# LiYu0524/Domain-RAG

Hardware: AMD Instinct MI355X
Metric: composited images/sec @1024^2, 30 Flux-Redux steps (higher is better)
Workload: dtype bf16; 1 GPU; Flux-Redux outpaint (Fill) 1024x1024, 30 steps, batch=8 per GPU (BASELINE configs[2]); global_batch=8, parallelism=dp1, weights=seeded random init of the FLUX.1-Fill-dev architecture

## Files before the change

domain-rag_amd/_lib.py:

```python
from __future__ import annotations

import ctypes
import os

HERE = os.path.dirname(os.path.abspath(__file__))
LIB_PATH = os.path.join(HERE, "lib", "libdomainrag_hip.so")
if os.environ.get("DRAG_LIB"):
    LIB_PATH = os.environ["DRAG_LIB"]

c_void_p, c_int, c_int64, c_float = ctypes.c_void_p, ctypes.c_int32, ctypes.c_int64, ctypes.c_float


class GemmArgs(ctypes.Structure):
    _fields_ = [
        ("A", c_void_p), ("W", c_void_p), ("C", c_void_p),
        ("bias", c_void_p), ("gate", c_void_p), ("resid", c_void_p),
        ("M", c_int), ("N", c_int), ("K", c_int),
        ("lda", c_int), ("a_rows_per_batch", c_int), ("a_batch_stride", c_int64),
        ("ldc", c_int), ("c_rows_per_batch", c_int), ("c_batch_stride", c_int64),
        ("ldg", c_int), ("act", c_int), ("act_n0", c_int), ("out_f32", c_int),
        ("C2", c_void_p), ("ldc2", c_int), ("n_split", c_int),
    ]


class ConvArgs(ctypes.Structure):
    _fields_ = [("x", c_void_p), ("w", c_void_p), ("y", c_void_p), ("bias", c_void_p), ("resid", c_void_p)] + \
               [(n, c_int) for n in ("B", "Ho", "Wo", "Hp", "Wp", "Cin", "Cout", "ldy", "stride", "oy", "ox", "act")]


class ResampleArgs(ctypes.Structure):
    _fields_ = [("src", c_void_p), ("dst", c_void_p), ("tmp", c_void_p), ("batch", c_int), ("channels", c_int),
                ("src_h", c_int), ("src_w", c_int), ("src_image_stride", c_int64), ("src_row_stride", c_int),
                ("out_h", c_int), ("out_w", c_int), ("dst_image_stride", c_int64), ("dst_row_stride", c_int),
                ("kx", c_void_p), ("bx", c_void_p), ("ksize_x", c_int), ("ky", c_void_p), ("by", c_void_p), ("ksize_y", c_int),
                ("tmp_row0", c_int), ("tmp_rows", c_int), ("src_col0", c_int), ("src_row0", c_int)]


class Conv2dF32Args(ctypes.Structure):
    _fields_ = [(n, c_void_p) for n in ("x", "w", "y", "scale", "shift", "addend", "resid")] + \
               [(n, c_int) for n in ("B", "Hi", "Wi", "Cin", "ldx", "Ho", "Wo", "Cout", "ldy", "ld_add", "ld_res",
                                     "KH", "KW", "stride", "pad", "pad_mode", "transposed", "act")]


SIGNATURES = {
    "drag_version": (c_int, []),
    "drag_last_error": (ctypes.c_char_p, []),
    "drag_set_option": (c_int, [ctypes.c_char_p, c_int]),
    "drag_get_option": (c_int, [ctypes.c_char_p, ctypes.POINTER(ctypes.c_int32)]),
    "drag_option_name": (ctypes.c_char_p, [c_int]),
    "drag_experiments_built": (c_int, []),
    "drag_gemm_bf16": (c_int, [ctypes.POINTER(GemmArgs), c_void_p]),
    "drag_gemm_bf16_pair": (c_int, [ctypes.POINTER(GemmArgs), ctypes.POINTER(GemmArgs), c_void_p]),
    "drag_gemm_bf16_pair_merges": (c_int, [c_int, c_int, c_int, c_int]),
    "drag_gemm_bf16_choice": (c_int, [c_int, c_int, c_int, c_int]),
    "drag_conv3x3_bf16_choice": (c_int, [c_int64, c_int, c_int]),
    "drag_gemm_bf16_cost": (c_int64, [c_int, c_int, c_int, c_int]),
    "drag_gemm_set_workspace": (c_int, [c_void_p, c_int64]),
    "drag_gemm_bf16_splitk_slices": (c_int, [ctypes.POINTER(GemmArgs)]),
    "drag_gemm_bf16_pair_splitk_slices": (c_int, [ctypes.POINTER(GemmArgs), ctypes.POINTER(GemmArgs)]),
    "drag_qk_norm_rope_vt_bf16": (c_int, [c_void_p] * 8 + [c_int] * 5 + [c_float, c_void_p]),
    "drag_attention_bf16": (c_int, [c_void_p] * 4 + [c_int] * 4 + [c_int64, c_int, c_int64, c_float, c_void_p]),
    "drag_k_norm_rope_vt_bf16": (c_int, [c_void_p] * 6 + [c_int] * 5 + [c_float, c_void_p]),
    "drag_attention_qprep_bf16": (c_int, [c_void_p] * 4 + [c_int] * 4 + [c_int64, c_int, c_int64, c_float] + [c_void_p] * 4 + [c_int, c_float, c_void_p]),
    "drag_attention_bf16_choice": (c_int, [c_int, c_int, c_int]),
    "drag_attention_v_bf16": (c_int, [c_void_p] * 4 + [c_int] * 4 + [c_int64, c_int, c_int64, c_float] + [c_void_p] * 4 + [c_int, c_float, c_void_p]),
    "drag_layernorm_modulate_bf16": (c_int, [c_void_p] * 6 + [c_int] * 4 + [c_int64, c_int, c_int, c_float, c_void_p]),
    "drag_act_bf16": (c_int, [c_void_p, c_void_p, c_int64, c_int, c_void_p]),
    "drag_timestep_embedding_bf16": (c_int, [c_void_p, c_void_p, c_int, c_int, c_void_p]),
    "drag_flow_euler_step_bf16": (c_int, [c_void_p, c_void_p, c_float, c_int64, c_void_p]),
    "drag_add_bf16": (c_int, [c_void_p, c_void_p, c_void_p, c_int64, c_void_p]),
    "drag_cast_f32_to_bf16": (c_int, [c_void_p, c_void_p, c_int64, c_void_p]),
    "drag_cast_bf16_to_f32": (c_int, [c_void_p, c_void_p, c_int64, c_void_p]),
    "drag_cosine_topk_workspace_bytes": (c_int64, [c_int64, c_int]),
    "drag_cosine_topk_f32": (c_int, [c_void_p, c_void_p, c_int64, c_int, c_int, c_int, c_void_p, c_void_p, c_void_p, c_void_p]),
    "drag_cosine_scores_f32": (c_int, [c_void_p, c_void_p, c_int64, c_int, c_int, c_void_p, c_void_p]),
    "drag_l2_normalize_f32": (c_int, [c_void_p, c_int64, c_int, c_void_p]),
    "drag_patchify_u8": (c_int, [c_void_p, c_void_p] + [c_int] * 5 + [ctypes.POINTER(c_float), ctypes.POINTER(c_float), c_void_p]),
    "drag_resample_u8": (c_int, [ctypes.POINTER(ResampleArgs), c_void_p]),
    "drag_scale_sum_bf16": (c_int, [c_void_p, c_void_p, c_void_p, c_int, c_int, c_int64, c_void_p]),
    "drag_resnet_stem_style_workspace_bytes": (c_int64, [c_int] * 3),
    "drag_resnet_stem_style_f32": (c_int, [c_void_p] * 5 + [c_int] * 3 + [c_float, c_void_p, c_void_p]),
    "drag_patchify_f32_nchw": (c_int, [c_void_p, c_void_p] + [c_int] * 5 + [c_void_p]),
    "drag_conv3x3_bf16": (c_int, [ctypes.POINTER(ConvArgs), c_void_p]),
    "drag_groupnorm_workspace_bytes": (c_int64, [c_int] * 4),
    "drag_groupnorm_silu_bf16": (c_int, [c_void_p] * 4 + [c_int] * 7 + [c_float, c_void_p, c_void_p]),
    "drag_pad_copy_bf16": (c_int, [c_void_p, c_void_p] + [c_int] * 5 + [c_void_p]),
    "drag_softmax_rows_f32_bf16": (c_int, [c_void_p, c_void_p, c_int64, c_int, c_int, c_float, c_void_p]),
    "drag_unpack_latents_bf16": (c_int, [c_void_p, c_void_p] + [c_int] * 5 + [c_float, c_float, c_void_p]),
    "drag_sample_pack_latents_bf16": (c_int, [c_void_p] * 3 + [c_int] * 5 + [c_float, c_float, c_void_p]),
    "drag_image_preprocess_u8": (c_int, [c_void_p] * 3 + [c_int] * 4 + [c_void_p]),
    "drag_image_postprocess_u8": (c_int, [c_void_p, c_void_p, c_int64, c_int, c_void_p]),
    "drag_mask_pack_u8": (c_int, [c_void_p, c_void_p] + [c_int] * 4 + [c_void_p]),
    "drag_flow_euler_rows_bf16": (c_int, [c_void_p, c_void_p, c_int64, c_int, c_int, c_int, c_float, c_void_p]),
    "drag_scale_noise_rows_bf16": (c_int, [c_void_p, c_void_p, c_int64, c_int, c_int, c_int, c_float, c_void_p]),
    "drag_conv2d_f32": (c_int, [ctypes.POINTER(Conv2dF32Args), c_void_p]),
    "drag_rfft2_f32": (c_int, [c_void_p] * 3 + [c_int] * 5 + [c_void_p] * 3),
    "drag_irfft2_f32": (c_int, [c_void_p] * 4 + [c_int] * 6 + [c_void_p] * 3),
    "drag_lama_prepare_u8": (c_int, [c_void_p] * 3 + [c_int] * 4 + [c_void_p]),
    "drag_vit_prepare_u8": (c_int, [c_void_p, c_void_p, c_int64, ctypes.POINTER(c_float), ctypes.POINTER(c_float), c_void_p]),
    "drag_vit_prepare_f32": (c_int, [c_void_p, c_void_p, c_int, c_int64, c_void_p]),
    "drag_layernorm_f32": (c_int, [c_void_p] * 4 + [c_int64, c_int, c_int64, c_int64, c_float, c_void_p]),
    "drag_clip_embed_ln_f32": (c_int, [c_void_p] * 6 + [c_int] * 3 + [c_float, c_void_p]),
    "drag_attention_small_f32": (c_int, [c_void_p, c_void_p] + [c_int] * 6 + [c_float, c_void_p]),
    "drag_lama_blend_u8": (c_int, [c_void_p, c_int, c_void_p, c_void_p, c_void_p] + [c_int] * 4 + [c_void_p]),
    "drag_cv_resize_linear_u8_f32": (c_int, [c_void_p] * 5 + [c_int] * 3 + [c_void_p]),
    "drag_textenc_attention_bf16": (c_int, [c_void_p] * 4 + [c_int] * 4 + [c_int64, c_int, c_int64, c_float, c_void_p, c_int, c_int, c_void_p]),
    "drag_t5_rmsnorm_bf16": (c_int, [c_void_p] * 3 + [c_int, c_int, c_float, c_void_p]),
    "drag_gated_new_gelu_bf16": (c_int, [c_void_p, c_void_p, c_int64, c_int, c_void_p]),
    "drag_quick_gelu_bf16": (c_int, [c_void_p, c_void_p, c_int64, c_void_p]),
    "drag_embed_gather_bf16": (c_int, [c_void_p] * 4 + [c_int64, c_int, c_int, c_int64, c_void_p]),
    "drag_file_sizes": (c_int, [c_void_p, c_int64, c_void_p, c_int]),
    "drag_read_files": (c_int, [c_void_p, c_int64, c_void_p, c_void_p, c_void_p, c_int]),
    "drag_jpeg_parse": (c_int, [c_void_p, c_void_p, c_int, c_void_p, c_void_p]),
    "drag_jpeg_decode_rgb": (c_int, [c_void_p] * 4 + [c_int, c_int64, c_int64, c_void_p, c_int64] + [c_void_p] * 5),
    "drag_png_plan": (c_int, [c_int] * 4 + [c_void_p, c_void_p]),
    "drag_png_encode": (c_int, [c_void_p] + [c_int] * 4 + [c_void_p, c_int64, c_void_p, c_int64, c_void_p, c_void_p]),
}

_lib = None


def load() -> ctypes.CDLL:
    global _lib
    if _lib is not None:
        return _lib
    if not os.path.exists(LIB_PATH):
        raise RuntimeError(
            f"{LIB_PATH} not found: the HIP extension has not been built "
            "(run `python -c 'import __graft_entry__ as g; g.build()'`). "
            "domain-rag_amd has no CPU / eager fallback.")
    import torch
    lib = ctypes.CDLL(LIB_PATH)
    for name, (res, args) in SIGNATURES.items():
        fn = getattr(lib, name)
        fn.restype = res
        fn.argtypes = args
    _lib = lib
    return lib


def check(rc: int, what: str) -> None:
    if rc != 0:
        msg = load().drag_last_error().decode(errors="replace")
        raise RuntimeError(f"{what} failed (rc={rc}): {msg}")
```

domain-rag_amd/csrc/attention.hip:

```cpp
#include "drag_common.h"
#pragma clang diagnostic ignored "-Winline-asm"
#include "attn_q64_tile.h"
#ifdef DRAG_EXPERIMENTS
#include "attn_q64_tile_exp.h"
#endif
#include <stdlib.h>
#include <type_traits>

namespace {

struct PrepArgs {
  bf16_t* qkv;
  bf16_t* vt;
  const bf16_t *wq_txt, *wk_txt, *wq_img, *wk_img;
  const float *cosT, *sinT;
  int B, S, H, ld, s_txt, s_pad;
  float eps;
  int skip_q;
};

__global__ __launch_bounds__(256) void qk_norm_rope_vt_kernel(PrepArgs p) {
  __shared__ __attribute__((aligned(16))) bf16_t sv[64 * 136];
  const int tid = threadIdx.x;
  const int s0 = blockIdx.x * 64, h = blockIdx.y, b = blockIdx.z;
// ... 12 lines not shown
      const bool ok = s < p.S;
      const int sc = ok ? s : p.S - 1;
      bf16_t* ptr = base + (long long)sc * p.ld + which * HD + h * 128 + sub * 8;
      const u32x4_t raw = *(const u32x4_t*)ptr;
      float x[8];
#pragma unroll
      for (int j = 0; j < 4; ++j) {
        x[2 * j] = bf2f((bf16_t)(raw[j] & 0xffff));
        x[2 * j + 1] = bf2f((bf16_t)(raw[j] >> 16));
      }
      float ss = 0.f;
#pragma unroll
      for (int j = 0; j < 8; ++j) ss += x[j] * x[j];
      ss += __shfl_xor(ss, 8, 64);
      ss += __shfl_xor(ss, 4, 64);
      ss += __shfl_xor(ss, 2, 64);
      ss += __shfl_xor(ss, 1, 64);
      const float rs = rsqrtf(ss * (1.0f / 128.0f) + p.eps);
      u32x4_t wr = (u32x4_t){0u, 0u, 0u, 0u};
      if (do_norm) {
        const bf16_t* wsel = which == 0 ? (sc < p.s_txt ? p.wq_txt : p.wq_img) : (sc < p.s_txt ? p.wk_txt : p.wk_img);
        wr = *(const u32x4_t*)(wsel + sub * 8);
      }
      f32x4_t c4 = (f32x4_t){1.f, 1.f, 1.f, 1.f}, s4 = (f32x4_t){0.f, 0.f, 0.f, 0.f};
      if (do_rope) {
        c4 = *(const f32x4_t*)(p.cosT + (long long)sc * 64 + sub * 4);
        s4 = *(const f32x4_t*)(p.sinT + (long long)sc * 64 + sub * 4);
      }
      u32x4_t o;
#pragma unroll
      for (int j = 0; j < 4; ++j) {
        float a0 = x[2 * j], a1 = x[2 * j + 1];
        if (do_norm) {
          a0 = rbf(rbf(a0 * rs) * bf2f((bf16_t)(wr[j] & 0xffff)));
          a1 = rbf(rbf(a1 * rs) * bf2f((bf16_t)(wr[j] >> 16)));
        }
        const float r0 = a0 * c4[j] - a1 * s4[j];
        const float r1 = a1 * c4[j] + a0 * s4[j];
        o[j] = pack2bf(r0, r1);
      }
      if (ok) *(u32x4_t*)ptr = o;
    }
  }

  if (p.vt == nullptr) return;
  for (int i = tid; i < 64 * 16; i += 256) {
    const int r = i >> 4, c = i & 15;
    const int s = s0 + r;
    u32x4_t v = (u32x4_t){0u, 0u, 0u, 0u};
    if (s < p.S) v = *(const u32x4_t*)(base + (long long)s * p.ld + 2 * HD + h * 128 + c * 8);
    *(u32x4_t*)(sv + r * 136 + c * 8) = v;
  }
  __syncthreads();
  bf16_t* vtb = p.vt + ((long long)(b * p.H + h) * 128) * p.s_pad + s0;
  for (int i = tid; i < 128 * 8; i += 256) {
    const int d = i >> 3, g8 = i & 7;
    uint32_t w[4];
#pragma unroll
    for (int j = 0; j < 8; j += 2) {
      const int q0 = 8 * g8 + j, q1 = q0 + 1;
      const int k0 = (q0 & ~15) + 8 * (((q0 & 15) & 7) >> 2) + 4 * ((q0 & 15) >> 3) + (q0 & 3);
      const int k1 = (q1 & ~15) + 8 * (((q1 & 15) & 7) >> 2) + 4 * ((q1 & 15) >> 3) + (q1 & 3);
      w[j >> 1] = (uint32_t)sv[k0 * 136 + d] | ((uint32_t)sv[k1 * 136 + d] << 16);
    }
    *(u32x4_t*)(vtb + (long long)d * p.s_pad + 8 * g8) = (u32x4_t){w[0], w[1], w[2], w[3]};
  }
}

struct AttnArgs {
  const bf16_t *q, *k, *vt;
  const bf16_t* v;
  bf16_t* out;
  int B, S, H, ld_qk, ld_o, s_pad;
  long long qk_bs, o_bs;
  float c;
  unsigned k_bytes, vt_bytes;
  unsigned k_bytes_all, vt_bytes_all;
  const bf16_t *wq_txt, *wq_img;
  const float *cosT, *sinT;
  int s_txt;
  float eps;
  int tune;
  int items;
};

constexpr float DEFER_THR = 8.0f;
constexpr int KT_BYTES = 64 * 256;
constexpr int VT_BYTES = 128 * 128;

template <int NW, int SCHED, bool QPREP, bool PMAX, bool VROW = false, bool PERSIST = false>
__global__ __launch_bounds__(512, 2) void attention_d128_kernel(AttnArgs p) {
  __shared__ __attribute__((aligned(16))) char smem[2 * KT_BYTES + 2 * VT_BYTES];
  const int w = wave_id(), l = lane_id();
  const int hh = l >> 5;
  constexpr int QB = NW * 32;
  constexpr int CPW = 16 / NW;
  const int nqb = (p.S + QB - 1) / QB;
  const int xcd = blockIdx.x & 7;
  int loc = blockIdx.x >> 3;
  const int nloc = ((p.B * p.H + 7) / 8) * nqb;
  const int lstep = PERSIST ? (int)(gridDim.x >> 3) : nloc;
  if (((loc / nqb) * 8 + xcd) >= p.B * p.H) return;
  int b, h, q0;
  unsigned soK, soV;
  auto item_offsets = [&](int lc, int& bb, int& hd, unsigned& ok, unsigned& ov) {
    const int bh = (lc / nqb) * 8 + xcd;
    bb = bh / p.H; hd = bh - bb * p.H;
    ok = (unsigned)(((long long)bb * p.qk_bs + hd * 128) * 2);
    ov = VROW ? ok : (unsigned)((((long long)(bb * p.H + hd)) * 128) * p.s_pad * 2);
  };
  item_offsets(loc, b, h, soK, soV);
  q0 = (loc - (loc / nqb) * nqb) * QB + w * 32;

  bf16x8_t qf[8];
  __amdgpu_buffer_rsrc_t rsK, rsV;
  if constexpr (PERSIST) {
    rsK = __builtin_amdgcn_make_buffer_rsrc((void*)p.k, 0, p.k_bytes_all, 0x00020000);
    rsV = __builtin_amdgcn_make_buffer_rsrc((void*)(VROW ? p.v : p.vt), 0, VROW ? p.k_bytes_all : p.vt_bytes_all, 0x00020000);
  } else {
    const long long kb = ((long long)b * p.qk_bs + h * 128) * 2;
    rsK = __builtin_amdgcn_make_buffer_rsrc((void*)((const char*)p.k + kb), 0, p.k_bytes, 0x00020000);
    if constexpr (VROW) rsV = __builtin_amdgcn_make_buffer_rsrc((void*)((const char*)p.v + kb), 0, p.k_bytes, 0x00020000);
    else rsV = __builtin_amdgcn_make_buffer_rsrc((void*)((const char*)p.vt + (long long)(b * p.H + h) * 128 * p.s_pad * 2), 0, p.vt_bytes, 0x00020000);
    soK = 0; soV = 0;
  }
  unsigned soKn = soK, soVn = soV;
  int krow[4];
  unsigned kslot[4], voff[4];
  const unsigned vrslot = (unsigned)(((l & 15) ^ (4 * ((l >> 4) & 3))) * 16);
#pragma unroll
  for (int i = 0; i < 4; ++i) {
    if (i >= CPW) break;
    const int c = w * CPW + i;
    krow[i] = c * 4 + (l >> 4);
    kslot[i] = (unsigned)(((l & 15) ^ (krow[i] & 15)) * 16);
    const int vrow = c * 8 + (l >> 3);
    const int vslot = (l & 7) ^ ((vrow >> 1) & 7);
    voff[i] = (unsigned)(((long long)vrow * p.s_pad + vslot * 8) * 2);
  }
  auto stage_k1 = [&](int buf, int kv0, int i) {
    const int c = w * CPW + i;
    const bool nx = PERSIST && kv0 >= p.s_pad;
    const int kvr = nx ? kv0 - p.s_pad : kv0;
    const int kr = min(kvr + krow[i], p.S - 1);
    const unsigned ko = (unsigned)((long long)kr * p.ld_qk * 2) + kslot[i];
    __builtin_amdgcn_raw_ptr_buffer_load_lds(rsK, (DRAG_LDS void*)((DRAG_LDS char*)smem + buf * KT_BYTES + c * 1024), 16, ko, nx ? soKn : soK, 0, 0);
  };
  auto stage_k = [&](int buf, int kv0) {
#pragma unroll
    for (int i = 0; i < 4; ++i) {
      if (i >= CPW) break;
      stage_k1(buf, kv0, i);
    }
  };
  auto stage_v1 = [&](int buf, int kv0, int i) {
    const int c = w * CPW + i;
    const bool nx = PERSIST && kv0 >= p.s_pad;
    const int kvr = nx ? kv0 - p.s_pad : kv0;
    const unsigned so = nx ? soVn : soV;
    DRAG_LDS char* dV = (DRAG_LDS char*)smem + 2 * KT_BYTES + buf * VT_BYTES + c * 1024;
    if constexpr (VROW) {
      const int vr = min(kvr + krow[i], p.S - 1);
      __builtin_amdgcn_raw_ptr_buffer_load_lds(rsV, (DRAG_LDS void*)dV, 16, (unsigned)((long long)vr * p.ld_qk * 2) + vrslot, so, 0, 0);
    } else {
      __builtin_amdgcn_raw_ptr_buffer_load_lds(rsV, (DRAG_LDS void*)dV, 16, voff[i], so + (unsigned)(kvr * 2), 0, 0);
    }
  };
  auto stage_v = [&](int buf, int kv0) {
#pragma unroll
    for (int i = 0; i < 4; ++i) {
      if (i >= CPW) break;
      stage_v1(buf, kv0, i);
    }
  };

  const int krd = (l & 31) * 256;
  const int kx = l & 15;
  const int vrd = (l & 31) * 128;
  const int vx = ((l & 31) >> 1) & 7;

  f32x16_t oacc[4];
  float m_run, l_run;

  const int nkv = p.s_pad / 64;
  f32x16_t scur[2], snext[2];
  {
  int ak[8], av[4];
#pragma unroll
  for (int ks = 0; ks < 8; ++ks) ak[ks] = krd + (((2 * ks + hh) ^ kx) << 4);
#pragma unroll
  for (int s2 = 0; s2 < 4; ++s2) av[s2] = vrd + (((2 * s2 + hh) ^ vx) << 4);
  int avd[4];
  {
    const int si = l & 15, g1 = (l >> 4) & 1;
#pragma unroll
// ... 110 lines not shown
    asm volatile("s_waitcnt vmcnt(0)" ::: "memory");
    __syncthreads();
    const float mt = PMAX ? mt_carry : mask_and_max(sc, kv0);
    if (!__all((mt - m_run) * p.c <= DEFER_THR)) {
      const float m_new = fmaxf(m_run, mt);
      const float alpha = __builtin_amdgcn_exp2f((m_run - m_new) * p.c);
      l_run *= alpha;
      m_run = m_new;
#pragma unroll
      for (int i = 0; i < 4; ++i)
#pragma unroll
        for (int r = 0; r < 16; ++r) oacc[i][r] *= alpha;
    }
    const float nmc = -(m_run * p.c);
    float ps = 0.f;
    u32x4_t pk[4];
    {
      bf16x8_t kf = *(const bf16x8_t*)(smem + (ak[0] + KN));
      bf16x8_t vpipe;
#pragma unroll
      for (int g = 0; g < 16; ++g) {
        const bf16x8_t kcur = kf;
        if (g < 15) {
          const int t1 = (g + 1) >> 3, ks1 = (g + 1) & 7;
          kf = *(const bf16x8_t*)(smem + (ak[ks1] + (KN + t1 * (32 * 256))));
        }
        bf16x8_t vfg;
        if (SCHED == 1 && g >= 4) vfg = read_v((g >> 2) - 1, g & 3, VB);
        if (SCHED == 2) {
          vfg = vpipe;
          if (g >= 3 && g < 15) vpipe = read_v(((g + 1) >> 2) - 1, (g + 1) & 3, VB);
        }
        sn[g >> 3] = __builtin_amdgcn_mfma_f32_32x32x16_bf16(kcur, qf[g & 7], (g & 7) == 0 ? zero16 : sn[g >> 3], 0, 0, 0);
        if (g < CPW) stage_k1(PAR, kv0 + 128, g);
        else if (g < 2 * CPW) stage_v1((PAR + 1) & 1, kv0 + 64, g - CPW);
        float y0, y1;
        asm volatile("v_fma_f32 %0, %2, %4, %5\n\tv_fma_f32 %1, %3, %4, %5"
                     : "=&v"(y0), "=&v"(y1) : "v"(sc[g >> 3][(2 * g) & 15]), "v"(sc[g >> 3][((2 * g) & 15) + 1]), "s"(p.c), "v"(nmc));
        const float e0 = __builtin_amdgcn_exp2f(y0);
        const float e1 = __builtin_amdgcn_exp2f(y1);
        ps += e0 + e1;
        uint32_t wd = pack2bf(e0, e1);
        asm volatile("" : "+v"(wd), "+v"(ps));
        pk[g >> 2][g & 3] = wd;
        if (SCHED >= 1 && g >= 4)
          oacc[g & 3] = __builtin_amdgcn_mfma_f32_32x32x16_bf16(vfg, __builtin_bit_cast(bf16x8_t, pk[(g >> 2) - 1]), oacc[g & 3], 0, 0, 0);
        __builtin_amdgcn_sched_barrier(0);
      }
    }
    l_run += ps;
    bf16x8_t pf[4];
#pragma unroll
    for (int s2 = 0; s2 < 4; ++s2) pf[s2] = __builtin_bit_cast(bf16x8_t, pk[s2]);
#pragma unroll
    for (int s2 = (SCHED >= 1 ? 3 : 0); s2 < 4; ++s2)
#pragma unroll
      for (int dt = 0; dt < 4; ++dt) {
        const bf16x8_t vf = read_v(s2, dt, VB);
        oacc[dt] = __builtin_amdgcn_mfma_f32_32x32x16_bf16(vf, pf[s2], oacc[dt], 0, 0, 0);
      }
    if (PMAX) mt_carry = mask_and_max(sn, kv0 + 64);
  };
  for (int it = 0; it < nkv; it += 2) {
    body(it, std::integral_constant<int, 0>{}, scur, snext);
    if (it + 1 < nkv) body(it + 1, std::integral_constant<int, 1>{}, snext, scur);
  }

  const float lt = l_run + __shfl_xor(l_run, 32, 64);
  const float inv = 1.0f / lt;
  const int qrow = q0 + (l & 31);
  if (p.tune & 2) {
    bf16_t* op = p.out + (long long)b * p.o_bs + (long long)qrow * p.ld_o + h * 128 + 8 * hh;
#pragma unroll
    for (int dt = 0; dt < 4; ++dt)
#pragma unroll
      for (int g = 0; g < 4; g += 2) {
        uint32_t a0 = pack2bf(oacc[dt][4 * g] * inv, oacc[dt][4 * g + 1] * inv);
        uint32_t a1 = pack2bf(oacc[dt][4 * g + 2] * inv, oacc[dt][4 * g + 3] * inv);
        uint32_t b0 = pack2bf(oacc[dt][4 * g + 4] * inv, oacc[dt][4 * g + 5] * inv);
        uint32_t b1 = pack2bf(oacc[dt][4 * g + 6] * inv, oacc[dt][4 * g + 7] * inv);
        const auto r0 = __builtin_amdgcn_permlane32_swap(a0, b0, false, false);
        const auto r1 = __builtin_amdgcn_permlane32_swap(a1, b1, false, false);
        const u32x4_t o = {r0[0], r1[0], r0[1], r1[1]};
        if (qrow < p.S) *(u32x4_t*)(op + 32 * dt + 8 * g) = o;
      }
  } else if (qrow < p.S) {
    bf16_t* op = p.out + (long long)b * p.o_bs + (long long)qrow * p.ld_o + h * 128 + 4 * hh;
#pragma unroll
    for (int dt = 0; dt < 4; ++dt)
#pragma unroll
      for (int g = 0; g < 4; ++g) {
        u32x2_t o;
        o[0] = pack2bf(oacc[dt][4 * g] * inv, oacc[dt][4 * g + 1] * inv);
        o[1] = pack2bf(oacc[dt][4 * g + 2] * inv, oacc[dt][4 * g + 3] * inv);
        *(u32x2_t*)(op + 32 * dt + 8 * g) = o;
      }
  }
  if (!has_next) break;
  loc += lstep;
  item_offsets(loc, b, h, soK, soV);
  q0 = (loc - (loc / nqb) * nqb) * QB + w * 32;
  }
  }
}


#define Q64_MFMA_S0(d, a, b) asm volatile("v_mfma_f32_32x32x16_bf16 %0, %1, %2, 0" : "=&v"(d) : "v"(a), "a"(b))
#define Q64_MFMA_S(d, a, b) asm volatile("v_mfma_f32_32x32x16_bf16 %0, %1, %2, %0" : "+v"(d) : "v"(a), "a"(b))
#define Q64_SETTLE_S(s4) asm volatile("s_nop 15\n\ts_nop 7" : "+v"(s4[0][0]), "+v"(s4[0][1]), "+v"(s4[1][0]), "+v"(s4[1][1]))
#define Q64_SETTLE_O(o, qg) asm volatile("s_nop 15\n\ts_nop 7" : "+a"(o[qg][0]), "+a"(o[qg][1]), "+a"(o[qg][2]), "+a"(o[qg][3]))

template <int OFF>
__device__ __forceinline__ void q64_lds_read(bf16x8_t& d, unsigned addr) { asm volatile("ds_read_b128 %0, %1 offset:%2" : "=v"(d) : "v"(addr), "n"(OFF)); }
template <int N>
__device__ __forceinline__ void q64_landed(bf16x8_t& a) { asm volatile("s_waitcnt lgkmcnt(%1)" : "+v"(a) : "n"(N)); }
template <int N>
__device__ __forceinline__ void q64_landed(bf16x8_t& a, bf16x8_t& b) { asm volatile("s_waitcnt lgkmcnt(%2)" : "+v"(a), "+v"(b) : "n"(N)); }
template <int N>
__device__ __forceinline__ void q64_landed(bf16x8_t& a, bf16x8_t& b, bf16x8_t& c, bf16x8_t& d) {
  asm volatile("s_waitcnt lgkmcnt(%4)" : "+v"(a), "+v"(b), "+v"(c), "+v"(d) : "n"(N));
}
__device__ __forceinline__ void q64_max3(float& d, float a, float b, float c) { asm volatile("v_max3_f32 %0, %1, %2, %3" : "=v"(d) : "v"(a), "v"(b), "v"(c)); }
#define Q64P_MFMA_O(d, a, pw) asm volatile("v_mfma_f32_32x32x16_bf16 %0, %1, %2, %0" : "+a"(d) : "v"(a), "v"(pw))
#define Q64_V1 "v_fma_f32 %[ya0], %[sa0], %[c], %[nma]\n\t"
#define Q64_V2 "v_fma_f32 %[ya1], %[sa1], %[c], %[nma]\n\t"
#define Q64_V3 "v_exp_f32 %[ya0], %[ya0]\n\t"
#define Q64_V4 "v_fma_f32 %[yb0], %[sb0], %[c], %[nmb]\n\t"
#define Q64_V5 "v_exp_f32 %[ya1], %[ya1]\n\t"
#define Q64_V6 "v_fma_f32 %[yb1], %[sb1], %[c], %[nmb]\n\t"
#define Q64_V7 "v_add_f32 %[ta], %[ya0], %[ya1]\n\t"
#define Q64_V8 "v_exp_f32 %[yb0], %[yb0]\n\t"
#define Q64_V9 "v_add_f32 %[psa], %[psa], %[ta]\n\t"
#define Q64_V10 "v_exp_f32 %[yb1], %[yb1]\n\t"
#define Q64_V11 "v_cvt_pk_bf16_f32 %[wa], %[ya0], %[ya1]\n\t"
#define Q64_V12 "v_add_f32 %[tb], %[yb0], %[yb1]\n\t"
#define Q64_V13 "v_add_f32 %[psb], %[psb], %[tb]\n\t"
#define Q64_V14 "v_cvt_pk_bf16_f32 %[wb], %[yb0], %[yb1]"
#define Q64_SC_IN(sc, T, E0) [sa0] "v"(sc[0][T][E0]), [sa1] "v"(sc[0][T][E0 + 1]), [sb0] "v"(sc[1][T][E0]), [sb1] "v"(sc[1][T][E0 + 1])
#define Q64_STEP_HI_A(C0, S0CONS, N, o0_, o1_, vf_, p0_, p1_, s0_, kf_, q0_, d1_, a1_, F1, d2_, a2_, F2, sc, T, E0, cc, nma_, nmb_)        \
  asm volatile("s_waitcnt lgkmcnt(%[n])\n\t" Q64_V1 Q64_V2                                                                                \
               "v_mfma_f32_32x32x16_bf16 %[o0], %[vf], %[p0], %[o0]\n\t"                                                                  \
               "ds_read_b128 %[d1], %[a1] offset:%[f1]\n\t" Q64_V3                                                                        \
               "v_mfma_f32_32x32x16_bf16 %[o1], %[vf], %[p1], %[o1]\n\t"                                                                  \
               "ds_read_b128 %[d2], %[a2] offset:%[f2]\n\t" Q64_V4 Q64_V5 Q64_V6                                                          \
               "v_mfma_f32_32x32x16_bf16 %[s0], %[kf], %[q0], " C0                                                                        \
               : [o0] "+a"(o0_), [o1] "+a"(o1_), [s0] S0CONS(s0_), [d1] "=&v"(d1_), [d2] "=&v"(d2_), [ya0] "=&v"(yA0), [ya1] "=&v"(yA1),  \
                 [yb0] "=&v"(yB0), [yb1] "=&v"(yB1)                                                                                       \
               : [n] "n"(N), [vf] "v"(vf_), [p0] "v"(p0_), [p1] "v"(p1_), [kf] "v"(kf_), [q0] "a"(q0_), [a1] "v"(a1_), [f1] "n"(F1),      \
                 [a2] "v"(a2_), [f2] "n"(F2), Q64_SC_IN(sc, T, E0), [c] "s"(cc), [nma] "v"(nma_), [nmb] "v"(nmb_))
#define Q64_STEP_HI_B(C1, S1CONS, s1_, kf_, q1_)                                                                                          \
  asm volatile(Q64_V7 Q64_V8 Q64_V9 Q64_V10 "v_mfma_f32_32x32x16_bf16 %[s1], %[kf], %[q1], " C1 "\n\t" Q64_V11 Q64_V12 Q64_V13 Q64_V14    \
               : [s1] S1CONS(s1_), [yb0] "+v"(yB0), [yb1] "+v"(yB1), [psa] "+v"(ps[0]), [psb] "+v"(ps[1]), [wa] "=&v"(wA),                \
                 [wb] "=&v"(wB), [ta] "=&v"(sA), [tb] "=&v"(sB)                                                                           \
               : [kf] "v"(kf_), [q1] "a"(q1_), [ya0] "v"(yA0), [ya1] "v"(yA1))
#define Q64_STEP_LO_A(WAIT, READ2, C0, C1, SCONS, N, s0_, s1_, kf_, q0_, q1_, d1_, a1_, F1, d2_, a2_, F2, sc, T, E0, cc, nma_, nmb_)       \
  asm volatile(WAIT Q64_V1 Q64_V2 "v_mfma_f32_32x32x16_bf16 %[s0], %[kf], %[q0], " C0 "\n\t"                                              \
               "ds_read_b128 %[d1], %[a1] offset:%[f1]\n\t" READ2 Q64_V3 Q64_V4 Q64_V5 Q64_V6 Q64_V7                                      \
               "v_mfma_f32_32x32x16_bf16 %[s1], %[kf], %[q1], " C1                                                                        \
               : [s0] SCONS(s0_), [s1] SCONS(s1_), [d1] "=&v"(d1_), [d2] "=&v"(d2_), [ya0] "=&v"(yA0), [ya1] "=&v"(yA1), [yb0] "=&v"(yB0),\
                 [yb1] "=&v"(yB1), [ta] "=&v"(sA)                                                                                         \
               : [n] "n"(N), [kf] "v"(kf_), [q0] "a"(q0_), [q1] "a"(q1_), [a1] "v"(a1_), [f1] "n"(F1), [a2] "v"(a2_), [f2] "n"(F2),       \
                 Q64_SC_IN(sc, T, E0), [c] "s"(cc), [nma] "v"(nma_), [nmb] "v"(nmb_))
#define Q64_STEP_LO_B(kf_)                                                                                                                \
  asm volatile(Q64_V8 Q64_V9 Q64_V10 Q64_V11 Q64_V12 Q64_V13 Q64_V14                                                                      \
               : [yb0] "+v"(yB0), [yb1] "+v"(yB1), [psa] "+v"(ps[0]), [psb] "+v"(ps[1]), [wa] "=&v"(wA), [wb] "=&v"(wB), [tb] "=&v"(sB)   \
               : [ya0] "v"(yA0), [ya1] "v"(yA1), [ta] "v"(sA), "v"(kf_))
template <class F, int G = 0>
__device__ __forceinline__ void q64_unroll16(F&& f) {
  if constexpr (G < 16) {
    f(std::integral_constant<int, G>{});
    q64_unroll16<F, G + 1>(f);
  }
}

#if DRAG_EXP
__device__ unsigned long long g_attn_stamps[512];
#define ATTN_STAMP(slot)                                                                                                  \
  do {                                                                                                                     \
    if (blockIdx.x == 0 && w == 0 && l == 0 && (slot) < 512) g_attn_stamps[(slot)] = __builtin_amdgcn_s_memtime();         \
  } while (0)
#else
#define ATTN_STAMP(slot) do { } while (0)
#endif
template <bool QPREP>
__global__ __launch_bounds__(256, 1) void attention_q64_kernel(AttnArgs p) {
  extern __shared__ __attribute__((aligned(16))) char smem[];
  const int w = wave_id(), l = lane_id();
  ATTN_STAMP(0);
  const int hh = l >> 5;
  constexpr int QB = 256, CPW = 4;
  const int nqb = (p.S + QB - 1) / QB;
  struct Item { int b, h, q0; };
  auto decode = [&](int item, Item& t) -> bool {
    const int xcd = item & 7, loc = item >> 3;
    const int bh = (loc / nqb) * 8 + xcd;
    t.b = bh / p.H;
    t.h = bh - t.b * p.H;
    t.q0 = (loc - (loc / nqb) * nqb) * QB + w * 64;
    return bh < p.B * p.H;
  };
  int item = (int)blockIdx.x;
  Item cur;
  if (!decode(item, cur)) return;

  bf16x8_t qf[2][8];
  auto k_descr = [&](const Item& t) {
    return __builtin_amdgcn_make_buffer_rsrc((void*)(p.k + (long long)t.b * p.qk_bs + t.h * 128), 0, p.k_bytes, 0x00020000);
  };
  auto v_descr = [&](const Item& t) {
    return __builtin_amdgcn_make_buffer_rsrc((void*)(p.vt + ((long long)(t.b * p.H + t.h) * 128) * p.s_pad), 0, p.vt_bytes, 0x00020000);
  };
  __amdgpu_buffer_rsrc_t rsK = k_descr(cur), rsV = v_descr(cur);
  int ksub = 0, vsub = 0;
  unsigned koff[4], voff[4];
#pragma unroll
  for (int i = 0; i < 4; ++i) {
    const int c = w * CPW + i;
    const int krow = c * 4 + (l >> 4);
    koff[i] = (unsigned)krow * (unsigned)(p.ld_qk * 2) + (unsigned)(((l & 15) ^ (krow & 15)) * 16);
    const int vrow = c * 8 + (l >> 3);
    const int vslot = (l & 7) ^ ((vrow >> 1) & 7);
    voff[i] = (unsigned)(((long long)vrow * p.s_pad + vslot * 8) * 2);
  }
  auto stage_k1 = [&](int buf, int kv0, int i) {
    const int c = w * CPW + i;
    const unsigned ko = koff[i] + (unsigned)(kv0 - ksub) * (unsigned)(p.ld_qk * 2);
    __builtin_amdgcn_raw_ptr_buffer_load_lds(rsK, (DRAG_LDS void*)((DRAG_LDS char*)smem + buf * KT_BYTES + c * 1024), 16, ko, 0, 0, 0);
  };
  auto stage_v1 = [&](int buf, int kv0, int i) {
    const int c = w * CPW + i;
    __builtin_amdgcn_raw_ptr_buffer_load_lds(rsV, (DRAG_LDS void*)((DRAG_LDS char*)smem + 2 * KT_BYTES + buf * VT_BYTES + c * 1024),
                                             16, voff[i], (kv0 - vsub) * 2, 0, 0);
  };
  const int krd = (l & 31) * 256, kx = l & 15;
  const int vrd = (l & 31) * 128, vx = ((l & 31) >> 1) & 7;
  int ak[8], av[4];
#pragma unroll
  for (int ks = 0; ks < 8; ++ks) ak[ks] = krd + (((2 * ks + hh) ^ kx) << 4);
#pragma unroll
  for (int s2 = 0; s2 < 4; ++s2) av[s2] = vrd + (((2 * s2 + hh) ^ vx) << 4);
  const unsigned lds0 = (unsigned)(size_t)(DRAG_LDS char*)smem;
  unsigned akl[8], avl[4];
  {
#pragma unroll
    for (int i = 0; i < 8; ++i) akl[i] = lds0 + (unsigned)ak[i];
#pragma unroll
    for (int i = 0; i < 4; ++i) avl[i] = lds0 + (unsigned)av[i];
#pragma unroll
    for (int i = 0; i < 8; ++i) asm volatile("" : "+v"(akl[i]));
#pragma unroll
    for (int i = 0; i < 4; ++i) asm volatile("" : "+v"(avl[i]));
  }

  const int nkv = p.s_pad / 64;
  const bool paired = (nkv & 1) == 0 && nkv >= 4;
  const f32x16_t zero16 = {0.f, 0.f, 0.f, 0.f, 0.f, 0.f, 0.f, 0.f, 0.f, 0.f, 0.f, 0.f, 0.f, 0.f, 0.f, 0.f};
  auto stage_first = [&]() {
#pragma unroll
    for (int i = 0; i < 4; ++i) stage_k1(0, 0, i);
#pragma unroll
    for (int i = 0; i < 4; ++i) stage_v1(0, 0, i);
    if (nkv > 1) {
#pragma unroll
      for (int i = 0; i < 4; ++i) stage_k1(1, 64, i);
    }
  };
  auto lane_now = [&]() { int v = l; asm volatile("" : "+v"(v)); return v; };
  DRAG_LDS char* const qlds = (DRAG_LDS char*)smem + 2 * KT_BYTES + 2 * VT_BYTES + w * 16384;
  auto q_request = [&](const Item& t, const int ll) {
    __amdgpu_buffer_rsrc_t rsQ = __builtin_amdgcn_make_buffer_rsrc((void*)(p.q + (long long)t.b * p.qk_bs + t.h * 128), 0, p.k_bytes, 0x00020000);
#pragma unroll
    for (int qg = 0; qg < 2; ++qg) {
      const int qr = min(t.q0 + 32 * qg + (ll & 31), p.S - 1);
      const unsigned vo = (unsigned)qr * (unsigned)(p.ld_qk * 2) + (unsigned)((ll >> 5) * 16);
#pragma unroll
      for (int ks = 0; ks < 8; ++ks)
        __builtin_amdgcn_raw_ptr_buffer_load_lds(rsQ, (DRAG_LDS void*)(qlds + (qg * 8 + ks) * 1024), 16, vo, ks * 32, 0, 0);
    }
  };
  auto q_fragments = [&](const Item& t, const int ll) {
    const int hh = ll >> 5;
// ... 214 lines not shown
        dma();
        Q64_STEP_HI_B("%[s1]", "+v", sn[1][T], kfr[G % 3], qa[1][G & 7]);
      } else if constexpr (G == 8) {
        Q64_STEP_HI_A("0", "=&v", younger, oacc[0][G & 3], oacc[1][G & 3], vfr[G % 3], pk[0][(G >> 2) - 1], pk[1][(G >> 2) - 1], sn[0][T],
                      kfr[G % 3], qa[0][G & 7], kfr[(G + 2) % 3], akl[(G + 2) & 7], KOFF, vfr[(G + 2) % 3], avl[((G + 2) >> 2) - 1], VOFF, sc, T, E0,
                      p.c, nmc[0], nmc[1]);
        dma();
        Q64_STEP_HI_B("0", "=&v", sn[1][T], kfr[G % 3], qa[1][G & 7]);
      } else if constexpr (G >= 4) {
        Q64_STEP_HI_A("%[s0]", "+v", younger, oacc[0][G & 3], oacc[1][G & 3], vfr[G % 3], pk[0][(G >> 2) - 1], pk[1][(G >> 2) - 1], sn[0][T],
                      kfr[G % 3], qa[0][G & 7], kfr[(G + 2) % 3], akl[(G + 2) & 7], KOFF, vfr[(G + 2) % 3], avl[((G + 2) >> 2) - 1], VOFF, sc, T, E0,
                      p.c, nmc[0], nmc[1]);
        dma();
        Q64_STEP_HI_B("%[s1]", "+v", sn[1][T], kfr[G % 3], qa[1][G & 7]);
      } else if constexpr (G == 0) {
        bf16x8_t none;
        Q64_STEP_LO_A("", "", "0", "0", "=&v", 0, sn[0][T], sn[1][T], kfr[0], qa[0][0], qa[1][0], kfr[2], akl[2], KOFF, none, akl[2], 0, sc, T, E0,
                      p.c, nmc[0], nmc[1]);
        dma();
        Q64_STEP_LO_B(kfr[0]);
      } else if constexpr (G == 1) {
        bf16x8_t none;
        Q64_STEP_LO_A("s_waitcnt lgkmcnt(%[n])\n\t", "", "%[s0]", "%[s1]", "+v", younger, sn[0][T], sn[1][T], kfr[G % 3], qa[0][G], qa[1][G],
                      kfr[(G + 2) % 3], akl[G + 2], KOFF, none, akl[2], 0, sc, T, E0, p.c, nmc[0], nmc[1]);
        dma();
        Q64_STEP_LO_B(kfr[G % 3]);
      } else {
        Q64_STEP_LO_A("s_waitcnt lgkmcnt(%[n])\n\t", "ds_read_b128 %[d2], %[a2] offset:%[f2]\n\t", "%[s0]", "%[s1]", "+v", younger, sn[0][T],
                      sn[1][T], kfr[G % 3], qa[0][G], qa[1][G], kfr[(G + 2) % 3], akl[G + 2], KOFF, vfr[(G + 2) % 3], avl[((G + 2) >> 2) - 1], VOFF,
                      sc, T, E0, p.c, nmc[0], nmc[1]);
        dma();
        Q64_STEP_LO_B(kfr[G % 3]);
      }
      pk[0][G >> 2][G & 3] = wA;
      pk[1][G >> 2][G & 3] = wB;
    };
    q64_unroll16(step);
    q64_landed<0>(vtr[0], vtr[1], vtr[2], vtr[3]);
#pragma unroll
    for (int qg = 0; qg < 2; ++qg) l_run[qg] += ps[qg];
  };
  {
    using P0 = std::integral_constant<int, 0>;
    using P1 = std::integral_constant<int, 1>;
    ATTN_STAMP(1);
    body(0, P0{}, scur, snext, std::true_type{});
    if (nkv > 1) body(1, P1{}, snext, scur, std::false_type{});
    for (int it = 2; it < nkv; it += 2) {
      body(it, P0{}, scur, snext, std::false_type{});
      if (it + 1 < nkv) body(it + 1, P1{}, snext, scur, std::false_type{});
    }
#pragma unroll
    for (int dt = 0; dt < 4; ++dt)
#pragma unroll
      for (int qg = 0; qg < 2; ++qg) Q64P_MFMA_O(oacc[qg][dt], vtr[dt], pk[qg][3]);
    ATTN_STAMP(2 + 2 * nkv);
  }
  const int le = lane_now();
  Item nxt = cur;
  if (has_next) {
    decode(item + (int)gridDim.x, nxt);
    q_request(nxt, le);
  }

#pragma unroll
  for (int qg = 0; qg < 2; ++qg) {
    Q64_SETTLE_O(oacc, qg);
    const float lt = l_run[qg] + __shfl_xor(l_run[qg], 32, 64);
    const float inv = 1.0f / lt;
    const int qrow = q0 + 32 * qg + (le & 31);
    if (p.tune & 2) {
      bf16_t* op = p.out + (long long)b * p.o_bs + (long long)qrow * p.ld_o + h * 128 + 8 * (le >> 5);
#pragma unroll
      for (int dt = 0; dt < 4; ++dt)
#pragma unroll
        for (int g = 0; g < 4; g += 2) {
          uint32_t a0 = pack2bf(oacc[qg][dt][4 * g] * inv, oacc[qg][dt][4 * g + 1] * inv);
          uint32_t a1 = pack2bf(oacc[qg][dt][4 * g + 2] * inv, oacc[qg][dt][4 * g + 3] * inv);
          uint32_t b0 = pack2bf(oacc[qg][dt][4 * g + 4] * inv, oacc[qg][dt][4 * g + 5] * inv);
          uint32_t b1 = pack2bf(oacc[qg][dt][4 * g + 6] * inv, oacc[qg][dt][4 * g + 7] * inv);
          const auto r0 = __builtin_amdgcn_permlane32_swap(a0, b0, false, false);
          const auto r1 = __builtin_amdgcn_permlane32_swap(a1, b1, false, false);
          const u32x4_t o = {r0[0], r1[0], r0[1], r1[1]};
          if (qrow < p.S) *(u32x4_t*)(op + 32 * dt + 8 * g) = o;
        }
    } else if (qrow < p.S) {
      bf16_t* op = p.out + (long long)b * p.o_bs + (long long)qrow * p.ld_o + h * 128 + 4 * (le >> 5);
#pragma unroll
      for (int dt = 0; dt < 4; ++dt)
#pragma unroll
        for (int g = 0; g < 4; ++g) {
          u32x2_t o;
          o[0] = pack2bf(oacc[qg][dt][4 * g] * inv, oacc[qg][dt][4 * g + 1] * inv);
          o[1] = pack2bf(oacc[qg][dt][4 * g + 2] * inv, oacc[qg][dt][4 * g + 3] * inv);
          *(u32x2_t*)(op + 32 * dt + 8 * g) = o;
        }
    }
  }
  ATTN_STAMP(3 + 2 * (p.s_pad / 64));
  if (!has_next) break;
  stores_behind = q0 + 64 <= p.S ? ((p.tune & 2) ? 16 : 32) : 0;
  wait_older_than_stores();
  q_fragments(nxt, le);
  q_to_agprs();
  ATTN_STAMP(5 + 2 * (p.s_pad / 64));
  item += (int)gridDim.x;
  cur = nxt;
  if (!paired) {
    rsK = k_descr(cur);
    rsV = v_descr(cur);
  }
  ksub = vsub = 0;
  staged = paired;
  }
}


typedef __attribute__((ext_vector_type(32))) float aq_f32x32_t;
typedef __attribute__((ext_vector_type(8))) uint32_t aq_u32x8_t;
typedef __attribute__((ext_vector_type(16))) uint32_t aq_u32x16_t;

template <bool QPREP, bool FOLD, int VAR = 0>
__global__ __launch_bounds__(256, 1) void attention_q64g_kernel(AttnArgs p) {
  static_assert(QPREP || !FOLD, "the fold needs the q preparation");
  static_assert(VAR == 0 || (FOLD && DRAG_EXP), "variants: fold form, experiment builds");
  extern __shared__ __attribute__((aligned(16))) char smem[];
  const int w = wave_id(), l = lane_id();
  constexpr int QB = 256, CPW = 4;
  const int nqb = (p.S + QB - 1) / QB;
  struct Item { int b, h, q0; };
  auto decode = [&](int item, Item& t) -> bool {
    const int xcd = item & 7, loc = item >> 3;
    const int bh = (loc / nqb) * 8 + xcd;
    t.b = bh / p.H;
    t.h = bh - t.b * p.H;
    t.q0 = (loc - (loc / nqb) * nqb) * QB + w * 64;
    return bh < p.B * p.H;
  };
  int item = (int)blockIdx.x;
  Item cur;
  if (!decode(item, cur)) return;
  auto k_descr = [&](const Item& t) {
    return __builtin_amdgcn_make_buffer_rsrc((void*)(p.k + (long long)t.b * p.qk_bs + t.h * 128), 0, p.k_bytes, 0x00020000);
  };
  auto v_descr = [&](const Item& t) {
    return __builtin_amdgcn_make_buffer_rsrc((void*)(p.vt + ((long long)(t.b * p.H + t.h) * 128) * p.s_pad), 0, p.vt_bytes, 0x00020000);
  };
  auto lane_now = [&]() { int v = l; asm volatile("" : "+v"(v)); return v; };
  const unsigned lds0 = (unsigned)(size_t)(DRAG_LDS char*)smem;
  auto lane_consts = [&](int ll, aq_u32x8_t& akl, aq_u32x16_t& misc) {
    const int hh = ll >> 5;
    const int krd = (ll & 31) * 256, kx = ll & 15;
    const int vrd = (ll & 31) * 128, vx = ((ll & 31) >> 1) & 7;
#pragma unroll
    for (int ks = 0; ks < 8; ++ks) akl[ks] = lds0 + (unsigned)(krd + (((2 * ks + hh) ^ kx) << 4));
#pragma unroll
    for (int s2 = 0; s2 < 4; ++s2) misc[s2] = lds0 + (unsigned)(vrd + (((2 * s2 + hh) ^ vx) << 4));
#pragma unroll
    for (int i = 0; i < 4; ++i) {
      const int c = w * CPW + i;
      const int krow = c * 4 + (ll >> 4);
      misc[4 + i] = (unsigned)krow * (unsigned)(p.ld_qk * 2) + (unsigned)(((ll & 15) ^ (krow & 15)) * 16);
      const int vrow = c * 8 + (ll >> 3);
      const int vslot = (ll & 7) ^ ((vrow >> 1) & 7);
      misc[8 + i] = (unsigned)(((long long)vrow * p.s_pad + vslot * 8) * 2);
      misc[12 + i] = 0u;
    }
  };
  auto stage_first = [&](const Item& t, int ll) {
    __amdgpu_buffer_rsrc_t rsK = k_descr(t), rsV = v_descr(t);
#pragma unroll
    for (int i = 0; i < 4; ++i) {
      const int c = w * CPW + i;
      const int krow = c * 4 + (ll >> 4);
      const unsigned ko = (unsigned)krow * (unsigned)(p.ld_qk * 2) + (unsigned)(((ll & 15) ^ (krow & 15)) * 16);
      const int vrow = c * 8 + (ll >> 3);
      const int vslot = (ll & 7) ^ ((vrow >> 1) & 7);
      const unsigned vo = (unsigned)(((long long)vrow * p.s_pad + vslot * 8) * 2);
      __builtin_amdgcn_raw_ptr_buffer_load_lds(rsK, (DRAG_LDS void*)((DRAG_LDS char*)smem + c * 1024), 16, ko, 0, 0, 0);
      __builtin_amdgcn_raw_ptr_buffer_load_lds(rsV, (DRAG_LDS void*)((DRAG_LDS char*)smem + 2 * KT_BYTES + c * 1024), 16, vo, 0, 0, 0);
      __builtin_amdgcn_raw_ptr_buffer_load_lds(rsK, (DRAG_LDS void*)((DRAG_LDS char*)smem + KT_BYTES + c * 1024), 16,
                                               ko + 64u * (unsigned)(p.ld_qk * 2), 0, 0, 0);
    }
  };
  DRAG_LDS char* const qlds = (DRAG_LDS char*)smem + 2 * KT_BYTES + 2 * VT_BYTES + w * 16384;
  auto q_request = [&](const Item& t, const int ll) {
    __amdgpu_buffer_rsrc_t rsQ = __builtin_amdgcn_make_buffer_rsrc((void*)(p.q + (long long)t.b * p.qk_bs + t.h * 128), 0, p.k_bytes, 0x00020000);
#pragma unroll
    for (int qg = 0; qg < 2; ++qg) {
      const int qr = min(t.q0 + 32 * qg + (ll & 31), p.S - 1);
      const unsigned vo = (unsigned)qr * (unsigned)(p.ld_qk * 2) + (unsigned)((ll >> 5) * 16);
#pragma unroll
      for (int ks = 0; ks < 8; ++ks)
        __builtin_amdgcn_raw_ptr_buffer_load_lds(rsQ, (DRAG_LDS void*)(qlds + (qg * 8 + ks) * 1024), 16, vo, ks * 32, 0, 0);
    }
  };
  auto q_fragments = [&](const Item& t, const int ll, aq_f32x32_t (&qin)[2]) {
    const int hh = ll >> 5;
#pragma unroll
    for (int qg = 0; qg < 2; ++qg) {
      u32x4_t raw[8];
#pragma unroll
      for (int ks = 0; ks < 8; ++ks) raw[ks] = *(const DRAG_LDS u32x4_t*)(qlds + (qg * 8 + ks) * 1024 + ll * 16);
      if constexpr (!QPREP) {
#pragma unroll
        for (int ks = 0; ks < 8; ++ks)
#pragma unroll
          for (int j = 0; j < 4; ++j) {
            const uint32_t word = raw[ks][j];
            qin[qg][4 * ks + j] = __builtin_bit_cast(float, word);
          }
      } else {
        const int qr = min(t.q0 + 32 * qg + (ll & 31), p.S - 1);
        const bf16_t* wsel = (qr < p.s_txt ? p.wq_txt : p.wq_img) + hh * 8;
        const float* cp = p.cosT + (long long)qr * 64 + hh * 4;
        const float* sp = p.sinT + (long long)qr * 64 + hh * 4;
        u32x4_t wr[8];
        f32x4_t c4[8], s4[8];
#pragma unroll
// ... 32 lines not shown
  q_request(cur, l);
  asm volatile("s_waitcnt vmcnt(0)" ::: "memory");
  q_fragments(cur, l, qin);
  int stores_behind = 0;
  auto wait_older_than_stores = [&]() {
    if (stores_behind == 16) asm volatile("s_waitcnt vmcnt(16)" ::: "memory");
    else if (stores_behind == 32) asm volatile("s_waitcnt vmcnt(32)" ::: "memory");
    else asm volatile("s_waitcnt vmcnt(0)" ::: "memory");
  };
  for (;;) {
    const int b = cur.b, h = cur.h, q0 = cur.q0;
    const bool has_next = item + (int)gridDim.x < p.items;
    Item nxt = cur;
    const bool have = has_next && decode(item + (int)gridDim.x, nxt);
    const __amdgpu_buffer_rsrc_t rsK = k_descr(cur), rsV = v_descr(cur);
    const __amdgpu_buffer_rsrc_t rsKn = have ? k_descr(nxt) : __builtin_amdgcn_make_buffer_rsrc((void*)p.k, 0, 0, 0x00020000);
    const __amdgpu_buffer_rsrc_t rsVn = have ? v_descr(nxt) : __builtin_amdgcn_make_buffer_rsrc((void*)p.vt, 0, 0, 0x00020000);
    aq_u32x8_t akl;
    aq_u32x16_t misc;
    lane_consts(lane_now(), akl, misc);
    const unsigned ldsw = (unsigned)__builtin_amdgcn_readfirstlane((int)(lds0 + (unsigned)w * 4096u));
    const unsigned npairs = (unsigned)(nkv - 2) / 2u;
    const unsigned ktile = 64u * (unsigned)(p.ld_qk * 2);
    const unsigned nvalid = (unsigned)(p.S - (nkv - 1) * 64);
    wait_older_than_stores();
    __syncthreads();
    aq_f32x32_t o4[4];
    f32x2_t lrun;
    [[maybe_unused]] f32x16_t lacc[2];
#define AQ64_OUTS "={a[0:31]}"(o4[0]), "={a[32:63]}"(o4[1]), "={a[64:95]}"(o4[2]), "={a[96:127]}"(o4[3]), "={v[208:209]}"(lrun)
#define AQ64_INS "{a[128:159]}"(qin[0]), "{a[160:191]}"(qin[1]), "{v[176:183]}"(akl), "{v[184:199]}"(misc), [rsk] "s"(rsK), [rsv] "s"(rsV), \
                 [rskn] "s"(rsKn), [rsvn] "s"(rsVn), [npairs] "s"(npairs), [ktile] "s"(ktile), [nvalid] "s"(nvalid), [ldsw] "s"(ldsw)
    if constexpr (!FOLD) asm volatile(AQ64_ITEM_NOFOLD : AQ64_OUTS : AQ64_INS, [c] "s"(p.c) : AQ64_CLOBBERS);
    else if constexpr (VAR == 0) asm volatile(AQ64_ITEM_FOLD : AQ64_OUTS : AQ64_INS : AQ64_CLOBBERS);
#if DRAG_EXP
    else if constexpr (VAR == 1) asm volatile(AQ64_ITEM_FOLD_V1 : AQ64_OUTS : AQ64_INS : AQ64_CLOBBERS);
    else if constexpr (VAR == 2) asm volatile(AQ64_ITEM_FOLD_V2 : AQ64_OUTS : AQ64_INS : AQ64_CLOBBERS);
    else if constexpr (VAR == 3) asm volatile(AQ64_ITEM_FOLD_V3 : AQ64_OUTS : AQ64_INS : AQ64_CLOBBERS);
    else if constexpr (VAR == 4) asm volatile(AQ64_ITEM_FOLD_V4 : AQ64_OUTS : AQ64_INS : AQ64_CLOBBERS);
    else if constexpr (VAR == 5) asm volatile(AQ64_ITEM_FOLD_V5 : AQ64_OUTS : AQ64_INS : AQ64_CLOBBERS);
    else if constexpr (VAR == 6) asm volatile(AQ64_ITEM_FOLD_V6 : AQ64_OUTS : AQ64_INS : AQ64_CLOBBERS);
    else if constexpr (VAR == 7) asm volatile(AQ64_ITEM_FOLD_V7 : AQ64_OUTS : AQ64_INS : AQ64_CLOBBERS);
    else if constexpr (VAR == 8) asm volatile(AQ64_ITEM_FOLD_V8 : AQ64_OUTS : AQ64_INS : AQ64_CLOBBERS);
    else if constexpr (VAR == 9) asm volatile(AQ64_ITEM_FOLD_V9 : AQ64_OUTS : AQ64_INS : AQ64_CLOBBERS);
    else if constexpr (VAR == 10) asm volatile(AQ64_ITEM_FOLD_V10 : AQ64_OUTS : AQ64_INS : AQ64_CLOBBERS);
    else if constexpr (VAR == 11) asm volatile(AQ64_ITEM_FOLD_V11 : AQ64_OUTS : AQ64_INS : AQ64_CLOBBERS);
    else if constexpr (VAR == 12) asm volatile(AQ64_ITEM_FOLD_V12 : AQ64_OUTS : AQ64_INS : AQ64_CLOBBERS);
    else if constexpr (VAR == 13) asm volatile(AQ64_ITEM_FOLD_V13 : AQ64_OUTS : AQ64_INS : AQ64_CLOBBERS);
    else if constexpr (VAR == 14) asm volatile(AQ64_ITEM_FOLD_V14 : AQ64_OUTS : AQ64_INS : AQ64_CLOBBERS);
    else if constexpr (VAR == 15) asm volatile(AQ64_ITEM_FOLD_V15 : AQ64_OUTS : AQ64_INS : AQ64_CLOBBERS);
    else if constexpr (VAR == 16) asm volatile(AQ64_ITEM_FOLD_V16 : AQ64_OUTS : AQ64_INS : AQ64_CLOBBERS);
    else if constexpr (VAR == 17) asm volatile(AQ64_ITEM_FOLD_V17 : AQ64_OUTS : AQ64_INS : AQ64_CLOBBERS);
    else if constexpr (VAR == 19) asm volatile(AQ64_ITEM_FOLD_V19 : AQ64_OUTS : AQ64_INS : AQ64_CLOBBERS);
    else if constexpr (VAR == 18)
      asm volatile(AQ64_ITEM_FOLD_V18
                   : "={a[0:31]}"(o4[0]), "={a[32:63]}"(o4[1]), "={a[64:95]}"(o4[2]), "={a[96:127]}"(o4[3]), "={a[224:239]}"(lacc[0]), "={a[240:255]}"(lacc[1])
                   : AQ64_INS : AQ64_CLOBBERS_LSUM);
#endif
#undef AQ64_OUTS
#undef AQ64_INS
    const int le = lane_now();
    if (has_next) q_request(nxt, le);
#pragma unroll
    for (int qg = 0; qg < 2; ++qg) {
      float lt;
      if constexpr (VAR == 18) lt = lacc[qg][0];
      else lt = lrun[qg] + __shfl_xor(lrun[qg], 32, 64);
      const float inv = 1.0f / lt;
      const int qrow = q0 + 32 * qg + (le & 31);
      auto oa = [&](int dt, int r) -> float { return o4[2 * qg + (dt >> 1)][16 * (dt & 1) + r]; };
      if (p.tune & 2) {
        bf16_t* op = p.out + (long long)b * p.o_bs + (long long)qrow * p.ld_o + h * 128 + 8 * (le >> 5);
#pragma unroll
        for (int dt = 0; dt < 4; ++dt)
#pragma unroll
          for (int g = 0; g < 4; g += 2) {
            uint32_t a0 = pack2bf(oa(dt, 4 * g) * inv, oa(dt, 4 * g + 1) * inv);
            uint32_t a1 = pack2bf(oa(dt, 4 * g + 2) * inv, oa(dt, 4 * g + 3) * inv);
            uint32_t b0 = pack2bf(oa(dt, 4 * g + 4) * inv, oa(dt, 4 * g + 5) * inv);
            uint32_t b1 = pack2bf(oa(dt, 4 * g + 6) * inv, oa(dt, 4 * g + 7) * inv);
            const auto r0 = __builtin_amdgcn_permlane32_swap(a0, b0, false, false);
            const auto r1 = __builtin_amdgcn_permlane32_swap(a1, b1, false, false);
            const u32x4_t o = {r0[0], r1[0], r0[1], r1[1]};
            if (qrow < p.S) *(u32x4_t*)(op + 32 * dt + 8 * g) = o;
          }
      } else if (qrow < p.S) {
        bf16_t* op = p.out + (long long)b * p.o_bs + (long long)qrow * p.ld_o + h * 128 + 4 * (le >> 5);
#pragma unroll
        for (int dt = 0; dt < 4; ++dt)
#pragma unroll
          for (int g = 0; g < 4; ++g) {
            u32x2_t o;
            o[0] = pack2bf(oa(dt, 4 * g) * inv, oa(dt, 4 * g + 1) * inv);
            o[1] = pack2bf(oa(dt, 4 * g + 2) * inv, oa(dt, 4 * g + 3) * inv);
            *(u32x2_t*)(op + 32 * dt + 8 * g) = o;
          }
      }
    }
    if (!has_next) break;
    stores_behind = q0 + 64 <= p.S ? ((p.tune & 2) ? 16 : 32) : 0;
    wait_older_than_stores();
    q_fragments(nxt, le, qin);
    item += (int)gridDim.x;
    cur = nxt;
  }
}

}

#if DRAG_EXP
extern "C" int drag_debug_attn_stamps(unsigned long long* host, int n) {
  return hipMemcpyFromSymbol(host, HIP_SYMBOL(g_attn_stamps), (size_t)n * sizeof(unsigned long long)) == hipSuccess ? 0 : -1;
}
#endif

extern "C" int drag_qk_norm_rope_vt_bf16(void* qkv, void* vt, const void* wq_txt, const void* wk_txt,
                                         const void* wq_img, const void* wk_img, const float* rope_cos,
                                         const float* rope_sin, int32_t B, int32_t S, int32_t H, int32_t ld,
                                         int32_t s_txt, float eps, void* stream) {
  DRAG_CHECK(qkv && vt, "drag_qk_norm_rope_vt_bf16: null pointer");
  DRAG_CHECK((wq_txt && wk_txt && wq_img && wk_img) || (!wq_txt && !wk_txt && !wq_img && !wk_img),
             "drag_qk_norm_rope_vt_bf16: norm weights are all-or-none");
  DRAG_CHECK((rope_cos == nullptr) == (rope_sin == nullptr), "drag_qk_norm_rope_vt_bf16: cos/sin come in pairs");
  DRAG_CHECK(B > 0 && S > 0 && H > 0 && ld >= 3 * H * 128 && ld % 8 == 0, "drag_qk_norm_rope_vt_bf16: bad shape");
  PrepArgs p;
  p.qkv = (bf16_t*)qkv; p.vt = (bf16_t*)vt;
  p.wq_txt = (const bf16_t*)wq_txt; p.wk_txt = (const bf16_t*)wk_txt;
  p.wq_img = (const bf16_t*)wq_img; p.wk_img = (const bf16_t*)wk_img;
  p.cosT = rope_cos; p.sinT = rope_sin;
  p.B = B; p.S = S; p.H = H; p.ld = ld; p.s_txt = s_txt; p.s_pad = (S + 63) / 64 * 64; p.eps = eps;
  p.skip_q = 0;
  hipLaunchKernelGGL(qk_norm_rope_vt_kernel, dim3((S + 63) / 64, H, B), dim3(256), 0, (hipStream_t)stream, p);
  DRAG_LAUNCH_CHECK();
  return 0;
}

extern "C" int drag_k_norm_rope_vt_bf16(void* qkv, void* vt, const void* wk_txt, const void* wk_img, const float* rope_cos,
                                        const float* rope_sin, int32_t B, int32_t S, int32_t H, int32_t ld, int32_t s_txt,
                                        float eps, void* stream) {
  DRAG_CHECK(qkv, "drag_k_norm_rope_vt_bf16: null pointer");
  DRAG_CHECK((wk_txt == nullptr) == (wk_img == nullptr), "drag_k_norm_rope_vt_bf16: norm weights come in pairs");
  DRAG_CHECK((rope_cos == nullptr) == (rope_sin == nullptr), "drag_k_norm_rope_vt_bf16: cos/sin come in pairs");
  DRAG_CHECK(B > 0 && S > 0 && H > 0 && ld >= 3 * H * 128 && ld % 8 == 0, "drag_k_norm_rope_vt_bf16: bad shape");
  PrepArgs p;
  p.qkv = (bf16_t*)qkv; p.vt = (bf16_t*)vt;
  p.wq_txt = (const bf16_t*)wk_txt; p.wk_txt = (const bf16_t*)wk_txt;
  p.wq_img = (const bf16_t*)wk_img; p.wk_img = (const bf16_t*)wk_img;
  p.cosT = rope_cos; p.sinT = rope_sin;
  p.B = B; p.S = S; p.H = H; p.ld = ld; p.s_txt = s_txt; p.s_pad = (S + 63) / 64 * 64; p.eps = eps;
  p.skip_q = 1;
  hipLaunchKernelGGL(qk_norm_rope_vt_kernel, dim3((S + 63) / 64, H, B), dim3(256), 0, (hipStream_t)stream, p);
  DRAG_LAUNCH_CHECK();
  return 0;
}

static int attention_launch(const void* q, const void* k, const void* vt, void* out, int32_t B, int32_t S, int32_t H,
                            int32_t ld_qk, int64_t qk_batch_stride, int32_t ld_o, int64_t o_batch_stride, float scale,
                            const void* wq_txt, const void* wq_img, const float* rope_cos, const float* rope_sin, int32_t s_txt,
                            float eps, void* stream, bool vrow = false);

static void attention_family(int32_t S, bool vrow, bool& w8, bool& q64) {
  w8 = !drag_opt(DRAG_OPT_ATTN_W4) && S >= 4096;
  const int q64opt = drag_opt(DRAG_OPT_ATTN_Q64);
  q64 = !vrow && q64opt != 2 && ((q64opt == 1 && S >= 1024) || (q64opt == 0 && w8 && (!DRAG_EXP || drag_opt(DRAG_OPT_ATTN_PERSIST) == 0)));
}

static bool attention_generated(int32_t S) {
  const int nkv = (S + 63) / 64;
  return drag_opt(DRAG_OPT_ATTN_GEN) != 1 && nkv % 2 == 0 && nkv >= 4;
}

extern "C" int drag_attention_bf16_choice(int32_t S, int32_t v_row_major, int32_t q_prep) {
  bool w8, q64;
  attention_family(S, v_row_major != 0, w8, q64);
  if (q64 && attention_generated(S)) return q_prep && drag_opt(DRAG_OPT_ATTN_GEN) != 2 ? 641 : 640;
  return q64 ? 64 : (w8 ? 8 : 4);
}

extern "C" int drag_attention_bf16(const void* q, const void* k, const void* vt, void* out, int32_t B, int32_t S,
                                   int32_t H, int32_t ld_qk, int64_t qk_batch_stride, int32_t ld_o,
                                   int64_t o_batch_stride, float scale, void* stream) {
  return attention_launch(q, k, vt, out, B, S, H, ld_qk, qk_batch_stride, ld_o, o_batch_stride, scale, nullptr, nullptr, nullptr,
                          nullptr, 0, 0.f, stream);
}

extern "C" int drag_attention_qprep_bf16(const void* q, const void* k, const void* vt, void* out, int32_t B, int32_t S,
                                         int32_t H, int32_t ld_qk, int64_t qk_batch_stride, int32_t ld_o,
                                         int64_t o_batch_stride, float scale, const void* wq_txt, const void* wq_img,
                                         const float* rope_cos, const float* rope_sin, int32_t s_txt, float eps, void* stream) {
  DRAG_CHECK(wq_txt && wq_img && rope_cos && rope_sin,
             "drag_attention_qprep_bf16: the fused q preparation needs both norm weights and both RoPE tables "
             "(drag_attention_bf16 takes an already prepared q)");
  DRAG_CHECK(s_txt >= 0 && s_txt <= S, "drag_attention_qprep_bf16: 0 <= s_txt <= S");
  return attention_launch(q, k, vt, out, B, S, H, ld_qk, qk_batch_stride, ld_o, o_batch_stride, scale, wq_txt, wq_img, rope_cos,
                          rope_sin, s_txt, eps, stream);
}

extern "C" int drag_attention_v_bf16(const void* q, const void* k, const void* v, void* out, int32_t B, int32_t S, int32_t H,
                                     int32_t ld_qk, int64_t qk_batch_stride, int32_t ld_o, int64_t o_batch_stride, float scale,
                                     const void* wq_txt, const void* wq_img, const float* rope_cos, const float* rope_sin,
                                     int32_t s_txt, float eps, void* stream) {
  const int given = (wq_txt != nullptr) + (wq_img != nullptr) + (rope_cos != nullptr) + (rope_sin != nullptr);
  DRAG_CHECK(given == 0 || given == 4, "drag_attention_v_bf16: the fused q preparation takes both norm weights and both RoPE tables, or none");
  DRAG_CHECK(given == 0 || (s_txt >= 0 && s_txt <= S), "drag_attention_v_bf16: 0 <= s_txt <= S");
  return attention_launch(q, k, v, out, B, S, H, ld_qk, qk_batch_stride, ld_o, o_batch_stride, scale, wq_txt, wq_img, rope_cos,
                          rope_sin, s_txt, eps, stream, true);
}

#if DRAG_EXP
static int persist_slots() {
  const int opt = drag_opt(DRAG_OPT_ATTN_PERSIST);
  if (opt >= 3) return opt;
  static int ncu8 = 0;
  if (ncu8 == 0) {
    int dev = 0, n = 0;
    if (hipGetDevice(&dev) != hipSuccess || hipDeviceGetAttribute(&n, hipDeviceAttributeMultiprocessorCount, dev) != hipSuccess || n <= 0) n = 256;
    ncu8 = n / 8 > 0 ? n / 8 : 1;
  }
  return ncu8;
}
#endif

static int attention_launch(const void* q, const void* k, const void* vt, void* out, int32_t B, int32_t S, int32_t H,
                            int32_t ld_qk, int64_t qk_batch_stride, int32_t ld_o, int64_t o_batch_stride, float scale,
                            const void* wq_txt, const void* wq_img, const float* rope_cos, const float* rope_sin, int32_t s_txt,
                            float eps, void* stream, bool vrow) {
  DRAG_CHECK(q && k && vt && out, "drag_attention_bf16: null pointer");
  DRAG_CHECK(B > 0 && S > 0 && H > 0, "drag_attention_bf16: bad shape");
  DRAG_CHECK(ld_qk % 8 == 0 && ld_o % 4 == 0, "drag_attention_bf16: ld_qk %% 8, ld_o %% 4 required");
  AttnArgs p;
  p.q = (const bf16_t*)q; p.k = (const bf16_t*)k; p.vt = (const bf16_t*)vt; p.v = (const bf16_t*)vt; p.out = (bf16_t*)out;
  p.B = B; p.S = S; p.H = H; p.ld_qk = ld_qk; p.ld_o = ld_o; p.s_pad = (S + 63) / 64 * 64;
  p.qk_bs = qk_batch_stride; p.o_bs = o_batch_stride;
  p.c = scale * 1.4426950408889634f;
  p.wq_txt = (const bf16_t*)wq_txt; p.wq_img = (const bf16_t*)wq_img; p.cosT = rope_cos; p.sinT = rope_sin;
  p.s_txt = s_txt; p.eps = eps;
  const long long kspan = ((long long)(S - 1) * ld_qk + 128) * 2;
  const long long vspan = (long long)128 * p.s_pad * 2;
  DRAG_CHECK(kspan < (1ll << 31), "drag_attention_bf16: K span must be < 2 GiB per (batch, head)");
  p.k_bytes = (unsigned)kspan; p.vt_bytes = (unsigned)vspan;
  const long long kall = ((long long)(B - 1) * qk_batch_stride + (H - 1) * 128) * 2 + kspan, vall = (long long)B * H * vspan;
  const bool fits32 = kall < (1ll << 32) && vall < (1ll << 32);
  p.k_bytes_all = fits32 ? (unsigned)kall : 0u; p.vt_bytes_all = fits32 ? (unsigned)vall : 0u;
  const int groups = (B * H + 7) / 8;
  bool w8, q64;
  attention_family(S, vrow, w8, q64);
  const int QB = (w8 || q64) ? 256 : 128;
  const int nqb2 = (S + QB - 1) / QB;
  const dim3 grid(8 * groups * nqb2);
  const int sched = drag_opt(DRAG_OPT_ATTN_SCHED);
  const bool qprep = wq_txt != nullptr;
  p.tune = drag_opt(DRAG_OPT_ATTN_TUNE);
  if (ld_o % 8 != 0 || ((uintptr_t)out & 15) != 0 || o_batch_stride % 8 != 0) p.tune &= ~2;
  const hipStream_t st = (hipStream_t)stream;
#define DRAG_ATTN_LAUNCH(NW, SC, QP, PM) hipLaunchKernelGGL((attention_d128_kernel<NW, SC, QP, PM>), grid, dim3(NW * 64), 0, st, p)
#define DRAG_ATTN_PICK(NW)                                                                           \
  do {                                                                                               \
    if (DRAG_EXP && sched == 3) { if (qprep) DRAG_ATTN_LAUNCH(NW, DRAG_EXP ? 2 : 1, true, true); else DRAG_ATTN_LAUNCH(NW, DRAG_EXP ? 2 : 1, false, true); }        \
    else if (sched >= 2) { if (qprep) DRAG_ATTN_LAUNCH(NW, 1, true, true); else DRAG_ATTN_LAUNCH(NW, 1, false, true); }   \
    else if (sched == 1) { if (qprep) DRAG_ATTN_LAUNCH(NW, 1, true, false); else DRAG_ATTN_LAUNCH(NW, 1, false, false); } \
    else { if (qprep) DRAG_ATTN_LAUNCH(NW, 0, true, false); else DRAG_ATTN_LAUNCH(NW, 0, false, false); }                 \
  } while (0)
  if (vrow) {
    if (w8) { if (qprep) hipLaunchKernelGGL((attention_d128_kernel<8, 1, true, true, true>), grid, dim3(512), 0, st, p);
              else hipLaunchKernelGGL((attention_d128_kernel<8, 1, false, true, true>), grid, dim3(512), 0, st, p); }
    else { if (qprep) hipLaunchKernelGGL((attention_d128_kernel<4, 1, true, true, true>), grid, dim3(256), 0, st, p);
           else hipLaunchKernelGGL((attention_d128_kernel<4, 1, false, true, true>), grid, dim3(256), 0, st, p); }
  } else if (q64) {
    constexpr int lds64 = 2 * KT_BYTES + 2 * VT_BYTES + 4 * 16384;
    static unsigned long long ready64 = 0;
    static int ncu64 = 0;
    int dev64 = 0;
    (void)hipGetDevice(&dev64);
    if (!((ready64 >> (dev64 & 63)) & 1ull)) {
      DRAG_CHECK(hipFuncSetAttribute(reinterpret_cast<const void*>(&attention_q64_kernel<true>), hipFuncAttributeMaxDynamicSharedMemorySize, lds64) == hipSuccess &&
                 hipFuncSetAttribute(reinterpret_cast<const void*>(&attention_q64_kernel<false>), hipFuncAttributeMaxDynamicSharedMemorySize, lds64) == hipSuccess,
                 "drag_attention: hipFuncSetAttribute(MaxDynamicSharedMemorySize) failed");
      ready64 |= 1ull << (dev64 & 63);
    }
    if (ncu64 == 0) {
      int n = 0;
      if (hipDeviceGetAttribute(&n, hipDeviceAttributeMultiprocessorCount, dev64) != hipSuccess || n <= 0) n = 256;
      ncu64 = (n & ~7) ? (n & ~7) : 8;
    }
    p.items = (int)grid.x;
    const int nkv64 = p.s_pad / 64;
    const int popt = drag_opt(DRAG_OPT_ATTN_WALK);
    const int pgrid = popt >= 8 && popt % 8 == 0 ? popt : ncu64;
    const bool walk = popt != 2 && (B * H) % 8 == 0 && (popt >= 8 || (nkv64 % 2 == 0 && nkv64 >= 4)) && p.items > pgrid;
    const dim3 grid64(walk ? (unsigned)pgrid : grid.x);
    const int gen = drag_opt(DRAG_OPT_ATTN_GEN);
    if (attention_generated(S)) {
      static unsigned long long readyg = 0;
      if (!((readyg >> (dev64 & 63)) & 1ull)) {
        DRAG_CHECK(hipFuncSetAttribute(reinterpret_cast<const void*>(&attention_q64g_kernel<true, true>), hipFuncAttributeMaxDynamicSharedMemorySize, lds64) == hipSuccess &&
                   hipFuncSetAttribute(reinterpret_cast<const void*>(&attention_q64g_kernel<true, false>), hipFuncAttributeMaxDynamicSharedMemorySize, lds64) == hipSuccess &&
                   hipFuncSetAttribute(reinterpret_cast<const void*>(&attention_q64g_kernel<false, false>), hipFuncAttributeMaxDynamicSharedMemorySize, lds64) == hipSuccess,
                   "drag_attention: hipFuncSetAttribute(MaxDynamicSharedMemorySize) failed");
        readyg |= 1ull << (dev64 & 63);
      }
#if DRAG_EXP
      if (qprep && gen >= 11 && gen <= 29) {
#define DRAG_AQV(V_) case 10 + V_: DRAG_CHECK(hipFuncSetAttribute(reinterpret_cast<const void*>(&attention_q64g_kernel<true, true, V_>), hipFuncAttributeMaxDynamicSharedMemorySize, lds64) == hipSuccess, "hipFuncSetAttribute"); \
        hipLaunchKernelGGL((attention_q64g_kernel<true, true, V_>), grid64, dim3(256), lds64, st, p); break
        switch (gen) { DRAG_AQV(1); DRAG_AQV(2); DRAG_AQV(3); DRAG_AQV(4); DRAG_AQV(5); DRAG_AQV(6); DRAG_AQV(7); DRAG_AQV(8); DRAG_AQV(9); DRAG_AQV(10); DRAG_AQV(11); DRAG_AQV(12); DRAG_AQV(13); DRAG_AQV(14); DRAG_AQV(15); DRAG_AQV(16); DRAG_AQV(17); DRAG_AQV(18); DRAG_AQV(19); }
#undef DRAG_AQV
      } else
#endif
      if (qprep && gen != 2) hipLaunchKernelGGL((attention_q64g_kernel<true, true>), grid64, dim3(256), lds64, st, p);
      else if (qprep) hipLaunchKernelGGL((attention_q64g_kernel<true, false>), grid64, dim3(256), lds64, st, p);
      else hipLaunchKernelGGL((attention_q64g_kernel<false, false>), grid64, dim3(256), lds64, st, p);
    } else if (qprep) hipLaunchKernelGGL((attention_q64_kernel<true>), grid64, dim3(256), lds64, st, p);
    else hipLaunchKernelGGL((attention_q64_kernel<false>), grid64, dim3(256), lds64, st, p);
#if DRAG_EXP
  } else if (w8 && sched == 2 && drag_opt(DRAG_OPT_ATTN_PERSIST) != 0 && fits32 && (B * H) % 8 == 0 && (p.s_pad / 64) % 2 == 0 &&
             nqb2 * groups > persist_slots()) {
    const dim3 pgrid(8 * persist_slots());
    if (qprep) hipLaunchKernelGGL((attention_d128_kernel<8, 1, true, true, false, true>), pgrid, dim3(512), 0, st, p);
    else hipLaunchKernelGGL((attention_d128_kernel<8, 1, false, true, false, true>), pgrid, dim3(512), 0, st, p);
#endif
  } else if (w8) DRAG_ATTN_PICK(8); else DRAG_ATTN_PICK(4);
#undef DRAG_ATTN_PICK
#undef DRAG_ATTN_LAUNCH
  DRAG_LAUNCH_CHECK();
  return 0;
}
```

domain-rag_amd/csrc/drag_common.h:

```cpp
#pragma once
#include <hip/hip_runtime.h>
#include <stdint.h>
#include "../../include/domainrag_hip.h"

typedef uint16_t bf16_t;

typedef __attribute__((ext_vector_type(8))) __bf16 bf16x8_t;
typedef __attribute__((ext_vector_type(8))) short short8_t;
typedef __attribute__((ext_vector_type(4))) short short4_t;
typedef __attribute__((ext_vector_type(4))) float f32x4_t;
typedef __attribute__((ext_vector_type(16))) float f32x16_t;
typedef __attribute__((ext_vector_type(4))) uint32_t u32x4_t;
typedef __attribute__((ext_vector_type(2))) uint32_t u32x2_t;

#define DRAG_LDS __attribute__((address_space(3)))

__device__ __forceinline__ float bf2f(bf16_t v) { return __uint_as_float(((uint32_t)v) << 16); }

typedef __attribute__((ext_vector_type(2))) float f32x2_t;
typedef __attribute__((ext_vector_type(2))) __bf16 bf16x2_t;

__device__ __forceinline__ bf16_t f2bf(float f) { return __builtin_bit_cast(bf16_t, (__bf16)f); }
__device__ __forceinline__ uint32_t pack2bf(float lo, float hi) {
  const f32x2_t v = {lo, hi};
  return __builtin_bit_cast(uint32_t, __builtin_convertvector(v, bf16x2_t));
}
__device__ __forceinline__ float rbf(float f) { return bf2f(f2bf(f)); }

__device__ __forceinline__ int wave_id() { return __builtin_amdgcn_readfirstlane((int)(threadIdx.x >> 6)); }
__device__ __forceinline__ int lane_id() { return (int)(threadIdx.x & 63); }

__device__ __forceinline__ float fast_sigmoid(float z) {
  return __builtin_amdgcn_rcpf(1.0f + __builtin_amdgcn_exp2f(-1.4426950408889634f * z));
}
__device__ __forceinline__ float act_gelu_tanh(float x) {
  const float k0 = 0.7978845608028654f, k1 = 0.044715f;
  const float u2 = 2.0f * k0 * x * (1.0f + k1 * x * x);
  return x * fast_sigmoid(u2);
}
__device__ __forceinline__ float act_gelu_erf(float x) { return 0.5f * x * (1.0f + erff(x * 0.7071067811865476f)); }
__device__ __forceinline__ float act_silu(float x) { return x * fast_sigmoid(x); }
__device__ __forceinline__ float act_quick_gelu(float x) { return x * fast_sigmoid(1.702f * x); }


__device__ __forceinline__ float apply_act(float x, int act) {
  switch (act) {
    case DRAG_ACT_GELU_TANH: return act_gelu_tanh(x);
    case DRAG_ACT_SILU: return act_silu(x);
    case DRAG_ACT_QUICK_GELU: return act_quick_gelu(x);
    case DRAG_ACT_GELU_ERF: return act_gelu_erf(x);
    default: return x;
  }
}

__device__ __forceinline__ int xcd_remap(int bid, int nwg) {
  const int q = nwg >> 3, r = nwg & 7;
  const int xcd = bid & 7, loc = bid >> 3;
  return (xcd < r ? xcd * (q + 1) : r * (q + 1) + (xcd - r) * q) + loc;
}

__device__ __forceinline__ float wave_sum(float v) {
#pragma unroll
  for (int m = 32; m >= 1; m >>= 1) v += __shfl_xor(v, m, 64);
  return v;
}
__device__ __forceinline__ float wave_max(float v) {
#pragma unroll
  for (int m = 32; m >= 1; m >>= 1) v = fmaxf(v, __shfl_xor(v, m, 64));
  return v;
}

#define DRAG_OPT_PRODUCT 0
#define DRAG_OPT_EXP_ANY (-1)
#define DRAG_OPTIONS(X)                                     \
  X(ATTN_SCHED, "attn_sched", 2, 3)                         \
  X(ATTN_W4, "attn_w4", 0, DRAG_OPT_PRODUCT)                \
  X(ATTN_TUNE, "attn_tune", 2, DRAG_OPT_PRODUCT)            \
  X(ATTN_Q64, "attn_q64", 0, DRAG_OPT_PRODUCT)              \
  X(GEMM_KERNEL, "gemm_kernel", 0, DRAG_OPT_PRODUCT)        \
  X(LN_GENERIC, "ln_generic", 0, DRAG_OPT_PRODUCT)          \
  X(GEMM_GROUP_M, "gemm_group_m", 0, DRAG_OPT_PRODUCT)      \
  X(TOPK_GRID, "topk_grid", 0, DRAG_OPT_PRODUCT)            \
  X(TOPK_DEPTH, "topk_depth", 0, DRAG_OPT_PRODUCT)          \
  X(ATTN_PERSIST, "attn_persist", 0, DRAG_OPT_EXP_ANY)      \
  X(TOPK_SELECT, "topk_select", 0, DRAG_OPT_PRODUCT)        \
  X(TOPK_DENSE_SAMPLE, "topk_dense_sample", 0, DRAG_OPT_PRODUCT) \
  X(TOPK_QT, "topk_qt", 0, DRAG_OPT_EXP_ANY)                \
  X(GEMM_PAIR, "gemm_pair", 0, DRAG_OPT_PRODUCT)            \
  X(GEMM_EPILOGUE, "gemm_epilogue", 0, DRAG_OPT_PRODUCT)    \
  X(TOPK_PATH, "topk_path", 0, DRAG_OPT_PRODUCT)            \
  X(TOPK_QREG, "topk_qreg", 0, DRAG_OPT_PRODUCT)            \
  X(GEMM_W4, "gemm_w4", 0, DRAG_OPT_PRODUCT)                \
  X(ATTN_WALK, "attn_walk", 0, DRAG_OPT_PRODUCT)            \
  X(GEMM_SPLITK, "gemm_splitk", 0, DRAG_OPT_PRODUCT)        \
  X(ATTN_GEN, "attn_gen", 0, DRAG_OPT_PRODUCT)              \
  X(GEMM_T128, "gemm_t128", 0, DRAG_OPT_PRODUCT)            \
  X(GEMM_NO_96, "gemm_no_96", 0, DRAG_OPT_PRODUCT)          \
  X(GEMM_NO_192, "gemm_no_192", 0, DRAG_OPT_PRODUCT)        \
  X(GEMM_NONPERSISTENT, "gemm_nonpersistent", 0, DRAG_OPT_PRODUCT) \
  X(GEMM_NARROW, "gemm_narrow", 0, DRAG_OPT_PRODUCT)        \
  X(CONV_NO_SMALL_COUT, "conv_no_small_cout", 0, DRAG_OPT_PRODUCT) \
  X(CONV_NO_LIN, "conv_no_lin", 0, DRAG_OPT_PRODUCT)        \
  X(CONV_TILE, "conv_tile", 0, DRAG_OPT_PRODUCT)
#define DRAG_OPT_ENUM(id, name, def, exp) DRAG_OPT_##id,
enum { DRAG_OPTIONS(DRAG_OPT_ENUM) DRAG_OPT_COUNT };
#undef DRAG_OPT_ENUM
int drag_opt(int idx);
#ifdef DRAG_EXPERIMENTS
#define DRAG_EXP 1
#else
#define DRAG_EXP 0
#endif

void drag_set_error(const char* msg);
#define DRAG_CHECK(cond, msg)          \
  do {                                 \
    if (!(cond)) {                     \
      drag_set_error(msg);             \
      return -1;                       \
    }                                  \
  } while (0)
#define DRAG_LAUNCH_CHECK()                                  \
  do {                                                       \
    hipError_t e__ = hipGetLastError();                      \
    if (e__ != hipSuccess) {                                 \
      drag_set_error(hipGetErrorString(e__));                \
      return -2;                                             \
    }                                                        \
  } while (0)
```

domain-rag_amd/csrc/gemm_bf16.hip:

```cpp
#include "drag_common.h"
#pragma clang diagnostic ignored "-Winline-asm"
#include <stdlib.h>

namespace {

constexpr int BM = 128, BN = 128, BK = 64;
constexpr int TILE_BYTES = BM * BK * 2;

struct RowMap {
  int rpb;
  long long bs;
  int ld;
  __device__ __forceinline__ long long off(int r) const {
    int b = r / rpb;
    int s = r - b * rpb;
    return (long long)b * bs + (long long)s * ld;
  }
};

struct ConvMap {
  int Ho, Wo, Hp, Wp, Cin, stride, oy, ox;
  __device__ __forceinline__ long long off(int m) const {
    const int hw = Ho * Wo;
    const int b = m / hw;
// ... 812 lines not shown
  pick_tile(p, (int)blockIdx.x, tm, tn);
  pick_segment(p, tm);
  const int m0 = tm * 256, n0 = tn * 256;
  const long long a0 = p.am.off(m0);
  const int wrows = min(256, p.N - n0);
  const unsigned long long pa = (unsigned long long)(uintptr_t)(p.A + a0), pw = (unsigned long long)(uintptr_t)(p.W + (long long)n0 * p.K);
  auto uni = [](uint32_t v) { return (uint32_t)__builtin_amdgcn_readfirstlane((int)v); };
  const long long a_span = (p.am.off(min(m0 + 255, p.M - 1)) - a0 + p.K) * 2;
  const u32x4_t rsA = {uni((uint32_t)pa), uni((uint32_t)(pa >> 32) & 0xffffu), uni((uint32_t)a_span), 0x00020000u};
  const u32x4_t rsW = {uni((uint32_t)pw), uni((uint32_t)(pw >> 32) & 0xffffu), uni((uint32_t)((long long)wrows * p.K * 2)), 0x00020000u};
  u32x8_t voA, voW;
#pragma unroll
  for (int i = 0; i < 8; ++i) {
    const int row = (w * 8 + i) * 8 + (l >> 3);
    const int slot = (l & 7) ^ ((row >> 1) & 7);
    const int ra = min(m0 + row, p.M - 1);
    voA[i] = (unsigned)((p.am.off(ra) - a0 + slot * 8) * 2);
    const int rw = min(row, wrows - 1);
    voW[i] = (unsigned)(((long long)rw * p.K + slot * 8) * 2);
  }
  const unsigned lds0 = (unsigned)(size_t)(DRAG_LDS char*)smem;
  const unsigned ldsw = (unsigned)__builtin_amdgcn_readfirstlane((int)(lds0 + (unsigned)w * 8192u));
  const int p0 = (l >> 4) ^ ((l & 15) >> 1);
  const int fa = (wr * 128 + (l & 15)) * 128;
  const int fb = A_BYTES + (wc * 128 + (l & 15)) * 128;
  u32x8_t rd;
#pragma unroll
  for (int b = 0; b < 2; ++b)
#pragma unroll
    for (int ks = 0; ks < 2; ++ks) {
      rd[4 * b + ks] = lds0 + (unsigned)(b * STAGE + fa + ((p0 ^ (ks * 4)) << 4));
      rd[4 * b + 2 + ks] = lds0 + (unsigned)(b * STAGE + fb + ((p0 ^ (ks * 4)) << 4));
    }
  f32x32_t accrow[8];
#pragma unroll
  for (int i = 0; i < 8; ++i)
#pragma unroll
    for (int r = 0; r < 32; ++r) accrow[i][r] = 0.f;
  unsigned n2 = (unsigned)(p.K / 128 - 1);
  unsigned soff = 0;
  const u32x2_t wrv = {lds0 + (unsigned)(w * 8192 + l * 16), lds0 + (unsigned)(STAGE + w * 8192 + l * 16)};
#define G4W_OUTS                                                                                                                              \
  "+{a[0:31]}"(accrow[0]), "+{a[32:63]}"(accrow[1]), "+{a[64:95]}"(accrow[2]), "+{a[96:127]}"(accrow[3]), "+{a[128:159]}"(accrow[4]),        \
      "+{a[160:191]}"(accrow[5]), "+{a[192:223]}"(accrow[6]), "+{a[224:255]}"(accrow[7]), [n2] "+s"(n2), [soff] "+s"(soff)
#define G4W_INS "{v[128:135]}"(voA), "{v[136:143]}"(voW), "{v[144:151]}"(rd), [rsa] "s"(rsA), [rsw] "s"(rsW), [ldsw] "s"(ldsw)
  if constexpr (V == 1) {
    asm volatile(G4W_D_STAGE0 G4W_FIRST_READS G4W_D_LOOP G4W_D_TAIL : G4W_OUTS : G4W_INS : G4W_CLOBBERS, "scc", "memory");
  } else if constexpr (V == 2) {
    asm volatile(G4W_D_STAGE0 G4W_FIRST_READS G4W_D2_LOOP G4W_D_TAIL : G4W_OUTS : G4W_INS : G4W_CLOBBERS, "scc", "memory");
  } else if constexpr (V == 3) {
    asm volatile(G4W_D_STAGE0 G4W_FIRST_READS G4W_D2_LOOP_A G4W_D_TAIL : G4W_OUTS : G4W_INS : G4W_CLOBBERS, "scc", "memory");
  } else if constexpr (V == 4) {
    asm volatile(G4W_D_STAGE0 G4W_FIRST_READS G4W_D2_LOOP_B G4W_D_TAIL : G4W_OUTS : G4W_INS : G4W_CLOBBERS, "scc", "memory");
  } else if constexpr (V == 5) {
    asm volatile(G4W_D_STAGE0 G4W_FIRST_READS G4W_D2_LOOP_C G4W_D_TAIL : G4W_OUTS : G4W_INS : G4W_CLOBBERS, "scc", "memory");
  } else {
    asm volatile(G4W_R_STAGE0 G4W_FIRST_READS G4W_R_LOOP G4W_R_TAIL : G4W_OUTS : G4W_INS, "{v[152:153]}"(wrv) : G4W_CLOBBERS_R, "scc", "memory");
  }
#undef G4W_OUTS
#undef G4W_INS
  f32x4_t acc[8][8];
#pragma unroll
  for (int mi = 0; mi < 8; ++mi)
#pragma unroll
    for (int ni = 0; ni < 8; ++ni)
#pragma unroll
      for (int r = 0; r < 4; ++r) acc[mi][ni][r] = accrow[mi][4 * ni + r];
  const GemmKArgs pd = dest_of(p, n0);
  if (p.wide) {
    __syncthreads();
    staged_epilogue<8, 256, 256, 8>(pd, m0, m0 + wr * 128, n0, n0 + wc * 128, l, acc, smem + w * 4096);
  } else {
    wave_epilogue<8, 256, 256, 8>(pd, m0, m0 + wr * 128 + (l & 15), n0, n0 + wc * 128 + (l >> 4) * 4, acc);
  }
}

#endif

typedef __attribute__((ext_vector_type(16))) uint32_t u32x16_t;
struct W4Tile {
  u32x4_t rsA, rsW;
  u32x16_t vo;
  int m0, n0;
};
__device__ __forceinline__ void w4_tile_state(const GemmKArgs& p, int tile, int w, int l, bool valid, W4Tile& t) {
  auto uni = [](uint32_t v) { return (uint32_t)__builtin_amdgcn_readfirstlane((int)v); };
  int tm, tn;
  pick_tile(p, tile, tm, tn);
  const int m0 = __builtin_amdgcn_readfirstlane(tm * 256), n0 = __builtin_amdgcn_readfirstlane(tn * 256);
  t.m0 = m0;
  t.n0 = n0;
  long long a0 = p.am.off(m0);
  const int wrows = min(256, p.N - n0);
  const bf16_t *Ab = p.A, *Wb = p.W;
  if (p.w_boff) {
    const int sl = m0 / p.am.rpb, r = m0 - sl * p.am.rpb;
    Wb += (long long)sl * p.w_boff;
    if (p.split_m1 > 0 && r >= p.split_m1) {
      Ab = p.A2; Wb = p.W2 + (long long)sl * p.w_boff;
      a0 = (long long)sl * p.am.bs + (long long)(r - p.split_m1) * p.am.ld;
    }
  }
  const unsigned long long pa = (unsigned long long)(uintptr_t)(Ab + a0), pw = (unsigned long long)(uintptr_t)(Wb + (long long)n0 * p.ldw);
  const bool interior = m0 + 256 <= p.M && wrows == 256 && m0 / p.am.rpb == (m0 + 255) / p.am.rpb;
  const long long a_span = interior ? ((long long)255 * p.am.ld + p.K) * 2 : (p.am.off(min(m0 + 255, p.M - 1)) - a0 + p.K) * 2;
  t.rsA = (u32x4_t){uni((uint32_t)pa), uni((uint32_t)(pa >> 32) & 0xffffu), valid ? uni((uint32_t)a_span) : 0u, 0x00020000u};
  t.rsW = (u32x4_t){uni((uint32_t)pw), uni((uint32_t)(pw >> 32) & 0xffffu), valid ? uni((uint32_t)(((long long)(wrows - 1) * p.ldw + p.K) * 2)) : 0u, 0x00020000u};
  if (interior) {
#pragma unroll
    for (int i = 0; i < 8; ++i) {
      const int row = (w * 8 + i) * 8 + (l >> 3);
      const int slot = (l & 7) ^ ((row >> 1) & 7);
      t.vo[i] = (unsigned)((row * p.am.ld + slot * 8) * 2);
      t.vo[8 + i] = (unsigned)((row * p.ldw + slot * 8) * 2);
    }
    return;
  }
#pragma unroll
  for (int i = 0; i < 8; ++i) {
    const int row = (w * 8 + i) * 8 + (l >> 3);
    const int slot = (l & 7) ^ ((row >> 1) & 7);
    const int ra = min(m0 + row, p.M - 1);
    t.vo[i] = (unsigned)((p.am.off(ra) - a0 + slot * 8) * 2);
    const int rw = min(row, wrows - 1);
    t.vo[8 + i] = (unsigned)(((long long)rw * p.ldw + slot * 8) * 2);
  }
}

#if DRAG_EXP
__device__ unsigned long long g_w4_stamps[8 * 64];
#define W4_STAMP(slot)                                                                                   \
  do {                                                                                                   \
    if (blockIdx.x == 0 && w == 0 && l == 0 && tile_no < 64) g_w4_stamps[tile_no * 8 + (slot)] = __builtin_amdgcn_s_memtime(); \
  } while (0)
#else
#define W4_STAMP(slot) do { } while (0)
#endif

__global__ __launch_bounds__(256, 1) void gemm_bf16_w4p(GemmKArgs p) {
  constexpr int A_BYTES = 256 * 128, STAGE = 2 * A_BYTES;
  extern __shared__ __attribute__((aligned(16))) char smem[];
  const int w = wave_id();
  const int l = lane_id();
  const int wr = w >> 1, wc = w & 1;
  const int P = (int)gridDim.x;
  const int nwg = p.tiles_m * p.tiles_n;
  int vb = (int)blockIdx.x;
  const unsigned lds0 = (unsigned)(size_t)(DRAG_LDS char*)smem;
  const unsigned ldsw = (unsigned)__builtin_amdgcn_readfirstlane((int)(lds0 + (unsigned)w * 8192u));
  auto lane_now = [&]() { int v = l; asm volatile("" : "+v"(v)); return v; };
  auto args_now = [&]() {
    GemmKArgs q = p;
    asm volatile("" : "+s"(q.tiles_n), "+s"(q.tiles_m), "+s"(q.group_m), "+s"(q.am.rpb), "+s"(q.cm.rpb), "+s"(q.M), "+s"(q.K), "+s"(q.am.ld), "+s"(q.cm.ld), "+s"(q.ldw));
    return q;
  };
  auto read_addrs = [&](int lv) {
    const int p0 = (lv >> 4) ^ ((lv & 15) >> 1);
    const int fa = (wr * 128 + (lv & 15)) * 128;
    const int fb = A_BYTES + (wc * 128 + (lv & 15)) * 128;
    u32x8_t rd;
#pragma unroll
    for (int b = 0; b < 2; ++b)
#pragma unroll
      for (int ks = 0; ks < 2; ++ks) {
        rd[4 * b + ks] = lds0 + (unsigned)(b * STAGE + fa + ((p0 ^ (ks * 4)) << 4));
        rd[4 * b + 2 + ks] = lds0 + (unsigned)(b * STAGE + fb + ((p0 ^ (ks * 4)) << 4));
      }
    return rd;
  };
  W4Tile cur, nxt;
  w4_tile_state(p, vb, w, lane_now(), true, cur);
  unsigned soff = 0;
  asm volatile(G4W_D_STAGE0_NOWAIT : [soff] "+s"(soff)
               : "{v[128:143]}"(cur.vo), [rsa] "s"(cur.rsA), [rsw] "s"(cur.rsW), [ldsw] "s"(ldsw) : "scc", "m0", "memory");
  int stores_behind = 0;
  [[maybe_unused]] int tile_no = 0;
  const bool late = DRAG_EXP && p.w4_late_state != 0;
  if (late) w4_tile_state(args_now(), vb + P < nwg ? vb + P : vb, w, lane_now(), vb + P < nwg, nxt);
  for (;;) {
    W4_STAMP(0);
    const bool have_next = vb + P < nwg;
    const int lt = lane_now();
    if (!late) w4_tile_state(args_now(), have_next ? vb + P : vb, w, lt, have_next, nxt);
    const u32x8_t rd = read_addrs(lt);
    W4_STAMP(1);
    if (stores_behind == 32) asm volatile("s_waitcnt vmcnt(32)" ::: "memory");
    else asm volatile("s_waitcnt vmcnt(0)" ::: "memory");
    W4_STAMP(2);
    f32x32_t accrow[8];
    unsigned n2 = (unsigned)(p.K / 128 - 2);
    asm volatile(G4W_P_FIRST G4W_P_PAIR0 G4W_P_LOOP G4W_P_TAIL
                 : "={a[0:31]}"(accrow[0]), "={a[32:63]}"(accrow[1]), "={a[64:95]}"(accrow[2]), "={a[96:127]}"(accrow[3]),
                   "={a[128:159]}"(accrow[4]), "={a[160:191]}"(accrow[5]), "={a[192:223]}"(accrow[6]), "={a[224:255]}"(accrow[7]),
                   [n2] "+s"(n2), [soff] "+s"(soff)
                 : "{v[128:143]}"(cur.vo), "{v[224:239]}"(nxt.vo), "{v[144:151]}"(rd), [rsa] "s"(cur.rsA), [rsw] "s"(cur.rsW),
                   [rsa2] "s"(nxt.rsA), [rsw2] "s"(nxt.rsW), [ldsw] "s"(ldsw)
                 : G4W_CLOBBERS, "scc", "memory");
    W4_STAMP(3);
    W4Tile nn;
    if (late) {
      const bool have2 = vb + 2 * P < nwg;
      w4_tile_state(args_now(), have2 ? vb + 2 * P : vb, w, lane_now(), have2, nn);
    }
    const int le = lane_now();
    f32x4_t acc[8][8];
#pragma unroll
    for (int mi = 0; mi < 8; ++mi)
#pragma unroll
      for (int ni = 0; ni < 8; ++ni)
#pragma unroll
        for (int r = 0; r < 4; ++r) acc[mi][ni][r] = accrow[mi][4 * ni + r];
    const GemmKArgs pe = args_now();
    const int m0 = cur.m0, n0 = cur.n0;
    const GemmKArgs pd = dest_of(pe, n0);
    bool fast = false;
    if (pd.wide) fast = staged_epilogue<8, 256, 256, 8>(pd, m0, m0 + wr * 128, n0, n0 + wc * 128, le, acc, smem + 2 * STAGE + w * 4096);
    else wave_epilogue<8, 256, 256, 8>(pd, m0, m0 + wr * 128 + (le & 15), n0, n0 + wc * 128 + (le >> 4) * 4, acc);
    stores_behind = fast ? 32 : 0;
    W4_STAMP(4);
    ++tile_no;
    if (!have_next) break;
    cur = nxt;
    if (late) nxt = nn;
    vb += P;
  }
}

constexpr int T2_HALF = 128 * BK * 2;
constexpr int T2_BUF = 4 * T2_HALF;

#define T2_BARRIER()                      \
  do {                                    \
    __builtin_amdgcn_sched_barrier(0);    \
    __builtin_amdgcn_s_barrier();         \
    __builtin_amdgcn_sched_barrier(0);    \
  } while (0)

template <int MODE, bool SEG>
__device__ __forceinline__ void t256_body(const GemmKArgs& p) {
  __shared__ __attribute__((aligned(16))) char smem[2 * T2_BUF + 8 * 2048];
  const int w = wave_id();
  const int l = lane_id();
  const int wr = w >> 2, wc = w & 3;
  const int P = (int)gridDim.x;
  const int nwg = p.tiles_m * p.tiles_n;
  int vb = (int)blockIdx.x;

  __amdgpu_buffer_rsrc_t rsA, rsW;
  unsigned vo[4][2];
  int lo[4][2];
  auto chunk_row0 = [&](int pc, int sub) {
    if (pc == 0) return 8 * sub;
    if (pc == 3) return 64 + 8 * sub;
    if (pc == 1) return sub < 4 ? 8 * sub : 64 + 8 * (sub - 4);
    return sub < 4 ? 32 + 8 * sub : 96 + 8 * (sub - 4);
  };
#pragma unroll
  for (int pc = 0; pc < 4; ++pc)
#pragma unroll
    for (int c2 = 0; c2 < 2; ++c2) {
      const int c = w * 2 + c2, half = c >> 3;
      lo[pc][c2] = ((pc == 0 || pc == 3 ? 0 : 2) + half) * T2_HALF + chunk_row0(pc, c & 7) * 128;
    }
  auto load_state = [&](int tile) {
    int tm, tn;
    pick_tile(p, tile, tm, tn);
    const bf16_t* A = p.A;
    const bf16_t* W = p.W;
    int M = p.M;
    RowMap am = p.am;
    if (SEG && p.seg_tiles_m > 0 && tm >= p.seg_tiles_m) { tm -= p.seg_tiles_m; A = p.A2; W = p.W2; M = p.M2; am = p.am2; }
    const int m0 = tm * 256, n0 = tn * 256;
    const long long a0 = MODE == 0 ? am.off(m0) : p.cv.off(m0);
    rsA = __builtin_amdgcn_make_buffer_rsrc((void*)(A + a0), 0, 0x7ffffff0u, 0x00020000);
    const int wrows = min(256, p.N - n0);
    rsW = __builtin_amdgcn_make_buffer_rsrc((void*)(W + (long long)n0 * p.K), 0, (unsigned)((long long)wrows * p.K * 2),
                                            0x00020000);
#pragma unroll
    for (int pc = 0; pc < 4; ++pc)
#pragma unroll
      for (int c2 = 0; c2 < 2; ++c2) {
        const int c = w * 2 + c2, half = c >> 3;
        const int row = chunk_row0(pc, c & 7) + (l >> 3);
        const int slot = (l & 7) ^ ((row >> 1) & 7);
        if (pc == 0 || pc == 3) {
          const int ra = min(m0 + half * 128 + row, M - 1);
          vo[pc][c2] = (unsigned)(((MODE == 0 ? am.off(ra) : p.cv.off(ra)) - a0 + slot * 8) * 2);
        } else {
          const int rw = min(half * 128 + row, wrows - 1);
          vo[pc][c2] = (unsigned)(((long long)rw * p.K + slot * 8) * 2);
        }
      }
  };
  const int cchunks = MODE == 1 ? p.cv.Cin / BK : 1;
  const int nk = p.K / BK;
// ... 158 lines not shown
  if (best && cbest * 10 <= cost * 9) {
    if (cost_out) *cost_out = cbest;
    return best;
  }
  if (pick != 24 && pick != 23 && M >= 1024 && N >= 256 && K >= 256 && !drag_opt(DRAG_OPT_GEMM_T128)) {
    const long long c256 = ((tile_rows(M1, M2, 256) * ((N + 255) / 256) + 255) / 256) * (256 + 256);
    if (c256 < cost) { pick = 2; cost = c256; }
  }
  if (cost_out) *cost_out = cost;
  return pick;
}

static int t256_grid(int ntiles) {
  static int ncu = 0;
  if (ncu == 0) {
    int dev = 0, n = 0;
    if (hipGetDevice(&dev) != hipSuccess || hipDeviceGetAttribute(&n, hipDeviceAttributeMultiprocessorCount, dev) != hipSuccess || n <= 0)
      n = 256;
    ncu = n & ~7;
    if (ncu == 0) ncu = 8;
  }
  if (drag_opt(DRAG_OPT_GEMM_NONPERSISTENT)) return ntiles;
  return ntiles < ncu ? ntiles : ncu;
}

static int fill_common(GemmKArgs& k, const void* A, const void* W, void* C, const void* bias, const void* gate,
                       const void* resid, int M, int N, int K, int ldc, int c_rpb, long long c_bs, int ldg, int act,
                       int act_n0, int out_f32) {
  k.A = (const bf16_t*)A; k.W = (const bf16_t*)W; k.C = C;
  k.bias = (const bf16_t*)bias; k.gate = (const bf16_t*)gate; k.resid = (const bf16_t*)resid;
  k.M = M; k.N = N; k.K = K;
  k.cm.rpb = c_rpb > 0 ? c_rpb : M; k.cm.bs = c_bs; k.cm.ld = ldc;
  k.ldg = ldg; k.act = act; k.act_n0 = act_n0; k.out_f32 = out_f32;
  k.a_bytes = 0; k.w_bytes = 0;
  k.ldw = K; k.w_boff = 0; k.split_m1 = 0;
  k.C2 = nullptr; k.ld2 = 0; k.n_split = 0;
  k.seg_tiles_m = 0; k.A2 = nullptr; k.W2 = nullptr; k.Cs2 = nullptr; k.bias2 = nullptr; k.gate2 = nullptr; k.resid2 = nullptr;
  k.M2 = 0; k.ldg2 = 0; k.wide2 = 0; k.am2 = RowMap{1, 0, 0}; k.cm2 = RowMap{1, 0, 0};
  k.epi_generic = drag_opt(DRAG_OPT_GEMM_EPILOGUE) == 1;
  k.w4_late_state = drag_opt(DRAG_OPT_GEMM_EPILOGUE) == 2;
  k.group_m = drag_opt(DRAG_OPT_GEMM_GROUP_M) > 0 ? drag_opt(DRAG_OPT_GEMM_GROUP_M) : (K >= 8192 || N >= 16384 ? 4 : 8);
  k.wide = !out_f32 && N % 8 == 0 && ldc % 8 == 0 && ((uintptr_t)C & 15) == 0 && (k.cm.rpb >= M || c_bs % 8 == 0) &&
           (!resid || ((uintptr_t)resid & 15) == 0) && (!gate || (((uintptr_t)gate & 15) == 0 && ldg % 8 == 0)) &&
           !drag_opt(DRAG_OPT_GEMM_NARROW);
  k.tiles_m = (M + BM - 1) / BM; k.tiles_n = (N + BN - 1) / BN;
  return k.tiles_m * k.tiles_n;
}

static int gemm_prepare(GemmKArgs& k, const drag_gemm_args* a, bool k_slices = false) {
  DRAG_CHECK(a != nullptr, "drag_gemm_bf16: null args");
  DRAG_CHECK(a->A && a->W && a->C, "drag_gemm_bf16: null operand pointer");
  DRAG_CHECK(a->M > 0 && a->N > 0 && a->K > 0, "drag_gemm_bf16: M, N, K must be positive");
  DRAG_CHECK(a->K % BK == 0, "drag_gemm_bf16: K must be a multiple of 64 (pad the weight)");
  DRAG_CHECK(a->N % 4 == 0, "drag_gemm_bf16: N must be a multiple of 4");
  DRAG_CHECK(a->lda % 8 == 0 && a->ldc % 4 == 0, "drag_gemm_bf16: lda %% 8 and ldc %% 4 required");
  DRAG_CHECK(!(a->gate && !a->resid), "drag_gemm_bf16: gate needs resid");
  DRAG_CHECK(a->act == DRAG_ACT_NONE || a->act == DRAG_ACT_GELU_TANH || a->act == DRAG_ACT_SILU || a->act == DRAG_ACT_QUICK_GELU,
             "drag_gemm_bf16: fused activation must be none, gelu-tanh, silu or quick-gelu (erf GELU: use drag_act_bf16)");
  fill_common(k, a->A, a->W, a->C, a->bias, a->gate, a->resid, a->M, a->N, a->K, a->ldc, a->c_rows_per_batch, a->c_batch_stride, a->ldg,
              a->act, a->act_n0, a->out_f32);
  k.am.rpb = a->a_rows_per_batch > 0 ? a->a_rows_per_batch : a->M;
  k.am.bs = a->a_batch_stride; k.am.ld = a->lda;
  k.cv = ConvMap{1, 1, 1, 1, 64, 1, 0, 0};
  DRAG_CHECK(k_slices || k.am.rpb >= a->M || k.am.bs >= (long long)(k.am.rpb - 1) * k.am.ld,
             "drag_gemm_bf16: a_batch_stride must not be smaller than one batch of rows");
  DRAG_CHECK(((long long)BM * a->lda + a->K) * 2 < (1ll << 30) && (long long)BN * a->K * 2 < (1ll << 31) &&
                 (k_slices || k.am.rpb >= a->M || (k.am.bs - (long long)(k.am.rpb - 1) * k.am.ld) * 2 < (1ll << 30)),
             "drag_gemm_bf16: tile span too large for 32-bit offsets");
  if (a->C2 != nullptr) {
    DRAG_CHECK(a->n_split > 0 && a->n_split < a->N && a->n_split % 256 == 0, "drag_gemm_bf16: n_split must be a multiple of 256 inside (0, N)");
    DRAG_CHECK(!a->out_f32 && !a->gate && !a->resid && a->c_rows_per_batch <= 0, "drag_gemm_bf16: the two-destination form takes dense bf16 outputs without gate / residual");
    DRAG_CHECK(a->ldc2 >= a->N - a->n_split && a->ldc >= a->n_split, "drag_gemm_bf16: ldc / ldc2 too small for their column ranges");
    k.C2 = a->C2; k.ld2 = a->ldc2; k.n_split = a->n_split;
    k.wide = k.wide && a->ldc2 % 8 == 0 && ((uintptr_t)a->C2 & 15) == 0;
    DRAG_CHECK(k.wide || a->ldc2 % 4 == 0, "drag_gemm_bf16: ldc2 % 4 required");
  }
  return 0;
}

static int gemm_choice(long long M1, long long M2, int N, int K, long long* cost_out = nullptr) {
  const int force = drag_opt(DRAG_OPT_GEMM_KERNEL);
  long long cost = 0;
  int choice;
  const bool w4_ok = M2 == 0 && N >= 256 && K >= 256 && K % 128 == 0;
  if (force >= 10) choice = force;
  else if (force == 3) choice = w4_ok ? 3 : ((N >= 256 && K >= 256) ? 2 : 0);
  else if (force == 2) choice = (N >= 256 && K >= 256) ? 2 : 0;
  else if (force == 1) choice = 0;
  else if (use_t256(M1, M2, N, K)) {
    choice = 2;
    cost = ((tile_rows(M1, M2, 256) * ((N + 255) / 256) + 255) / 256) * (256 + 256);
    const long long tiles4 = tile_rows(M1, 0, 256) * ((N + 255) / 256);
    const int w4 = drag_opt(DRAG_OPT_GEMM_W4);
    const bool enough = w4 == 2 ? true : w4 == 3 ? tiles4 >= 256 : tiles4 >= 256 && (K >= 8192 || tiles4 >= 768);
    if (w4_ok && w4 != 1 && enough) choice = 3;
  } else choice = deep_policy(M1, M2, N, K, &cost);
  if (cost_out) *cost_out = cost;
  return choice;
}

static int gemm_launch(const drag_gemm_args* a, const drag_gemm_args* b, void* stream, int w_total_k = 0, const drag_gemm_args* split_second = nullptr) {
  GemmKArgs k, k2;
  if (int rc = gemm_prepare(k, a, w_total_k > 0)) return rc;
  if (w_total_k > 0) {
    k.ldw = w_total_k; k.w_boff = a->K;
    if (split_second) { k.split_m1 = a->a_rows_per_batch - split_second->M; k.A2 = (const bf16_t*)split_second->A; k.W2 = (const bf16_t*)split_second->W; }
  }
  if (b != nullptr) {
    if (int rc = gemm_prepare(k2, b)) return rc;
    k.A2 = k2.A; k.W2 = k2.W; k.Cs2 = k2.C; k.bias2 = k2.bias; k.gate2 = k2.gate; k.resid2 = k2.resid;
    k.M2 = k2.M; k.ldg2 = k2.ldg; k.wide2 = k2.wide; k.am2 = k2.am; k.cm2 = k2.cm;
  }
  const int choice = w_total_k > 0 ? 3 : gemm_choice(a->M, b ? b->M : 0, a->N, a->K);
  const hipStream_t st_ = (hipStream_t)stream;
  auto tiles_of = [&](int tm) {
    k.tiles_m = (a->M + tm - 1) / tm;
    if (b) { k.seg_tiles_m = k.tiles_m; k.tiles_m += (b->M + tm - 1) / tm; }
  };
  if (choice == 3) {
    k.tiles_m = (a->M + 255) / 256; k.tiles_n = (a->N + 255) / 256;
    if (drag_opt(DRAG_OPT_GEMM_GROUP_M) <= 0) k.group_m = a->N >= 16384 ? 2 : (a->N <= 3072 && a->K < 8192 ? 8 : 4);
    constexpr int lds4 = 131072 + 4 * 4096;
    static unsigned long long ready4 = 0;
    int dev4 = 0;
    (void)hipGetDevice(&dev4);
    if (!((ready4 >> (dev4 & 63)) & 1ull)) {
      DRAG_CHECK(hipFuncSetAttribute(reinterpret_cast<const void*>(&gemm_bf16_w4p), hipFuncAttributeMaxDynamicSharedMemorySize, lds4) == hipSuccess,
                 "drag_gemm_bf16: hipFuncSetAttribute(MaxDynamicSharedMemorySize) failed");
      ready4 |= 1ull << (dev4 & 63);
    }
    hipLaunchKernelGGL(gemm_bf16_w4p, dim3(t256_grid(k.tiles_m * k.tiles_n)), dim3(256), lds4, st_, k);
  } else if (choice == 2) {
    tiles_of(256); k.tiles_n = (a->N + 255) / 256;
    const dim3 g(t256_grid(k.tiles_m * k.tiles_n));
    if (b) hipLaunchKernelGGL(gemm_bf16_t256_pair, g, dim3(512), 0, st_, k);
    else hipLaunchKernelGGL((gemm_bf16_t256<0>), g, dim3(512), 0, st_, k);
  } else if (choice) {
    const int deep = choice;
    const int ni = deep >= 100 ? 6 : 4, mi = (deep % 100) / 10, st = deep % 10;
    DRAG_CHECK((deep >= 400 && deep <= 405) || ((mi >= 1 && mi <= 4) && st >= 2 && st <= 4), "drag_gemm_bf16: gemm_kernel must be 0, 1, 2, 10 * MI + ST or 100 + 10 * MI + ST of a gemm_bf16_deep<MI, ST, NI> that is built");
    tiles_of(deep >= 400 ? 256 : 32 * mi); k.tiles_n = (a->N + 32 * ni - 1) / (32 * ni);
    const dim3 g(k.tiles_m * k.tiles_n);
#define DRAG_DEEP_LAUNCH(MI_, ST_, NI_)                                                                                    \
  {                                                                                                                        \
    constexpr int lds = ST_ * (32 * MI_ + 32 * NI_) * 128;                                                                 \
    static unsigned long long ready = 0;         \
    int dev_ = 0;                                                                                                          \
    (void)hipGetDevice(&dev_);                                                                                             \
    if (!((ready >> (dev_ & 63)) & 1ull)) {                                                                                \
      DRAG_CHECK(hipFuncSetAttribute(reinterpret_cast<const void*>(&gemm_bf16_deep<MI_, ST_, NI_>),                       \
                                     hipFuncAttributeMaxDynamicSharedMemorySize, lds) == hipSuccess,                      \
                 "drag_gemm_bf16: hipFuncSetAttribute(MaxDynamicSharedMemorySize) failed");                               \
      ready |= 1ull << (dev_ & 63);                                                                                        \
    }                                                                                                                      \
    hipLaunchKernelGGL((gemm_bf16_deep<MI_, ST_, NI_>), g, dim3(256), lds, st_, k);                                       \
  }                                                                                                                        \
  break
#define DRAG_DEEP(MI_, ST_) case 10 * MI_ + ST_: DRAG_DEEP_LAUNCH(MI_, ST_, 4)
#define DRAG_DEEP6(MI_, ST_) case 100 + 10 * MI_ + ST_: DRAG_DEEP_LAUNCH(MI_, ST_, 6)
#if DRAG_EXP
    if (deep >= 400 && deep <= 405) {
      DRAG_CHECK(a->K % 128 == 0 && a->K >= 256 && b == nullptr, "drag_gemm_bf16: gemm_kernel 400 (gemm_bf16_w4) needs K % 128 == 0, K >= 256, one segment");
      k.tiles_m = (a->M + 255) / 256; k.tiles_n = (a->N + 255) / 256;
      const dim3 g4(k.tiles_m * k.tiles_n);
#define DRAG_W4(V_) case 400 + V_: DRAG_CHECK(hipFuncSetAttribute(reinterpret_cast<const void*>(&gemm_bf16_w4<V_>), hipFuncAttributeMaxDynamicSharedMemorySize, 131072) == hipSuccess, "hipFuncSetAttribute"); \
      hipLaunchKernelGGL((gemm_bf16_w4<V_>), g4, dim3(256), 131072, st_, k); break
      switch (deep) { DRAG_W4(0); DRAG_W4(1); DRAG_W4(2); DRAG_W4(3); DRAG_W4(4); DRAG_W4(5); default: DRAG_CHECK(false, "drag_gemm_bf16: gemm_kernel 400..405"); }
#undef DRAG_W4
      DRAG_LAUNCH_CHECK();
      return 0;
    }
#endif
    switch (deep) {
      DRAG_DEEP(4, 2); DRAG_DEEP(4, 3);
      DRAG_DEEP(3, 2); DRAG_DEEP(3, 3);
      DRAG_DEEP(2, 2); DRAG_DEEP(2, 3); DRAG_DEEP(2, 4);
      DRAG_DEEP(1, 3); DRAG_DEEP(1, 4);
      DRAG_DEEP6(1, 3); DRAG_DEEP6(2, 3); DRAG_DEEP6(3, 3); DRAG_DEEP6(4, 3);
      DRAG_DEEP6(3, 2); DRAG_DEEP6(4, 2); DRAG_DEEP6(3, 4); DRAG_DEEP6(4, 4);
      default: DRAG_CHECK(false, "drag_gemm_bf16: gemm_kernel names a gemm_bf16_deep<MI, ST, NI> that is not built (42 43 32 33 22 23 24 13 14 | 113 123 133 143 132 142 134 144)");
    }
#undef DRAG_DEEP
#undef DRAG_DEEP6
#undef DRAG_DEEP_LAUNCH
  } else {
    tiles_of(BM); k.tiles_n = (a->N + BN - 1) / BN;
    hipLaunchKernelGGL(gemm_bf16_t128<0>, dim3(k.tiles_m * k.tiles_n), dim3(256), 0, st_, k);
  }
  DRAG_LAUNCH_CHECK();
  return 0;
}

static void* g_splitk_ws[64];
static long long g_splitk_ws_bytes[64];
extern "C" int drag_gemm_set_workspace(void* ptr, int64_t bytes) {
  int dev = 0;
  DRAG_CHECK(hipGetDevice(&dev) == hipSuccess && dev >= 0 && dev < 64, "drag_gemm_set_workspace: no current device");
  DRAG_CHECK((ptr == nullptr) == (bytes <= 0) && ((uintptr_t)ptr & 255) == 0, "drag_gemm_set_workspace: a 256-byte aligned device buffer and its size, or (null, 0)");
  g_splitk_ws[dev] = ptr;
  g_splitk_ws_bytes[dev] = ptr ? (long long)bytes : 0;
  return 0;
}

// ... 47 lines not shown
  if (hipGetDevice(&dev) != hipSuccess || dev < 0 || dev >= 64 || g_splitk_ws[dev] == nullptr) return 0;
  auto fits = [](const drag_gemm_args* x) {
    return x->M % 256 == 0 && x->N % 256 == 0 && !x->out_f32 && !x->C2 && x->act == DRAG_ACT_NONE &&
           !(x->a_rows_per_batch > 0 && x->a_rows_per_batch < x->M) &&
           x->ldc % 4 == 0 && x->ldg % 4 == 0 && !(x->c_rows_per_batch > 0 && x->c_batch_stride % 4);
  };
  if (!fits(a) || (b && (!fits(b) || b->lda != a->lda || b->N != a->N || b->K != a->K))) return 0;
  const long long rows = a->M + (b ? b->M : 0);
  const long long tiles = (rows / 256) * (a->N / 256);
  int best = 0;
  for (int s = 2; s <= 8; ++s) {
    if (a->K % (128 * s) || a->K / s < 1024 || tiles * s > 256) continue;
    if ((long long)s * rows * a->N * 4 > g_splitk_ws_bytes[dev]) continue;
    best = s;
  }
  if (opt >= 2) return (opt <= 8 && a->K % (128 * opt) == 0 && a->K / opt >= 256 && (long long)opt * rows * a->N * 4 <= g_splitk_ws_bytes[dev]) ? opt : 0;
  return (tiles <= 96 && a->K >= 12288) ? best : 0;
}

static int splitk_reduce(const drag_gemm_args* a, int S, int slice_rows, int row0, const float* part, void* stream) {
  SplitReduceArgs r{};
  r.part = part; r.slice_rows = slice_rows; r.row0 = row0; r.C = (bf16_t*)a->C;
  r.bias = (const bf16_t*)a->bias; r.gate = (const bf16_t*)a->gate; r.resid = (const bf16_t*)a->resid;
  r.S = S; r.M = a->M; r.N = a->N; r.ldg = a->ldg;
  r.cm.rpb = a->c_rows_per_batch > 0 ? a->c_rows_per_batch : a->M; r.cm.bs = a->c_batch_stride; r.cm.ld = a->ldc;
  const long long n = (long long)a->M * (a->N / 4);
  const dim3 g((unsigned)((n + 255) / 256));
  switch (S) {
#define DRAG_RED(S_) case S_: hipLaunchKernelGGL(splitk_reduce_kernel<S_>, g, dim3(256), 0, (hipStream_t)stream, r); break
    DRAG_RED(2); DRAG_RED(3); DRAG_RED(4); DRAG_RED(5); DRAG_RED(6); DRAG_RED(7); DRAG_RED(8);
#undef DRAG_RED
    default: DRAG_CHECK(false, "drag_gemm_bf16: 2 ... 8 K slices");
  }
  DRAG_LAUNCH_CHECK();
  return 0;
}

static int gemm_splitk(const drag_gemm_args* a, const drag_gemm_args* b, int S, void* stream) {
  int dev = 0;
  (void)hipGetDevice(&dev);
  const int rows = a->M + (b ? b->M : 0);
  drag_gemm_args v{};
  v.A = a->A; v.W = a->W; v.C = g_splitk_ws[dev];
  v.M = S * rows; v.N = a->N; v.K = a->K / S;
  v.lda = a->lda; v.a_rows_per_batch = rows; v.a_batch_stride = a->K / S;
  v.ldc = a->N; v.c_rows_per_batch = rows; v.c_batch_stride = (long long)rows * a->N;
  v.out_f32 = 1;
  if (int rc = gemm_launch(&v, nullptr, stream, a->K, b)) return rc;
  if (int rc = splitk_reduce(a, S, rows, 0, (const float*)g_splitk_ws[dev], stream)) return rc;
  return b ? splitk_reduce(b, S, rows, a->M, (const float*)g_splitk_ws[dev], stream) : 0;
}

extern "C" int drag_gemm_bf16(const drag_gemm_args* a, void* stream) {
  if (a != nullptr && a->A && a->W && a->C && a->M > 0 && a->N > 0 && a->K > 0) {
    if (const int S = splitk_slices(a)) {
      DRAG_CHECK(!(a->gate && !a->resid), "drag_gemm_bf16: gate needs resid");
      return gemm_splitk(a, nullptr, S, stream);
    }
  }
  return gemm_launch(a, nullptr, stream);
}
extern "C" int drag_gemm_bf16_splitk_slices(const drag_gemm_args* a) { return a ? splitk_slices(a) : 0; }
extern "C" int drag_gemm_bf16_pair_splitk_slices(const drag_gemm_args* a, const drag_gemm_args* b) { return a && b ? splitk_slices(a, b) : 0; }
#if DRAG_EXP
extern "C" int drag_debug_w4_stamps(unsigned long long* host, int n) {
  return hipMemcpyFromSymbol(host, HIP_SYMBOL(g_w4_stamps), (size_t)n * sizeof(unsigned long long)) == hipSuccess ? 0 : -1;
}
#endif

extern "C" int drag_gemm_bf16_choice(int M1, int M2, int N, int K) { return gemm_choice(M1, M2 > 0 ? M2 : 0, N, K); }
extern "C" int64_t drag_gemm_bf16_cost(int M1, int M2, int N, int K) {
  long long c = 0;
  gemm_choice(M1, M2 > 0 ? M2 : 0, N, K, &c);
  return (int64_t)c;
}

extern "C" int drag_gemm_bf16_pair_merges(int M1, int M2, int N, int K) {
  const int opt = drag_opt(DRAG_OPT_GEMM_PAIR);
  if (opt == 1) return 0;
  if (opt == 2) return 1;
  long long c1 = 0, c2 = 0, cm = 0;
  const int k1 = gemm_choice(M1, 0, N, K, &c1);
  const int k2 = gemm_choice(M2, 0, N, K, &c2);
  gemm_choice(M1, M2, N, K, &cm);
  if (cm <= 0) return 0;
  auto persistent = [](int k) { return k == 2 || k == 3; };
  return cm < c1 + c2 || (cm == c1 + c2 && (!persistent(k1) || !persistent(k2)));
}

extern "C" int drag_gemm_bf16_pair(const drag_gemm_args* a, const drag_gemm_args* b, void* stream) {
  DRAG_CHECK(a != nullptr && b != nullptr, "drag_gemm_bf16_pair: null args");
  DRAG_CHECK(a->N == b->N && a->K == b->K, "drag_gemm_bf16_pair: the two problems must share N and K");
  DRAG_CHECK(a->act == b->act && a->act_n0 == b->act_n0 && a->out_f32 == b->out_f32, "drag_gemm_bf16_pair: the two problems must share activation and output type");
  DRAG_CHECK(a->C2 == nullptr && b->C2 == nullptr, "drag_gemm_bf16_pair: no two-destination outputs");
  DRAG_CHECK((a->gate != nullptr) == (b->gate != nullptr) && (a->resid != nullptr) == (b->resid != nullptr) && (a->bias != nullptr) == (b->bias != nullptr),
             "drag_gemm_bf16_pair: the two problems must have the same epilogue operands");
  if (a->A && a->W && a->C && b->A && b->W && b->C && a->M > 0 && b->M > 0 && a->N > 0 && a->K > 0) {
    if (const int S = splitk_slices(a, b)) {
      DRAG_CHECK(!(a->gate && !a->resid), "drag_gemm_bf16_pair: gate needs resid");
      return gemm_splitk(a, b, S, stream);
    }
  }
  if (!drag_gemm_bf16_pair_merges(a->M, b->M, a->N, a->K)) {
    if (int rc = drag_gemm_bf16(a, stream)) return rc;
    return drag_gemm_bf16(b, stream);
  }
  return gemm_launch(a, b, stream);
}

extern "C" int drag_conv3x3_bf16_choice(int64_t M, int Cout, int Cin) { return use_t256(M, 0, Cout, 9 * Cin) ? 2 : 0; }

extern "C" int drag_conv3x3_bf16(const drag_conv_args* a, void* stream) {
  DRAG_CHECK(a != nullptr && a->x && a->w && a->y, "drag_conv3x3_bf16: null pointer");
  DRAG_CHECK(a->B > 0 && a->Ho > 0 && a->Wo > 0 && a->Hp > 0 && a->Wp > 0, "drag_conv3x3_bf16: bad shape");
  DRAG_CHECK(a->Cin % BK == 0, "drag_conv3x3_bf16: Cin must be a multiple of 64 (zero-pad channels)");
  DRAG_CHECK(a->Cout % 4 == 0 && a->ldy % 4 == 0, "drag_conv3x3_bf16: Cout and ldy must be multiples of 4");
  DRAG_CHECK(a->stride == 1 || a->stride == 2, "drag_conv3x3_bf16: stride 1 or 2");
  DRAG_CHECK(a->act == DRAG_ACT_NONE || a->act == DRAG_ACT_GELU_TANH || a->act == DRAG_ACT_SILU || a->act == DRAG_ACT_QUICK_GELU,
             "drag_conv3x3_bf16: fused activation must be none, gelu-tanh, silu or quick-gelu");
  DRAG_CHECK((a->Ho - 1) * a->stride + a->oy + 2 <= a->Hp - 1 && (a->Wo - 1) * a->stride + a->ox + 2 <= a->Wp - 1,
             "drag_conv3x3_bf16: taps leave the padded input");
  GemmKArgs k;
  const long long M = (long long)a->B * a->Ho * a->Wo;
  DRAG_CHECK(M < (1ll << 31), "drag_conv3x3_bf16: too many output pixels");
  const int grid = fill_common(k, a->x, a->w, a->y, a->bias, nullptr, a->resid, (int)M, a->Cout, 9 * a->Cin, a->ldy, 0, 0,
                               0, a->act, 0, 0);
  k.am.rpb = (int)M; k.am.bs = 0; k.am.ld = a->Cin;
  k.cv = ConvMap{a->Ho, a->Wo, a->Hp, a->Wp, a->Cin, a->stride, a->oy, a->ox};
  DRAG_CHECK(((long long)(BM * a->stride + 3 * a->Wp * 2) * a->Cin) * 2 < (1ll << 30), "drag_conv3x3_bf16: tile span too large");
  if (use_t256(M, 0, a->Cout, 9 * a->Cin)) {
    k.tiles_m = (int)((M + 255) / 256); k.tiles_n = (a->Cout + 255) / 256;
    hipLaunchKernelGGL(gemm_bf16_t256<1>, dim3(t256_grid(k.tiles_m * k.tiles_n)), dim3(512), 0, (hipStream_t)stream, k);
  } else
    hipLaunchKernelGGL(gemm_bf16_t128<1>, dim3(grid), dim3(256), 0, (hipStream_t)stream, k);
  DRAG_LAUNCH_CHECK();
  return 0;
}
```

domain-rag_amd/flux.py:

```python
from __future__ import annotations

import math

import torch

import os

from . import ops
from .flux_params import FluxConfig

_SEPARATE_QPREP = os.environ.get("DRAG_QPREP_SEPARATE", "") not in ("", "0")
_FUSED_QKV_MLP = {"": None, "0": False}.get(os.environ.get("DRAG_QKV_MLP_FUSED", ""), True)


def rope_tables(ids: torch.Tensor, axes_dims=(16, 56, 56), theta: float = 10000.0):
    cos, sin = [], []
    pos = ids.detach().to("cpu", torch.float64)
    for i, d in enumerate(axes_dims):
        freqs = 1.0 / (theta ** (torch.arange(0, d, 2, dtype=torch.float64) / d))
        ang = torch.outer(pos[:, i], freqs)
        cos.append(ang.cos().float())
        sin.append(ang.sin().float())
    return torch.cat(cos, dim=1).contiguous(), torch.cat(sin, dim=1).contiguous()

# ... 130 lines not shown
            gp = ops.timestep_embedding(self._g1000, 256)
            h = ops.gemm(gp, w[pre + "guidance_embedder.linear_1.weight"], bias=w[pre + "guidance_embedder.linear_1.bias"], act=ops.ACT_SILU)
            emb = ops.gemm(h, w[pre + "guidance_embedder.linear_2.weight"], bias=w[pre + "guidance_embedder.linear_2.bias"], resid=emb)
        h = ops.gemm(pooled, w[pre + "text_embedder.linear_1.weight"], bias=w[pre + "text_embedder.linear_1.bias"], act=ops.ACT_SILU)
        return ops.gemm(h, w[pre + "text_embedder.linear_2.weight"], bias=w[pre + "text_embedder.linear_2.bias"], resid=emb)

    def forward(self, hidden, enc, pooled, timestep, img_ids, txt_ids, guidance=None, taps: dict | None = None):
        cfg = self.cfg
        D, H = cfg.dim, cfg.num_attention_heads
        F = cfg.mlp_ratio * D
        B, Si, _ = hidden.shape
        St = enc.shape[1]
        S = St + Si
        ws = self._workspace(B, St, Si)
        x, nrm, qkv, vt, attn, catb, mod = ws["x"], ws["nrm"], ws["qkv"], ws["vt"], ws["attn"], ws["cat"], ws["mod"]
        cos, sin = self._rope(txt_ids, img_ids)
        hidden = hidden.contiguous(); enc = enc.contiguous(); pooled = pooled.contiguous()
        Mi, Mt, M = B * Si, B * St, B * S
        x_img = x.view(-1)[St * D:]
        scale = 1.0 / math.sqrt(cfg.attention_head_dim)

        ops.gemm(hidden.view(Mi, -1), self.w["x_embedder.weight"], out=x_img, bias=self.w["x_embedder.bias"], M=Mi,
                 c_rows_per_batch=Si, c_batch_stride=S * D, ldc=D)
        ops.gemm(enc.view(Mt, -1), self.w["context_embedder.weight"], out=x, bias=self.w["context_embedder.bias"], M=Mt,
                 c_rows_per_batch=St, c_batch_stride=S * D, ldc=D)
        if cfg.guidance_embeds and guidance is None:
            raise ValueError("this model has a guidance embedding: pass guidance")
        if timestep is not None:
            self._set_times(torch.as_tensor(timestep, dtype=torch.float32).cpu().reshape(-1),
                            None if guidance is None else torch.as_tensor(guidance, dtype=torch.float32).cpu().reshape(-1))
        temb = self._temb(pooled, cfg.guidance_embeds)
        st = ops.act(temb, ops.ACT_SILU)
        ops.gemm(st, self.mod_w, out=mod, bias=self.mod_b)
        modv = mod.view(-1)
        LM = self.mod_total
        if taps is not None:
            taps["temb"] = temb.clone()
            taps["x_embed"] = x[:, St:].clone(); taps["ctx_embed"] = x[:, :St].clone()

        nrm_img = nrm.view(-1)[: Mi * D]
        nrm_txt = nrm.view(-1)[Mi * D: (Mi + Mt) * D]
        qkv_img = qkv.view(-1)[St * 3 * D:]
        attn_img = attn.view(-1)[St * D:]
        hid = catb.view(-1)
        hid_txt = hid[Mi * F:]

        for i, blk in enumerate(self.double):
            mo, cmo = self.mod_off[(i, "norm1")], self.mod_off[(i, "norm1_context")]
            ops.layernorm(x_img, nrm_img, Mi, D, scale=modv[mo + D:], shift=modv[mo:], ldx=D, rows_per_batch=Si,
                          x_batch_stride=S * D, ld_mod=LM)
            ops.layernorm(x, nrm_txt, Mt, D, scale=modv[cmo + D:], shift=modv[cmo:], ldx=D, rows_per_batch=St,
                          x_batch_stride=S * D, ld_mod=LM)
            ops.gemm_pair(dict(a=nrm_img, w=blk["wqkv"], out=qkv_img, bias=blk["bqkv"], M=Mi, lda=D, c_rows_per_batch=Si,
                               c_batch_stride=S * 3 * D, ldc=3 * D),
                          dict(a=nrm_txt, w=blk["cwqkv"], out=qkv, bias=blk["cbqkv"], M=Mt, lda=D, c_rows_per_batch=St,
                               c_batch_stride=S * 3 * D, ldc=3 * D))
            if _SEPARATE_QPREP:
                ops.qk_norm_rope_vt(qkv, vt, blk["cnq"], blk["cnk"], blk["nq"], blk["nk"], cos, sin, B, S, H, 3 * D, St)
                ops.attention(qkv, qkv.view(-1)[D:], vt, attn, B, S, H, 3 * D, S * 3 * D, D, S * D, scale)
            else:
                ops.k_norm_rope_vt(qkv, vt, blk["cnk"], blk["nk"], cos, sin, B, S, H, 3 * D, St)
                ops.attention_qprep(qkv, qkv.view(-1)[D:], vt, attn, B, S, H, 3 * D, S * 3 * D, D, S * D, scale,
                                    blk["cnq"], blk["nq"], cos, sin, St)
            ops.gemm_pair(dict(a=attn_img, w=blk["wo"], out=x_img, bias=blk["bo"], M=Mi, a_rows_per_batch=Si, a_batch_stride=S * D,
                               lda=D, c_rows_per_batch=Si, c_batch_stride=S * D, ldc=D, gate=modv[mo + 2 * D:], resid=x_img, ldg=LM),
                          dict(a=attn, w=blk["cwo"], out=x, bias=blk["cbo"], M=Mt, a_rows_per_batch=St, a_batch_stride=S * D,
                               lda=D, c_rows_per_batch=St, c_batch_stride=S * D, ldc=D, gate=modv[cmo + 2 * D:], resid=x, ldg=LM))
            ops.layernorm(x_img, nrm_img, Mi, D, scale=modv[mo + 4 * D:], shift=modv[mo + 3 * D:], ldx=D,
                          rows_per_batch=Si, x_batch_stride=S * D, ld_mod=LM)
            ops.layernorm(x, nrm_txt, Mt, D, scale=modv[cmo + 4 * D:], shift=modv[cmo + 3 * D:], ldx=D,
                          rows_per_batch=St, x_batch_stride=S * D, ld_mod=LM)
            ops.gemm_pair(dict(a=nrm_img, w=blk["w1"], out=hid, bias=blk["b1"], act=ops.ACT_GELU_TANH, M=Mi, lda=D, ldc=F),
                          dict(a=nrm_txt, w=blk["cw1"], out=hid_txt, bias=blk["cb1"], act=ops.ACT_GELU_TANH, M=Mt, lda=D, ldc=F))
            ops.gemm_pair(dict(a=hid, w=blk["w2"], out=x_img, bias=blk["b2"], M=Mi, lda=F, c_rows_per_batch=Si,
                               c_batch_stride=S * D, ldc=D, gate=modv[mo + 5 * D:], resid=x_img, ldg=LM),
                          dict(a=hid_txt, w=blk["cw2"], out=x, bias=blk["cb2"], M=Mt, lda=F, c_rows_per_batch=St,
                               c_batch_stride=S * D, ldc=D, gate=modv[cmo + 5 * D:], resid=x, ldg=LM))
            if taps is not None:
                taps[f"double.{i}"] = x.clone()

        cat_mlp = catb.view(-1)[D:]
        fused_qkv_mlp = (3 * D) % 256 == 0 and (_FUSED_QKV_MLP if _FUSED_QKV_MLP is not None else
                                                ops.gemm_cost(M, 3 * D + F, D) * 10 <= (ops.gemm_cost(M, 3 * D, D) + ops.gemm_cost(M, F, D)) * 9)
        for i, blk in enumerate(self.single):
            mo = self.mod_off[("s", i)]
            ops.layernorm(x, nrm, M, D, scale=modv[mo + D:], shift=modv[mo:], ldx=D, ld_mod=LM, rows_per_batch=S,
                          x_batch_stride=S * D)
            if fused_qkv_mlp:
                ops.gemm(nrm, blk["wqkvm"], out=qkv, bias=blk["bqkvm"], act=ops.ACT_GELU_TANH, act_n0=3 * D, M=M, lda=D, ldc=3 * D,
                         out2=cat_mlp, ldc2=D + F, n_split=3 * D)
            else:
                ops.gemm(nrm, blk["wqkvm"][: 3 * D], out=qkv, bias=blk["bqkvm"][: 3 * D], M=M, lda=D, ldc=3 * D)
                ops.gemm(nrm, blk["wqkvm"][3 * D:], out=cat_mlp, bias=blk["bqkvm"][3 * D:], act=ops.ACT_GELU_TANH, M=M, lda=D, ldc=D + F)
            if _SEPARATE_QPREP:
                ops.qk_norm_rope_vt(qkv, vt, blk["nq"], blk["nk"], blk["nq"], blk["nk"], cos, sin, B, S, H, 3 * D, 0)
                ops.attention(qkv, qkv.view(-1)[D:], vt, catb, B, S, H, 3 * D, S * 3 * D, D + F, S * (D + F), scale)
            else:
                ops.k_norm_rope_vt(qkv, vt, blk["nk"], blk["nk"], cos, sin, B, S, H, 3 * D, 0)
                ops.attention_qprep(qkv, qkv.view(-1)[D:], vt, catb, B, S, H, 3 * D, S * 3 * D, D + F, S * (D + F), scale,
                                    blk["nq"], blk["nq"], cos, sin, 0)
            ops.gemm(catb, blk["wo"], out=x, bias=blk["bo"], M=M, lda=D + F, c_rows_per_batch=S, c_batch_stride=S * D,
                     ldc=D, gate=modv[mo + 2 * D:], resid=x, ldg=LM)
            if taps is not None:
                taps[f"single.{i}"] = x.clone()

        mo = self.mod_off["out"]
        ops.layernorm(x_img, nrm_img, Mi, D, scale=modv[mo:], shift=modv[mo + D:], ldx=D, rows_per_batch=Si,
                      x_batch_stride=S * D, ld_mod=LM)
        ops.gemm(nrm_img, self.w["proj_out.weight"], out=ws["out"], bias=self.w["proj_out.bias"], M=Mi, lda=D,
                 ldc=cfg.out_channels)
        return ws["out"].view(B, Si, cfg.out_channels)

    MAX_GRAPHS = 3

    def forward_graphed(self, hidden, enc, pooled, timestep, img_ids, txt_ids, guidance=None):
        t = torch.as_tensor(timestep, dtype=torch.float32).cpu().reshape(-1)
        g = None if guidance is None else torch.as_tensor(guidance, dtype=torch.float32).cpu().reshape(-1)
        rope_key = self._ids_key(txt_ids, img_ids)
        key = (hidden.data_ptr(), enc.data_ptr(), pooled.data_ptr(), tuple(hidden.shape), tuple(enc.shape), tuple(pooled.shape),
               guidance is None, rope_key)
        cache = self.__dict__.setdefault("_graphs", {})
        ent = cache.pop(key, None)
        if ent is None:
            while len(cache) >= self.MAX_GRAPHS:
                cache.pop(next(iter(cache)))
            self._ws_key = self._rope_key = None
            self._t1000 = self._g1000 = None
            self._set_times(t, g)
            rope = self._rope(txt_ids, img_ids)
            ws = self._workspace(hidden.shape[0], enc.shape[1], hidden.shape[1])
            self.forward(hidden, enc, pooled, None, img_ids, txt_ids, g)
            torch.cuda.synchronize()
            graph = torch.cuda.CUDAGraph()
            with torch.cuda.graph(graph):
                out = self.forward(hidden, enc, pooled, None, img_ids, txt_ids, g)
            ent = dict(graph=graph, out=out, ws=ws, rope=rope, times=(self._t1000, self._g1000))
            self._ws_key = self._rope_key = None
            self._t1000 = self._g1000 = None
        cache[key] = ent
        t1000, g1000 = ent["times"]
        t1000.copy_((t.to(torch.bfloat16) * 1000).float())
        if g is not None:
            g1000.copy_((g.to(torch.bfloat16) * 1000).float())
        ent["graph"].replay()
        return ent["out"]

    __call__ = forward
```

domain-rag_amd/ops.py:

```python
from __future__ import annotations

import contextlib
import ctypes
import os

import torch

from . import _lib
from ._lib import GemmArgs, check

ACT_NONE, ACT_GELU_TANH, ACT_SILU, ACT_QUICK_GELU, ACT_GELU_ERF = 0, 1, 2, 3, 4


class GemmRecorder:

    def __init__(self, every: int = 1, f32: bool = False):
        self.every = max(1, int(every))
        self.f32 = f32
        self.events = []
        self.shapes = []
        self.is_conv = []
        self.attn = []

    def totals(self):
# ... 74 lines not shown
            set_option(name, v)
            old.append((name, prev))
        yield
    finally:
        for name, prev in reversed(old):
            set_option(name, prev)


def experiments_built() -> bool:
    return bool(_lib.load().drag_experiments_built())


def _stream() -> int:
    return torch.cuda.current_stream().cuda_stream


def _p(t):
    return None if t is None else ctypes.c_void_p(t.data_ptr())


def _need(t: torch.Tensor, dtype, name: str):
    if not t.is_cuda:
        raise RuntimeError(f"{name}: expected a GPU tensor (domain-rag_amd has no CPU path)")
    if t.dtype != dtype:
        raise TypeError(f"{name}: expected {dtype}, got {t.dtype}")


def _gemm_args(a, w, out, bias, act, act_n0, gate, resid, out_f32, M, a_rows_per_batch, a_batch_stride, lda, c_rows_per_batch,
               c_batch_stride, ldc, ldg, out2, ldc2, n_split):
    _need(a, torch.bfloat16, "gemm.a")
    _need(w, torch.bfloat16, "gemm.w")
    N, K = w.shape
    if not w.is_contiguous():
        raise ValueError("gemm.w must be contiguous [N, K]")
    if M is None:
        M = a.numel() // K
        if lda is None:
            if a.dim() < 2 or a.stride(-1) != 1:
                raise ValueError("gemm.a must have unit inner stride")
            lda = a.stride(-2) if a.dim() >= 2 else K
    if lda is None:
        lda = K
    if out is None:
        out = torch.empty((M, N), dtype=torch.float32 if out_f32 else torch.bfloat16, device=a.device)
    if ldc is None:
        ldc = out.stride(-2) if out.dim() >= 2 and out.stride(-1) == 1 else N
    if c_rows_per_batch == 0 and (out2 is None or (0 < n_split < N and n_split % 256 == 0)):
        def _room(t):
            return t.untyped_storage().nbytes() // t.element_size() - t.storage_offset()
        cols = n_split if out2 is not None else N
        if (M - 1) * ldc + cols > _room(out):
            raise ValueError(f"gemm.out: {M} rows of stride {ldc} x {cols} columns do not fit the destination ({_room(out)} elements from its start)")
        if out2 is not None and (M - 1) * ldc2 + (N - n_split) > _room(out2):
            raise ValueError(f"gemm.out2: {M} rows of stride {ldc2} x {N - n_split} columns do not fit the destination ({_room(out2)} elements from its start)")
    args = GemmArgs()
    args.A, args.W, args.C = a.data_ptr(), w.data_ptr(), out.data_ptr()
    args.bias = bias.data_ptr() if bias is not None else None
    args.gate = gate.data_ptr() if gate is not None else None
    args.resid = resid.data_ptr() if resid is not None else None
    args.M, args.N, args.K = M, N, K
    args.lda, args.a_rows_per_batch, args.a_batch_stride = lda, a_rows_per_batch, a_batch_stride
    args.ldc, args.c_rows_per_batch, args.c_batch_stride = ldc, c_rows_per_batch, c_batch_stride
    args.ldg, args.act, args.act_n0, args.out_f32 = ldg, act, act_n0, int(out_f32)
    if out2 is not None:
        _need(out2, torch.bfloat16, "gemm.out2")
        args.C2, args.ldc2, args.n_split = out2.data_ptr(), ldc2, n_split
    return args, out, (M, N, K)


def _recorded(call, shape, kind=False):
    if _recorder is None:
        call()
        return
    s_ev, e_ev = torch.cuda.Event(enable_timing=True), torch.cuda.Event(enable_timing=True)
    s_ev.record()
    call()
    e_ev.record()
    M, N, K = shape
    _recorder.events.append((s_ev, e_ev, 2.0 * M * N * K))
    _recorder.shapes.append(shape)
    _recorder.is_conv.append(kind)


def _recorded_attention(call, B, S, H, qprep, vrow):
    if _recorder is None:
        call()
        return
    fam = _lib.load().drag_attention_bf16_choice(S, int(vrow), int(qprep))
    q = "true" if qprep else "false"
    gen = get_option("attn_gen")
    variant = f", {gen - 10}" if experiments_built() and 11 <= gen <= 29 else ""
    name = {64: f"attention_q64_kernel<{q}>", 640: f"attention_q64g_kernel<{q}, false>", 641: f"attention_q64g_kernel<{q}, true{variant}>"}.get(
        fam, f"attention_d128_kernel<{fam}, ..., {q}, ...>")
    s_ev, e_ev = torch.cuda.Event(enable_timing=True), torch.cuda.Event(enable_timing=True)
    s_ev.record()
    call()
    e_ev.record()
    _recorder.attn.append((s_ev, e_ev, 4.0 * S * S * 128 * H * B, name))


_gemm_workspaces: dict[int, torch.Tensor] = {}
_retired_workspaces: list[torch.Tensor] = []
_workspace_stream: dict[int, int] = {}


def _workspace_guard(a: torch.Tensor) -> None:
    idx = a.device.index
    if idx != torch.cuda.current_device():
        raise RuntimeError(f"gemm: operands on cuda:{idx} but the current device is cuda:{torch.cuda.current_device()} "
                           "(the library launches on — and takes the split-K workspace of — the current device)")
    if torch.cuda.is_current_stream_capturing():
        return
    st = torch.cuda.current_stream()
    last = _workspace_stream.get(idx)
    if last is not None and last != st.cuda_stream:
        ev = torch.cuda.Event()
        ev.record(torch.cuda.ExternalStream(last, device=a.device) if last != 0 else torch.cuda.default_stream(a.device))
        st.wait_event(ev)
    _workspace_stream[idx] = st.cuda_stream


def gemm_workspace(device: torch.device, mbytes: int | None = None) -> None:
    import os
    idx = device.index if device.index is not None else torch.cuda.current_device()
    if mbytes is None:
        mbytes = int(os.environ.get("DRAG_GEMM_WORKSPACE_MB", "64"))
    lib = _lib.load()
    if torch.cuda.is_current_stream_capturing():
        raise RuntimeError("gemm_workspace: not during stream capture (the buffer must outlive the graph: register it before capturing)")
    old = _gemm_workspaces.get(idx)
    if old is not None and old.numel() > 0:
        _retired_workspaces.append(old)
    with torch.cuda.device(idx):
        if mbytes <= 0:
            _gemm_workspaces[idx] = torch.empty(0, dtype=torch.uint8, device=device)
            check(lib.drag_gemm_set_workspace(None, 0), "drag_gemm_set_workspace")
            return
        ws = torch.empty(mbytes << 20, dtype=torch.uint8, device=device)
        check(lib.drag_gemm_set_workspace(ctypes.c_void_p(ws.data_ptr()), ws.numel()), "drag_gemm_set_workspace")
        _gemm_workspaces[idx] = ws


def gemm(a: torch.Tensor, w: torch.Tensor, out: torch.Tensor | None = None, *, bias=None, act: int = ACT_NONE,
         act_n0: int = 0, gate=None, resid=None, out_f32: bool = False, M: int | None = None,
         a_rows_per_batch: int = 0, a_batch_stride: int = 0, lda: int | None = None,
         c_rows_per_batch: int = 0, c_batch_stride: int = 0, ldc: int | None = None, ldg: int = 0,
         out2: torch.Tensor | None = None, ldc2: int = 0, n_split: int = 0) -> torch.Tensor:
    lib = _lib.load()
    if a.is_cuda and a.device.index not in _gemm_workspaces and not torch.cuda.is_current_stream_capturing():
        gemm_workspace(a.device)
    if a.is_cuda:
        _workspace_guard(a)
    args, out, shape = _gemm_args(a, w, out, bias, act, act_n0, gate, resid, out_f32, M, a_rows_per_batch, a_batch_stride, lda,
                                  c_rows_per_batch, c_batch_stride, ldc, ldg, out2, ldc2, n_split)
    slices = lib.drag_gemm_bf16_splitk_slices(ctypes.byref(args)) if _recorder is not None else 0
    _recorded(lambda: check(lib.drag_gemm_bf16(ctypes.byref(args), _stream()), "drag_gemm_bf16"), shape, ("splitk", slices) if slices else False)
    return out


def gemm_cost(M: int, N: int, K: int, M2: int = 0) -> int:
    return int(_lib.load().drag_gemm_bf16_cost(M, M2, N, K))


def gemm_pair(first: dict, second: dict):
    lib = _lib.load()
    packed = []
    for kw in (first, second):
        kw = dict(kw)
        a, w, out = kw.pop("a"), kw.pop("w"), kw.pop("out", None)
        d = dict(bias=None, act=ACT_NONE, act_n0=0, gate=None, resid=None, out_f32=False, M=None, a_rows_per_batch=0, a_batch_stride=0,
                 lda=None, c_rows_per_batch=0, c_batch_stride=0, ldc=None, ldg=0)
        unknown = set(kw) - set(d)
        if unknown:
            raise TypeError(f"gemm_pair: unexpected arguments {sorted(unknown)}")
        d.update(kw)
        packed.append(_gemm_args(a, w, out, d["bias"], d["act"], d["act_n0"], d["gate"], d["resid"], d["out_f32"], d["M"], d["a_rows_per_batch"],
                                 d["a_batch_stride"], d["lda"], d["c_rows_per_batch"], d["c_batch_stride"], d["ldc"], d["ldg"], None, 0, 0))
    (a1, o1, s1), (a2, o2, s2) = packed
    if s1[1:] != s2[1:]:
        raise ValueError(f"gemm_pair: the two problems must share N and K (got {s1} and {s2})")
    if (a1.act, a1.act_n0, a1.out_f32) != (a2.act, a2.act_n0, a2.out_f32):
        raise ValueError("gemm_pair: the two problems must share activation, act_n0 and output type")
    if first["a"].is_cuda and first["a"].device.index not in _gemm_workspaces and not torch.cuda.is_current_stream_capturing():
        gemm_workspace(first["a"].device)
    if first["a"].is_cuda:
        _workspace_guard(first["a"])
    slices = lib.drag_gemm_bf16_pair_splitk_slices(ctypes.byref(a1), ctypes.byref(a2))
    if slices:
        _recorded(lambda: check(lib.drag_gemm_bf16_pair(ctypes.byref(a1), ctypes.byref(a2), _stream()), "drag_gemm_bf16_pair"),
                  (s1[0] + s2[0], s1[1], s1[2]), ("splitk", slices))
    elif lib.drag_gemm_bf16_pair_merges(s1[0], s2[0], s1[1], s1[2]):
        _recorded(lambda: check(lib.drag_gemm_bf16_pair(ctypes.byref(a1), ctypes.byref(a2), _stream()), "drag_gemm_bf16_pair"),
                  (s1[0] + s2[0], s1[1], s1[2]), ("pair", s1[0], s2[0]))
    else:
        for args_i, s_i in ((a1, s1), (a2, s2)):
            sl = lib.drag_gemm_bf16_splitk_slices(ctypes.byref(args_i)) if _recorder is not None else 0
            _recorded(lambda: check(lib.drag_gemm_bf16(ctypes.byref(args_i), _stream()), "drag_gemm_bf16"), s_i, ("splitk", sl) if sl else False)
    return o1, o2


def qk_norm_rope_vt(qkv: torch.Tensor, vt: torch.Tensor, wq_txt, wk_txt, wq_img, wk_img, rope_cos, rope_sin,
                    B: int, S: int, H: int, ld: int, s_txt: int, eps: float = 1e-6) -> None:
    lib = _lib.load()
    _need(qkv, torch.bfloat16, "qkv")
    _need(vt, torch.bfloat16, "vt")
    if rope_cos is not None:
        _need(rope_cos, torch.float32, "rope_cos")
    check(lib.drag_qk_norm_rope_vt_bf16(_p(qkv), _p(vt), _p(wq_txt), _p(wk_txt), _p(wq_img), _p(wk_img),
                                        _p(rope_cos), _p(rope_sin), B, S, H, ld, s_txt, eps, _stream()),
          "drag_qk_norm_rope_vt_bf16")


def attention(q: torch.Tensor, k: torch.Tensor, vt: torch.Tensor, out: torch.Tensor, B: int, S: int, H: int,
              ld_qk: int, qk_batch_stride: int, ld_o: int, o_batch_stride: int, scale: float) -> None:
    lib = _lib.load()
    _need(q, torch.bfloat16, "q")
    _need(out, torch.bfloat16, "out")
    _recorded_attention(lambda: check(lib.drag_attention_bf16(_p(q), _p(k), _p(vt), _p(out), B, S, H, ld_qk, qk_batch_stride, ld_o,
                                                              o_batch_stride, scale, _stream()), "drag_attention_bf16"), B, S, H, False, False)


def k_norm_rope_vt(qkv: torch.Tensor, vt: torch.Tensor, wk_txt, wk_img, rope_cos, rope_sin, B: int, S: int, H: int, ld: int,
                   s_txt: int, eps: float = 1e-6) -> None:
    lib = _lib.load()
    _need(qkv, torch.bfloat16, "qkv")
    if vt is not None:
        _need(vt, torch.bfloat16, "vt")
    check(lib.drag_k_norm_rope_vt_bf16(_p(qkv), _p(vt), _p(wk_txt), _p(wk_img), _p(rope_cos), _p(rope_sin), B, S, H, ld, s_txt,
                                       eps, _stream()), "drag_k_norm_rope_vt_bf16")


def attention_qprep(q: torch.Tensor, k: torch.Tensor, vt: torch.Tensor, out: torch.Tensor, B: int, S: int, H: int, ld_qk: int,
                    qk_batch_stride: int, ld_o: int, o_batch_stride: int, scale: float, wq_txt, wq_img, rope_cos, rope_sin,
                    s_txt: int, eps: float = 1e-6) -> None:
    lib = _lib.load()
    _need(q, torch.bfloat16, "q")
    _need(out, torch.bfloat16, "out")
    if rope_cos is not None:
        _need(rope_cos, torch.float32, "rope_cos")
    _recorded_attention(lambda: check(lib.drag_attention_qprep_bf16(_p(q), _p(k), _p(vt), _p(out), B, S, H, ld_qk, qk_batch_stride, ld_o,
                                                                    o_batch_stride, scale, _p(wq_txt), _p(wq_img), _p(rope_cos), _p(rope_sin),
                                                                    s_txt, eps, _stream()), "drag_attention_qprep_bf16"), B, S, H, True, False)


def attention_v(q: torch.Tensor, k: torch.Tensor, v: torch.Tensor, out: torch.Tensor, B: int, S: int, H: int, ld_qk: int,
                qk_batch_stride: int, ld_o: int, o_batch_stride: int, scale: float, wq_txt=None, wq_img=None, rope_cos=None,
                rope_sin=None, s_txt: int = 0, eps: float = 1e-6) -> None:
    lib = _lib.load()
    _need(q, torch.bfloat16, "q")
    _need(v, torch.bfloat16, "v")
    _need(out, torch.bfloat16, "out")
    if rope_cos is not None:
        _need(rope_cos, torch.float32, "rope_cos")
    _recorded_attention(lambda: check(lib.drag_attention_v_bf16(_p(q), _p(k), _p(v), _p(out), B, S, H, ld_qk, qk_batch_stride, ld_o, o_batch_stride,
                                                                scale, _p(wq_txt), _p(wq_img), _p(rope_cos), _p(rope_sin), s_txt, eps, _stream()),
                                      "drag_attention_v_bf16"), B, S, H, wq_txt is not None, True)


def layernorm(x: torch.Tensor, y: torch.Tensor, M: int, D: int, *, scale=None, shift=None, gamma=None, beta=None,
              ldx: int | None = None, rows_per_batch: int = 0, x_batch_stride: int = 0, ldy: int | None = None,
              ld_mod: int = 0, eps: float = 1e-6) -> torch.Tensor:
    lib = _lib.load()
    _need(x, torch.bfloat16, "x")
    _need(y, torch.bfloat16, "y")
    check(lib.drag_layernorm_modulate_bf16(_p(x), _p(y), _p(scale), _p(shift), _p(gamma), _p(beta), M, D,
                                           ldx if ldx is not None else D, rows_per_batch, x_batch_stride,
                                           ldy if ldy is not None else D, ld_mod, eps, _stream()),
          "drag_layernorm_modulate_bf16")
    return y


def act(x: torch.Tensor, kind: int, out: torch.Tensor | None = None) -> torch.Tensor:
    lib = _lib.load()
    _need(x, torch.bfloat16, "x")
    if out is None:
        out = torch.empty_like(x)
    check(lib.drag_act_bf16(_p(x), _p(out), x.numel(), kind, _stream()), "drag_act_bf16")
    return out


def timestep_embedding(t: torch.Tensor, dim: int) -> torch.Tensor:
    lib = _lib.load()
    _need(t, torch.float32, "t")
    out = torch.empty((t.numel(), dim), dtype=torch.bfloat16, device=t.device)
    check(lib.drag_timestep_embedding_bf16(_p(t), _p(out), t.numel(), dim, _stream()), "drag_timestep_embedding_bf16")
    return out


def flow_euler_step(x: torch.Tensor, v: torch.Tensor, dt: float) -> None:
    lib = _lib.load()
    _need(x, torch.bfloat16, "x")
    _need(v, torch.bfloat16, "v")
    check(lib.drag_flow_euler_step_bf16(_p(x), _p(v), dt, x.numel(), _stream()), "drag_flow_euler_step_bf16")


def add(a: torch.Tensor, b: torch.Tensor, out: torch.Tensor | None = None) -> torch.Tensor:
    lib = _lib.load()
    _need(a, torch.bfloat16, "a")
    if out is None:
        out = torch.empty_like(a)
    check(lib.drag_add_bf16(_p(a), _p(b), _p(out), a.numel(), _stream()), "drag_add_bf16")
    return out


def to_bf16(x: torch.Tensor) -> torch.Tensor:
    lib = _lib.load()
    _need(x, torch.float32, "x")
    out = torch.empty(x.shape, dtype=torch.bfloat16, device=x.device)
    check(lib.drag_cast_f32_to_bf16(_p(x), _p(out), x.numel(), _stream()), "drag_cast_f32_to_bf16")
    return out


def to_f32(x: torch.Tensor) -> torch.Tensor:
    lib = _lib.load()
    _need(x, torch.bfloat16, "x")
    out = torch.empty(x.shape, dtype=torch.float32, device=x.device)
    check(lib.drag_cast_bf16_to_f32(_p(x), _p(out), x.numel(), _stream()), "drag_cast_bf16_to_f32")
    return out


def _need_rows(t: torch.Tensor, name: str):
    if t.dim() != 2 or not t.is_contiguous():
        raise ValueError(f"{name}: expected a contiguous [rows, d] matrix (got shape {tuple(t.shape)}, strides {t.stride()}); "
                         "call .contiguous() on views")


def cosine_topk(corpus: torch.Tensor, queries: torch.Tensor, k: int):
# ... 328 lines not shown
```

include/domainrag_hip.h:

```cpp
#ifndef DOMAINRAG_HIP_H
#define DOMAINRAG_HIP_H
#include <stdint.h>
#ifdef __cplusplus
extern "C" {
#endif

int drag_version(void);
const char* drag_last_error(void);
int drag_set_option(const char* name, int32_t value);
int drag_get_option(const char* name, int32_t* value);
const char* drag_option_name(int32_t index);
int drag_experiments_built(void);

#define DRAG_ACT_NONE 0
#define DRAG_ACT_GELU_TANH 1
#define DRAG_ACT_SILU 2
#define DRAG_ACT_QUICK_GELU 3
#define DRAG_ACT_GELU_ERF 4

typedef struct drag_gemm_args {
  const void* A;
  const void* W;
  void* C;
  const void* bias;
  const void* gate;
  const void* resid;
  int32_t M, N, K;
  int32_t lda, a_rows_per_batch;
  int64_t a_batch_stride;
  int32_t ldc, c_rows_per_batch;
  int64_t c_batch_stride;
  int32_t ldg;
  int32_t act, act_n0;
  int32_t out_f32;
  void* C2;
  int32_t ldc2, n_split;
} drag_gemm_args;
int drag_gemm_bf16(const drag_gemm_args* args, void* stream);
int drag_gemm_bf16_pair(const drag_gemm_args* a, const drag_gemm_args* b, void* stream);
int drag_gemm_bf16_pair_merges(int M1, int M2, int N, int K);
int drag_gemm_bf16_choice(int M1, int M2, int N, int K);
int drag_conv3x3_bf16_choice(int64_t M, int Cout, int Cin);
int64_t drag_gemm_bf16_cost(int M1, int M2, int N, int K);
int drag_gemm_set_workspace(void* ptr, int64_t bytes);
int drag_gemm_bf16_splitk_slices(const drag_gemm_args* args);
int drag_gemm_bf16_pair_splitk_slices(const drag_gemm_args* a, const drag_gemm_args* b);

typedef struct drag_conv_args {
  const void* x;
  const void* w;
  void* y;
  const void* bias;
  const void* resid;
  int32_t B, Ho, Wo, Hp, Wp, Cin, Cout, ldy, stride, oy, ox, act;
} drag_conv_args;
int drag_conv3x3_bf16(const drag_conv_args* args, void* stream);

int drag_qk_norm_rope_vt_bf16(void* qkv, void* vt, const void* wq_txt, const void* wk_txt,
                              const void* wq_img, const void* wk_img, const float* rope_cos,
                              const float* rope_sin, int32_t B, int32_t S, int32_t H, int32_t ld,
                              int32_t s_txt, float eps, void* stream);

int drag_attention_bf16(const void* q, const void* k, const void* vt, void* out, int32_t B,
                        int32_t S, int32_t H, int32_t ld_qk, int64_t qk_batch_stride, int32_t ld_o,
                        int64_t o_batch_stride, float scale, void* stream);

int drag_k_norm_rope_vt_bf16(void* qkv, void* vt, const void* wk_txt, const void* wk_img, const float* rope_cos,
                             const float* rope_sin, int32_t B, int32_t S, int32_t H, int32_t ld, int32_t s_txt,
                             float eps, void* stream);
int drag_attention_qprep_bf16(const void* q, const void* k, const void* vt, void* out, int32_t B, int32_t S, int32_t H,
                              int32_t ld_qk, int64_t qk_batch_stride, int32_t ld_o, int64_t o_batch_stride, float scale,
                              const void* wq_txt, const void* wq_img, const float* rope_cos, const float* rope_sin,
                              int32_t s_txt, float eps, void* stream);
int drag_attention_v_bf16(const void* q, const void* k, const void* v, void* out, int32_t B, int32_t S, int32_t H, int32_t ld_qk,
                          int64_t qk_batch_stride, int32_t ld_o, int64_t o_batch_stride, float scale, const void* wq_txt,
                          const void* wq_img, const float* rope_cos, const float* rope_sin, int32_t s_txt, float eps, void* stream);

int drag_attention_bf16_choice(int32_t S, int32_t v_row_major, int32_t q_prep);

int drag_layernorm_modulate_bf16(const void* x, void* y, const void* scale, const void* shift,
                                 const void* gamma, const void* beta, int32_t M, int32_t D,
                                 int32_t ldx, int32_t rows_per_batch, int64_t x_batch_stride,
                                 int32_t ldy, int32_t ld_mod, float eps, void* stream);

int drag_act_bf16(const void* x, void* y, int64_t n, int32_t act, void* stream);
int drag_timestep_embedding_bf16(const float* t, void* out, int32_t B, int32_t dim, void* stream);
int drag_flow_euler_step_bf16(void* x, const void* v, float dt, int64_t n, void* stream);
int drag_add_bf16(const void* a, const void* b, void* y, int64_t n, void* stream);
int drag_cast_f32_to_bf16(const float* x, void* y, int64_t n, void* stream);
int drag_cast_bf16_to_f32(const void* x, float* y, int64_t n, void* stream);

int drag_patchify_u8(const void* img, void* out, int32_t B, int32_t H, int32_t W, int32_t P, int32_t ldo,
                     const float* mean3, const float* std3, void* stream);
int drag_scale_sum_bf16(const void* x, const float* scales, void* out, int32_t G, int32_t N, int64_t elems,
                        void* stream);

int64_t drag_cosine_topk_workspace_bytes(int64_t N, int32_t Q);
int drag_cosine_topk_f32(const float* corpus, const float* queries, int64_t N, int32_t d,
                         int32_t Q, int32_t k, float* out_d, int64_t* out_i, void* workspace,
                         void* stream);
int drag_cosine_scores_f32(const float* corpus, const float* queries, int64_t N, int32_t d, int32_t Q,
                           float* scores, void* stream);
int64_t drag_resnet_stem_style_workspace_bytes(int32_t B, int32_t H, int32_t W);
int drag_resnet_stem_style_f32(const float* img, const float* conv_w, const float* bn_scale, const float* bn_shift,
                               float* out, int32_t B, int32_t H, int32_t W, float eps, void* workspace, void* stream);
typedef struct drag_resample_args {
  const uint8_t* src;
  uint8_t* dst;
  uint8_t* tmp;
  int32_t batch, channels;
  int32_t src_h, src_w;
  int64_t src_image_stride;
  int32_t src_row_stride;
  int32_t out_h, out_w;
  int64_t dst_image_stride;
  int32_t dst_row_stride;
  const int32_t* kx;
  const int32_t* bx;
  int32_t ksize_x;
  const int32_t* ky;
  const int32_t* by;
  int32_t ksize_y;
  int32_t tmp_row0, tmp_rows;
  int32_t src_col0, src_row0;
} drag_resample_args;
int drag_resample_u8(const drag_resample_args* args, void* stream);
int drag_patchify_f32_nchw(const float* img, void* out, int32_t B, int32_t H, int32_t W, int32_t P, int32_t ldo,
                           void* stream);
int drag_l2_normalize_f32(float* x, int64_t rows, int32_t d, void* stream);

int64_t drag_groupnorm_workspace_bytes(int32_t B, int32_t H, int32_t W, int32_t C);
int drag_groupnorm_silu_bf16(const void* x, void* y, const void* gamma, const void* beta, int32_t B,
                             int32_t H, int32_t W, int32_t C, int32_t groups, int32_t out_pad,
                             int32_t silu, float eps, void* workspace, void* stream);
int drag_pad_copy_bf16(const void* x, void* y, int32_t B, int32_t H, int32_t W, int32_t C, int32_t upsample,
                       void* stream);
int drag_softmax_rows_f32_bf16(const float* x, void* y, int64_t rows, int32_t cols, int32_t ldy, float scale,
                               void* stream);
int drag_unpack_latents_bf16(const void* tokens, void* y, int32_t B, int32_t h, int32_t w, int32_t ld, int32_t C,
                             float scaling, float shift, void* stream);
int drag_sample_pack_latents_bf16(const void* moments, const void* noise, void* tokens, int32_t B, int32_t H,
                                  int32_t W, int32_t ldm, int32_t ld, float scaling, float shift, void* stream);
int drag_image_preprocess_u8(const void* img, const void* mask, void* y, int32_t B, int32_t H, int32_t W, int32_t C,
                             void* stream);
int drag_image_postprocess_u8(const void* x, void* out, int64_t npix, int32_t ld, void* stream);
int drag_mask_pack_u8(const void* mask, void* tokens, int32_t B, int32_t H, int32_t W, int32_t ld, void* stream);
int drag_flow_euler_rows_bf16(void* x, const void* v, int64_t rows, int32_t cols, int32_t ldx, int32_t ldv, float dt,
                              void* stream);
int drag_scale_noise_rows_bf16(void* x, const void* noise, int64_t rows, int32_t cols, int32_t ldx, int32_t ldn,
                               float sigma, void* stream);

#define DRAG_PAD_ZERO 0
#define DRAG_PAD_REFLECT 1
#define DRAG_CONV_ACT_NONE 0
#define DRAG_CONV_ACT_RELU 1
#define DRAG_CONV_ACT_SIGMOID 2
// ... 73 lines not shown
```

Baseline: 0.4957 images/s.

## Compute only image-row queries and MLP in the last single-stream block

In the final single-stream transformer block only the image tokens feed proj_out, so this computes Q, the MLP and the output projection for image rows only, while K and V still cover the whole sequence. It adds a query-row-window option to the attention kernels that skips query blocks below the first image row and masks stores below it. Separately, the 4-wave GEMM kernel gains two-segment (pair) support, so paired GEMMs can use it and the pair-merge heuristic changes. The cost is more GEMM launches in that block and extra kernel arguments and branches.

```diff
diff --git a/domain-rag_amd/_lib.py b/domain-rag_amd/_lib.py
--- a/domain-rag_amd/_lib.py
+++ b/domain-rag_amd/_lib.py
@@ -63,6 +63,8 @@
     "drag_k_norm_rope_vt_bf16": (c_int, [c_void_p] * 6 + [c_int] * 5 + [c_float, c_void_p]),
     "drag_attention_qprep_bf16": (c_int, [c_void_p] * 4 + [c_int] * 4 + [c_int64, c_int, c_int64, c_float] + [c_void_p] * 4 + [c_int, c_float, c_void_p]),
     "drag_attention_bf16_choice": (c_int, [c_int, c_int, c_int]),
+    "drag_attention_win_bf16": (c_int, [c_void_p] * 4 + [c_int] * 4 + [c_int64, c_int, c_int64, c_float, c_int, c_void_p]),
+    "drag_attention_qprep_win_bf16": (c_int, [c_void_p] * 4 + [c_int] * 4 + [c_int64, c_int, c_int64, c_float] + [c_void_p] * 4 + [c_int, c_float, c_int, c_void_p]),
     "drag_attention_v_bf16": (c_int, [c_void_p] * 4 + [c_int] * 4 + [c_int64, c_int, c_int64, c_float] + [c_void_p] * 4 + [c_int, c_float, c_void_p]),
     "drag_layernorm_modulate_bf16": (c_int, [c_void_p] * 6 + [c_int] * 4 + [c_int64, c_int, c_int, c_float, c_void_p]),
     "drag_act_bf16": (c_int, [c_void_p, c_void_p, c_int64, c_int, c_void_p]),
diff --git a/domain-rag_amd/csrc/attention.hip b/domain-rag_amd/csrc/attention.hip
--- a/domain-rag_amd/csrc/attention.hip
+++ b/domain-rag_amd/csrc/attention.hip
@@ -118,6 +118,7 @@
   float eps;
   int tune;
   int items;
+  int q_blk0, q_lo;
 };
 
 constexpr float DEFER_THR = 8.0f;
@@ -131,7 +132,7 @@
   const int hh = l >> 5;
   constexpr int QB = NW * 32;
   constexpr int CPW = 16 / NW;
-  const int nqb = (p.S + QB - 1) / QB;
+  const int nqb = (p.S - p.q_blk0 + QB - 1) / QB;
   const int xcd = blockIdx.x & 7;
   int loc = blockIdx.x >> 3;
   const int nloc = ((p.B * p.H + 7) / 8) * nqb;
@@ -146,7 +147,7 @@
     ov = VROW ? ok : (unsigned)((((long long)(bb * p.H + hd)) * 128) * p.s_pad * 2);
   };
   item_offsets(loc, b, h, soK, soV);
-  q0 = (loc - (loc / nqb) * nqb) * QB + w * 32;
+  q0 = p.q_blk0 + (loc - (loc / nqb) * nqb) * QB + w * 32;
 
   bf16x8_t qf[8];
   __amdgpu_buffer_rsrc_t rsK, rsV;
@@ -423,9 +424,9 @@
         const auto r0 = __builtin_amdgcn_permlane32_swap(a0, b0, false, false);
         const auto r1 = __builtin_amdgcn_permlane32_swap(a1, b1, false, false);
         const u32x4_t o = {r0[0], r1[0], r0[1], r1[1]};
-        if (qrow < p.S) *(u32x4_t*)(op + 32 * dt + 8 * g) = o;
-      }
-  } else if (qrow < p.S) {
+        if (qrow < p.S && qrow >= p.q_lo) *(u32x4_t*)(op + 32 * dt + 8 * g) = o;
+      }
+  } else if (qrow < p.S && qrow >= p.q_lo) {
     bf16_t* op = p.out + (long long)b * p.o_bs + (long long)qrow * p.ld_o + h * 128 + 4 * hh;
 #pragma unroll
     for (int dt = 0; dt < 4; ++dt)
@@ -440,7 +441,7 @@
   if (!has_next) break;
   loc += lstep;
   item_offsets(loc, b, h, soK, soV);
-  q0 = (loc - (loc / nqb) * nqb) * QB + w * 32;
+  q0 = p.q_blk0 + (loc - (loc / nqb) * nqb) * QB + w * 32;
   }
   }
 }
@@ -530,14 +531,14 @@
   ATTN_STAMP(0);
   const int hh = l >> 5;
   constexpr int QB = 256, CPW = 4;
-  const int nqb = (p.S + QB - 1) / QB;
+  const int nqb = (p.S - p.q_blk0 + QB - 1) / QB;
   struct Item { int b, h, q0; };
   auto decode = [&](int item, Item& t) -> bool {
     const int xcd = item & 7, loc = item >> 3;
     const int bh = (loc / nqb) * 8 + xcd;
     t.b = bh / p.H;
     t.h = bh - t.b * p.H;
-    t.q0 = (loc - (loc / nqb) * nqb) * QB + w * 64;
+    t.q0 = p.q_blk0 + (loc - (loc / nqb) * nqb) * QB + w * 64;
     return bh < p.B * p.H;
   };
   int item = (int)blockIdx.x;
@@ -918,9 +919,9 @@
           const auto r0 = __builtin_amdgcn_permlane32_swap(a0, b0, false, false);
           const auto r1 = __builtin_amdgcn_permlane32_swap(a1, b1, false, false);
           const u32x4_t o = {r0[0], r1[0], r0[1], r1[1]};
-          if (qrow < p.S) *(u32x4_t*)(op + 32 * dt + 8 * g) = o;
+          if (qrow < p.S && qrow >= p.q_lo) *(u32x4_t*)(op + 32 * dt + 8 * g) = o;
         }
-    } else if (qrow < p.S) {
+    } else if (qrow < p.S && qrow >= p.q_lo) {
       bf16_t* op = p.out + (long long)b * p.o_bs + (long long)qrow * p.ld_o + h * 128 + 4 * (le >> 5);
 #pragma unroll
       for (int dt = 0; dt < 4; ++dt)
@@ -935,7 +936,7 @@
   }
   ATTN_STAMP(3 + 2 * (p.s_pad / 64));
   if (!has_next) break;
-  stores_behind = q0 + 64 <= p.S ? ((p.tune & 2) ? 16 : 32) : 0;
+  stores_behind = q0 + 64 <= p.S && q0 >= p.q_lo ? ((p.tune & 2) ? 16 : 32) : 0;
   wait_older_than_stores();
   q_fragments(nxt, le);
   q_to_agprs();
@@ -963,14 +964,14 @@
   extern __shared__ __attribute__((aligned(16))) char smem[];
   const int w = wave_id(), l = lane_id();
   constexpr int QB = 256, CPW = 4;
-  const int nqb = (p.S + QB - 1) / QB;
+  const int nqb = (p.S - p.q_blk0 + QB - 1) / QB;
   struct Item { int b, h, q0; };
   auto decode = [&](int item, Item& t) -> bool {
     const int xcd = item & 7, loc = item >> 3;
     const int bh = (loc / nqb) * 8 + xcd;
     t.b = bh / p.H;
     t.h = bh - t.b * p.H;
-    t.q0 = (loc - (loc / nqb) * nqb) * QB + w * 64;
+    t.q0 = p.q_blk0 + (loc - (loc / nqb) * nqb) * QB + w * 64;
     return bh < p.B * p.H;
   };
   int item = (int)blockIdx.x;
@@ -1169,9 +1170,9 @@
             const auto r0 = __builtin_amdgcn_permlane32_swap(a0, b0, false, false);
             const auto r1 = __builtin_amdgcn_permlane32_swap(a1, b1, false, false);
             const u32x4_t o = {r0[0], r1[0], r0[1], r1[1]};
-            if (qrow < p.S) *(u32x4_t*)(op + 32 * dt + 8 * g) = o;
+            if (qrow < p.S && qrow >= p.q_lo) *(u32x4_t*)(op + 32 * dt + 8 * g) = o;
           }
-      } else if (qrow < p.S) {
+      } else if (qrow < p.S && qrow >= p.q_lo) {
         bf16_t* op = p.out + (long long)b * p.o_bs + (long long)qrow * p.ld_o + h * 128 + 4 * (le >> 5);
 #pragma unroll
         for (int dt = 0; dt < 4; ++dt)
@@ -1185,7 +1186,7 @@
       }
     }
     if (!has_next) break;
-    stores_behind = q0 + 64 <= p.S ? ((p.tune & 2) ? 16 : 32) : 0;
+    stores_behind = q0 + 64 <= p.S && q0 >= p.q_lo ? ((p.tune & 2) ? 16 : 32) : 0;
     wait_older_than_stores();
     q_fragments(nxt, le, qin);
     item += (int)gridDim.x;
@@ -1244,7 +1245,7 @@
 static int attention_launch(const void* q, const void* k, const void* vt, void* out, int32_t B, int32_t S, int32_t H,
                             int32_t ld_qk, int64_t qk_batch_stride, int32_t ld_o, int64_t o_batch_stride, float scale,
                             const void* wq_txt, const void* wq_img, const float* rope_cos, const float* rope_sin, int32_t s_txt,
-                            float eps, void* stream, bool vrow = false);
+                            float eps, void* stream, bool vrow = false, int32_t q_row0 = 0);
 
 static void attention_family(int32_t S, bool vrow, bool& w8, bool& q64) {
   w8 = !drag_opt(DRAG_OPT_ATTN_W4) && S >= 4096;
@@ -1283,6 +1284,27 @@
                           rope_sin, s_txt, eps, stream);
 }
 
+extern "C" int drag_attention_win_bf16(const void* q, const void* k, const void* vt, void* out, int32_t B, int32_t S, int32_t H,
+                                       int32_t ld_qk, int64_t qk_batch_stride, int32_t ld_o, int64_t o_batch_stride, float scale,
+                                       int32_t q_row0, void* stream) {
+  DRAG_CHECK(q_row0 >= 0 && q_row0 < S, "drag_attention_win_bf16: 0 <= q_row0 < S");
+  return attention_launch(q, k, vt, out, B, S, H, ld_qk, qk_batch_stride, ld_o, o_batch_stride, scale, nullptr, nullptr, nullptr,
+                          nullptr, 0, 0.f, stream, false, drag_opt(DRAG_OPT_ATTN_QWIN) == 1 ? 0 : q_row0);
+}
+
+extern "C" int drag_attention_qprep_win_bf16(const void* q, const void* k, const void* vt, void* out, int32_t B, int32_t S,
+                                             int32_t H, int32_t ld_qk, int64_t qk_batch_stride, int32_t ld_o,
+                                             int64_t o_batch_stride, float scale, const void* wq_txt, const void* wq_img,
+                                             const float* rope_cos, const float* rope_sin, int32_t s_txt, float eps,
+                                             int32_t q_row0, void* stream) {
+  DRAG_CHECK(wq_txt && wq_img && rope_cos && rope_sin,
+             "drag_attention_qprep_win_bf16: the fused q preparation needs both norm weights and both RoPE tables");
+  DRAG_CHECK(s_txt >= 0 && s_txt <= S, "drag_attention_qprep_win_bf16: 0 <= s_txt <= S");
+  DRAG_CHECK(q_row0 >= 0 && q_row0 < S, "drag_attention_qprep_win_bf16: 0 <= q_row0 < S");
+  return attention_launch(q, k, vt, out, B, S, H, ld_qk, qk_batch_stride, ld_o, o_batch_stride, scale, wq_txt, wq_img, rope_cos,
+                          rope_sin, s_txt, eps, stream, false, drag_opt(DRAG_OPT_ATTN_QWIN) == 1 ? 0 : q_row0);
+}
+
 extern "C" int drag_attention_v_bf16(const void* q, const void* k, const void* v, void* out, int32_t B, int32_t S, int32_t H,
                                      int32_t ld_qk, int64_t qk_batch_stride, int32_t ld_o, int64_t o_batch_stride, float scale,
                                      const void* wq_txt, const void* wq_img, const float* rope_cos, const float* rope_sin,
@@ -1311,17 +1333,18 @@
 static int attention_launch(const void* q, const void* k, const void* vt, void* out, int32_t B, int32_t S, int32_t H,
                             int32_t ld_qk, int64_t qk_batch_stride, int32_t ld_o, int64_t o_batch_stride, float scale,
                             const void* wq_txt, const void* wq_img, const float* rope_cos, const float* rope_sin, int32_t s_txt,
-                            float eps, void* stream, bool vrow) {
+                            float eps, void* stream, bool vrow, int32_t q_row0) {
   DRAG_CHECK(q && k && vt && out, "drag_attention_bf16: null pointer");
   DRAG_CHECK(B > 0 && S > 0 && H > 0, "drag_attention_bf16: bad shape");
   DRAG_CHECK(ld_qk % 8 == 0 && ld_o % 4 == 0, "drag_attention_bf16: ld_qk %% 8, ld_o %% 4 required");
+  DRAG_CHECK(q_row0 >= 0 && q_row0 < S, "drag_attention_bf16: 0 <= q_row0 < S");
   AttnArgs p;
   p.q = (const bf16_t*)q; p.k = (const bf16_t*)k; p.vt = (const bf16_t*)vt; p.v = (const bf16_t*)vt; p.out = (bf16_t*)out;
   p.B = B; p.S = S; p.H = H; p.ld_qk = ld_qk; p.ld_o = ld_o; p.s_pad = (S + 63) / 64 * 64;
   p.qk_bs = qk_batch_stride; p.o_bs = o_batch_stride;
   p.c = scale * 1.4426950408889634f;
   p.wq_txt = (const bf16_t*)wq_txt; p.wq_img = (const bf16_t*)wq_img; p.cosT = rope_cos; p.sinT = rope_sin;
-  p.s_txt = s_txt; p.eps = eps;
+  p.s_txt = s_txt; p.eps = eps; p.q_lo = q_row0; p.q_blk0 = q_row0 & ~63;
   const long long kspan = ((long long)(S - 1) * ld_qk + 128) * 2;
   const long long vspan = (long long)128 * p.s_pad * 2;
   DRAG_CHECK(kspan < (1ll << 31), "drag_attention_bf16: K span must be < 2 GiB per (batch, head)");
@@ -1333,7 +1356,7 @@
   bool w8, q64;
   attention_family(S, vrow, w8, q64);
   const int QB = (w8 || q64) ? 256 : 128;
-  const int nqb2 = (S + QB - 1) / QB;
+  const int nqb2 = (S - p.q_blk0 + QB - 1) / QB;
   const dim3 grid(8 * groups * nqb2);
   const int sched = drag_opt(DRAG_OPT_ATTN_SCHED);
   const bool qprep = wq_txt != nullptr;
diff --git a/domain-rag_amd/csrc/drag_common.h b/domain-rag_amd/csrc/drag_common.h
--- a/domain-rag_amd/csrc/drag_common.h
+++ b/domain-rag_amd/csrc/drag_common.h
@@ -101,7 +101,9 @@
   X(GEMM_NARROW, "gemm_narrow", 0, DRAG_OPT_PRODUCT)        \
   X(CONV_NO_SMALL_COUT, "conv_no_small_cout", 0, DRAG_OPT_PRODUCT) \
   X(CONV_NO_LIN, "conv_no_lin", 0, DRAG_OPT_PRODUCT)        \
-  X(CONV_TILE, "conv_tile", 0, DRAG_OPT_PRODUCT)
+  X(CONV_TILE, "conv_tile", 0, DRAG_OPT_PRODUCT)            \
+  X(ATTN_QWIN, "attn_qwin", 0, DRAG_OPT_PRODUCT)            \
+  X(GEMM_W4_PAIR, "gemm_w4_pair", 0, DRAG_OPT_PRODUCT)
 #define DRAG_OPT_ENUM(id, name, def, exp) DRAG_OPT_##id,
 enum { DRAG_OPTIONS(DRAG_OPT_ENUM) DRAG_OPT_COUNT };
 #undef DRAG_OPT_ENUM
diff --git a/domain-rag_amd/csrc/gemm_bf16.hip b/domain-rag_amd/csrc/gemm_bf16.hip
--- a/domain-rag_amd/csrc/gemm_bf16.hip
+++ b/domain-rag_amd/csrc/gemm_bf16.hip
@@ -918,17 +918,23 @@
   u32x4_t rsA, rsW;
   u32x16_t vo;
   int m0, n0;
+  int seg;
 };
 __device__ __forceinline__ void w4_tile_state(const GemmKArgs& p, int tile, int w, int l, bool valid, W4Tile& t) {
   auto uni = [](uint32_t v) { return (uint32_t)__builtin_amdgcn_readfirstlane((int)v); };
   int tm, tn;
   pick_tile(p, tile, tm, tn);
+  const bool seg2 = p.seg_tiles_m > 0 && tm >= p.seg_tiles_m;
+  if (seg2) tm -= p.seg_tiles_m;
+  const int M = seg2 ? p.M2 : p.M;
+  const RowMap am = seg2 ? p.am2 : p.am;
   const int m0 = __builtin_amdgcn_readfirstlane(tm * 256), n0 = __builtin_amdgcn_readfirstlane(tn * 256);
   t.m0 = m0;
   t.n0 = n0;
-  long long a0 = p.am.off(m0);
+  t.seg = __builtin_amdgcn_readfirstlane(seg2 ? 1 : 0);
+  long long a0 = am.off(m0);
   const int wrows = min(256, p.N - n0);
-  const bf16_t *Ab = p.A, *Wb = p.W;
+  const bf16_t *Ab = seg2 ? p.A2 : p.A, *Wb = seg2 ? p.W2 : p.W;
   if (p.w_boff) {
     const int sl = m0 / p.am.rpb, r = m0 - sl * p.am.rpb;
     Wb += (long long)sl * p.w_boff;
@@ -938,8 +944,8 @@
     }
   }
   const unsigned long long pa = (unsigned long long)(uintptr_t)(Ab + a0), pw = (unsigned long long)(uintptr_t)(Wb + (long long)n0 * p.ldw);
-  const bool interior = m0 + 256 <= p.M && wrows == 256 && m0 / p.am.rpb == (m0 + 255) / p.am.rpb;
-  const long long a_span = interior ? ((long long)255 * p.am.ld + p.K) * 2 : (p.am.off(min(m0 + 255, p.M - 1)) - a0 + p.K) * 2;
+  const bool interior = m0 + 256 <= M && wrows == 256 && m0 / am.rpb == (m0 + 255) / am.rpb;
+  const long long a_span = interior ? ((long long)255 * am.ld + p.K) * 2 : (am.off(min(m0 + 255, M - 1)) - a0 + p.K) * 2;
   t.rsA = (u32x4_t){uni((uint32_t)pa), uni((uint32_t)(pa >> 32) & 0xffffu), valid ? uni((uint32_t)a_span) : 0u, 0x00020000u};
   t.rsW = (u32x4_t){uni((uint32_t)pw), uni((uint32_t)(pw >> 32) & 0xffffu), valid ? uni((uint32_t)(((long long)(wrows - 1) * p.ldw + p.K) * 2)) : 0u, 0x00020000u};
   if (interior) {
@@ -947,7 +953,7 @@
     for (int i = 0; i < 8; ++i) {
       const int row = (w * 8 + i) * 8 + (l >> 3);
       const int slot = (l & 7) ^ ((row >> 1) & 7);
-      t.vo[i] = (unsigned)((row * p.am.ld + slot * 8) * 2);
+      t.vo[i] = (unsigned)((row * am.ld + slot * 8) * 2);
       t.vo[8 + i] = (unsigned)((row * p.ldw + slot * 8) * 2);
     }
     return;
@@ -956,8 +962,8 @@
   for (int i = 0; i < 8; ++i) {
     const int row = (w * 8 + i) * 8 + (l >> 3);
     const int slot = (l & 7) ^ ((row >> 1) & 7);
-    const int ra = min(m0 + row, p.M - 1);
-    t.vo[i] = (unsigned)((p.am.off(ra) - a0 + slot * 8) * 2);
+    const int ra = min(m0 + row, M - 1);
+    t.vo[i] = (unsigned)((am.off(ra) - a0 + slot * 8) * 2);
     const int rw = min(row, wrows - 1);
     t.vo[8 + i] = (unsigned)(((long long)rw * p.ldw + slot * 8) * 2);
   }
@@ -988,6 +994,7 @@
   auto args_now = [&]() {
     GemmKArgs q = p;
     asm volatile("" : "+s"(q.tiles_n), "+s"(q.tiles_m), "+s"(q.group_m), "+s"(q.am.rpb), "+s"(q.cm.rpb), "+s"(q.M), "+s"(q.K), "+s"(q.am.ld), "+s"(q.cm.ld), "+s"(q.ldw));
+    asm volatile("" : "+s"(q.seg_tiles_m), "+s"(q.am2.rpb), "+s"(q.cm2.rpb), "+s"(q.M2), "+s"(q.am2.ld), "+s"(q.cm2.ld));
     return q;
   };
   auto read_addrs = [&](int lv) {
@@ -1046,7 +1053,11 @@
       for (int ni = 0; ni < 8; ++ni)
 #pragma unroll
         for (int r = 0; r < 4; ++r) acc[mi][ni][r] = accrow[mi][4 * ni + r];
-    const GemmKArgs pe = args_now();
+    GemmKArgs pe = args_now();
+    if (cur.seg) {
+      pe.C = pe.Cs2; pe.bias = pe.bias2; pe.gate = pe.gate2; pe.resid = pe.resid2;
+      pe.M = pe.M2; pe.ldg = pe.ldg2; pe.wide = pe.wide2; pe.cm = pe.cm2;
+    }
     const int m0 = cur.m0, n0 = cur.n0;
     const GemmKArgs pd = dest_of(pe, n0);
     bool fast = false;
@@ -1371,7 +1382,7 @@
   const int force = drag_opt(DRAG_OPT_GEMM_KERNEL);
   long long cost = 0;
   int choice;
-  const bool w4_ok = M2 == 0 && N >= 256 && K >= 256 && K % 128 == 0;
+  const bool w4_ok = (M2 == 0 || drag_opt(DRAG_OPT_GEMM_W4_PAIR) != 1) && N >= 256 && K >= 256 && K % 128 == 0;
   if (force >= 10) choice = force;
   else if (force == 3) choice = w4_ok ? 3 : ((N >= 256 && K >= 256) ? 2 : 0);
   else if (force == 2) choice = (N >= 256 && K >= 256) ? 2 : 0;
@@ -1379,7 +1390,7 @@
   else if (use_t256(M1, M2, N, K)) {
     choice = 2;
     cost = ((tile_rows(M1, M2, 256) * ((N + 255) / 256) + 255) / 256) * (256 + 256);
-    const long long tiles4 = tile_rows(M1, 0, 256) * ((N + 255) / 256);
+    const long long tiles4 = tile_rows(M1, M2, 256) * ((N + 255) / 256);
     const int w4 = drag_opt(DRAG_OPT_GEMM_W4);
     const bool enough = w4 == 2 ? true : w4 == 3 ? tiles4 >= 256 : tiles4 >= 256 && (K >= 8192 || tiles4 >= 768);
     if (w4_ok && w4 != 1 && enough) choice = 3;
@@ -1407,7 +1418,7 @@
     if (b) { k.seg_tiles_m = k.tiles_m; k.tiles_m += (b->M + tm - 1) / tm; }
   };
   if (choice == 3) {
-    k.tiles_m = (a->M + 255) / 256; k.tiles_n = (a->N + 255) / 256;
+    tiles_of(256); k.tiles_n = (a->N + 255) / 256;
     if (drag_opt(DRAG_OPT_GEMM_GROUP_M) <= 0) k.group_m = a->N >= 16384 ? 2 : (a->N <= 3072 && a->K < 8192 ? 8 : 4);
     constexpr int lds4 = 131072 + 4 * 4096;
     static unsigned long long ready4 = 0;
@@ -1621,10 +1632,15 @@
   long long c1 = 0, c2 = 0, cm = 0;
   const int k1 = gemm_choice(M1, 0, N, K, &c1);
   const int k2 = gemm_choice(M2, 0, N, K, &c2);
-  gemm_choice(M1, M2, N, K, &cm);
+  const int km = gemm_choice(M1, M2, N, K, &cm);
   if (cm <= 0) return 0;
   auto persistent = [](int k) { return k == 2 || k == 3; };
-  return cm < c1 + c2 || (cm == c1 + c2 && (!persistent(k1) || !persistent(k2)));
+  auto short_8wave = [&](int k, long long M) {
+    const long long rounds = (tile_rows(M, 0, 256) * ((N + 255) / 256) + 255) / 256;
+    return k == 2 && rounds * K < 3 * 3072;
+  };
+  const bool to_4wave = km == 3 && ((k1 == 3 && short_8wave(k2, M2)) || (k2 == 3 && short_8wave(k1, M1)));
+  return cm < c1 + c2 || (cm == c1 + c2 && (!persistent(k1) || !persistent(k2) || to_4wave));
 }
 
 extern "C" int drag_gemm_bf16_pair(const drag_gemm_args* a, const drag_gemm_args* b, void* stream) {
diff --git a/domain-rag_amd/flux.py b/domain-rag_amd/flux.py
--- a/domain-rag_amd/flux.py
+++ b/domain-rag_amd/flux.py
@@ -236,10 +236,14 @@
         cat_mlp = catb.view(-1)[D:]
         fused_qkv_mlp = (3 * D) % 256 == 0 and (_FUSED_QKV_MLP if _FUSED_QKV_MLP is not None else
                                                 ops.gemm_cost(M, 3 * D + F, D) * 10 <= (ops.gemm_cost(M, 3 * D, D) + ops.gemm_cost(M, F, D)) * 9)
+        image_rows_only = taps is None and len(self.single) > 0 and ops.get_option("attn_qwin") == 0
         for i, blk in enumerate(self.single):
             mo = self.mod_off[("s", i)]
             ops.layernorm(x, nrm, M, D, scale=modv[mo + D:], shift=modv[mo:], ldx=D, ld_mod=LM, rows_per_batch=S,
                           x_batch_stride=S * D)
+            if image_rows_only and i == len(self.single) - 1:
+                self._last_single_image_rows(blk, ws, modv, mo, cos, sin, B, St, Si, scale)
+                break
             if fused_qkv_mlp:
                 ops.gemm(nrm, blk["wqkvm"], out=qkv, bias=blk["bqkvm"], act=ops.ACT_GELU_TANH, act_n0=3 * D, M=M, lda=D, ldc=3 * D,
                          out2=cat_mlp, ldc2=D + F, n_split=3 * D)
@@ -264,6 +268,37 @@
         ops.gemm(nrm_img, self.w["proj_out.weight"], out=ws["out"], bias=self.w["proj_out.bias"], M=Mi, lda=D,
                  ldc=cfg.out_channels)
         return ws["out"].view(B, Si, cfg.out_channels)
+
+    def _last_single_image_rows(self, blk, ws, modv, mo, cos, sin, B, St, Si, scale):
+        cfg = self.cfg
+        D, H = cfg.dim, cfg.num_attention_heads
+        F = cfg.mlp_ratio * D
+        S = St + Si
+        M, Mi, LM = B * S, B * Si, self.mod_total
+        x, nrm, qkv, vt, catb = ws["x"], ws["nrm"], ws["qkv"], ws["vt"], ws["cat"]
+        x_img = x.view(-1)[St * D:]
+        nrm_img = nrm.view(-1)[St * D:]
+        cat_img = catb.view(-1)[St * (D + F):]
+        w, bias = blk["wqkvm"], blk["bqkvm"]
+        ops.gemm(nrm, w[D: 3 * D], out=qkv.view(-1)[D:], bias=bias[D: 3 * D], M=M, lda=D, ldc=3 * D)
+        ops.gemm(nrm_img, w[:D], out=qkv.view(-1)[St * 3 * D:], bias=bias[:D], M=Mi, a_rows_per_batch=Si, a_batch_stride=S * D, lda=D,
+                 c_rows_per_batch=Si, c_batch_stride=S * 3 * D, ldc=3 * D)
+        Sq0 = St & ~63
+        if Sq0 < St:
+            ops.gemm(nrm.view(-1)[Sq0 * D:], w[:D], out=qkv.view(-1)[Sq0 * 3 * D:], bias=bias[:D], M=B * (St - Sq0),
+                     a_rows_per_batch=St - Sq0, a_batch_stride=S * D, lda=D, c_rows_per_batch=St - Sq0, c_batch_stride=S * 3 * D,
+                     ldc=3 * D)
+        ops.gemm(nrm_img, w[3 * D:], out=cat_img[D:], bias=bias[3 * D:], act=ops.ACT_GELU_TANH, M=Mi, a_rows_per_batch=Si,
+                 a_batch_stride=S * D, lda=D, c_rows_per_batch=Si, c_batch_stride=S * (D + F), ldc=D + F)
+        if _SEPARATE_QPREP:
+            ops.qk_norm_rope_vt(qkv, vt, blk["nq"], blk["nk"], blk["nq"], blk["nk"], cos, sin, B, S, H, 3 * D, 0)
+            ops.attention_win(qkv, qkv.view(-1)[D:], vt, catb, B, S, H, 3 * D, S * 3 * D, D + F, S * (D + F), scale, St)
+        else:
+            ops.k_norm_rope_vt(qkv, vt, blk["nk"], blk["nk"], cos, sin, B, S, H, 3 * D, 0)
+            ops.attention_qprep_win(qkv, qkv.view(-1)[D:], vt, catb, B, S, H, 3 * D, S * 3 * D, D + F, S * (D + F), scale,
+                                    blk["nq"], blk["nq"], cos, sin, 0, St)
+        ops.gemm(cat_img, blk["wo"], out=x_img, bias=blk["bo"], M=Mi, a_rows_per_batch=Si, a_batch_stride=S * (D + F), lda=D + F,
+                 c_rows_per_batch=Si, c_batch_stride=S * D, ldc=D, gate=modv[mo + 2 * D:], resid=x_img, ldg=LM)
 
     MAX_GRAPHS = 3
 
diff --git a/domain-rag_amd/ops.py b/domain-rag_amd/ops.py
--- a/domain-rag_amd/ops.py
+++ b/domain-rag_amd/ops.py
@@ -180,7 +180,7 @@
     _recorder.is_conv.append(kind)
 
 
-def _recorded_attention(call, B, S, H, qprep, vrow):
+def _recorded_attention(call, B, S, H, qprep, vrow, q_rows=None):
     if _recorder is None:
         call()
         return
@@ -194,7 +194,7 @@
     s_ev.record()
     call()
     e_ev.record()
-    _recorder.attn.append((s_ev, e_ev, 4.0 * S * S * 128 * H * B, name))
+    _recorder.attn.append((s_ev, e_ev, 4.0 * (S if q_rows is None else q_rows) * S * 128 * H * B, name))
 
 
 _gemm_workspaces: dict[int, torch.Tensor] = {}
@@ -341,6 +341,38 @@
                                                                     s_txt, eps, _stream()), "drag_attention_qprep_bf16"), B, S, H, True, False)
 
 
+def _window_rows(S: int, q_row0: int) -> int:
+    if not 0 <= q_row0 < S:
+        raise ValueError(f"attention: q_row0 = {q_row0} outside [0, {S})")
+    return S if get_option("attn_qwin") == 1 else S - (q_row0 & ~63)
+
+
+def attention_win(q: torch.Tensor, k: torch.Tensor, vt: torch.Tensor, out: torch.Tensor, B: int, S: int, H: int, ld_qk: int,
+                  qk_batch_stride: int, ld_o: int, o_batch_stride: int, scale: float, q_row0: int) -> None:
+    lib = _lib.load()
+    _need(q, torch.bfloat16, "q")
+    _need(out, torch.bfloat16, "out")
+    rows = _window_rows(S, q_row0)
+    _recorded_attention(lambda: check(lib.drag_attention_win_bf16(_p(q), _p(k), _p(vt), _p(out), B, S, H, ld_qk, qk_batch_stride, ld_o,
+                                                                  o_batch_stride, scale, q_row0, _stream()), "drag_attention_win_bf16"),
+                        B, S, H, False, False, rows)
+
+
+def attention_qprep_win(q: torch.Tensor, k: torch.Tensor, vt: torch.Tensor, out: torch.Tensor, B: int, S: int, H: int, ld_qk: int,
+                        qk_batch_stride: int, ld_o: int, o_batch_stride: int, scale: float, wq_txt, wq_img, rope_cos, rope_sin,
+                        s_txt: int, q_row0: int, eps: float = 1e-6) -> None:
+    lib = _lib.load()
+    _need(q, torch.bfloat16, "q")
+    _need(out, torch.bfloat16, "out")
+    if rope_cos is not None:
+        _need(rope_cos, torch.float32, "rope_cos")
+    rows = _window_rows(S, q_row0)
+    _recorded_attention(lambda: check(lib.drag_attention_qprep_win_bf16(_p(q), _p(k), _p(vt), _p(out), B, S, H, ld_qk, qk_batch_stride, ld_o,
+                                                                        o_batch_stride, scale, _p(wq_txt), _p(wq_img), _p(rope_cos),
+                                                                        _p(rope_sin), s_txt, eps, q_row0, _stream()),
+                                      "drag_attention_qprep_win_bf16"), B, S, H, True, False, rows)
+
+
 def attention_v(q: torch.Tensor, k: torch.Tensor, v: torch.Tensor, out: torch.Tensor, B: int, S: int, H: int, ld_qk: int,
                 qk_batch_stride: int, ld_o: int, o_batch_stride: int, scale: float, wq_txt=None, wq_img=None, rope_cos=None,
                 rope_sin=None, s_txt: int = 0, eps: float = 1e-6) -> None:
diff --git a/include/domainrag_hip.h b/include/domainrag_hip.h
--- a/include/domainrag_hip.h
+++ b/include/domainrag_hip.h
@@ -72,6 +72,12 @@
                               int32_t ld_qk, int64_t qk_batch_stride, int32_t ld_o, int64_t o_batch_stride, float scale,
                               const void* wq_txt, const void* wq_img, const float* rope_cos, const float* rope_sin,
                               int32_t s_txt, float eps, void* stream);
+int drag_attention_win_bf16(const void* q, const void* k, const void* vt, void* out, int32_t B, int32_t S, int32_t H, int32_t ld_qk,
+                            int64_t qk_batch_stride, int32_t ld_o, int64_t o_batch_stride, float scale, int32_t q_row0, void* stream);
+int drag_attention_qprep_win_bf16(const void* q, const void* k, const void* vt, void* out, int32_t B, int32_t S, int32_t H,
+                                  int32_t ld_qk, int64_t qk_batch_stride, int32_t ld_o, int64_t o_batch_stride, float scale,
+                                  const void* wq_txt, const void* wq_img, const float* rope_cos, const float* rope_sin,
+                                  int32_t s_txt, float eps, int32_t q_row0, void* stream);
 int drag_attention_v_bf16(const void* q, const void* k, const void* v, void* out, int32_t B, int32_t S, int32_t H, int32_t ld_qk,
                           int64_t qk_batch_stride, int32_t ld_o, int64_t o_batch_stride, float scale, const void* wq_txt,
                           const void* wq_img, const float* rope_cos, const float* rope_sin, int32_t s_txt, float eps, void* stream);
```

Result: no change. 0.4978 images/s (median of 6 runs) (+0.4%).
